# tjtiger86/dl-swin-gan

Measured on AMD Instinct MI355X. Metric: cine slices/sec (fwd+bwd) at 10-iter unroll, 1/2/4/8 GPU; PSNR vs ref, higher is better.
Workload: dtype fp32

## Files before the change

### dl-swin-gan_amd/csrc/conv3d_f16x3.hip

```cpp
#include "conv3d_common.h"
#include "f16x3_common.h"
#include <type_traits>

namespace {
__device__ uint4 g_wg_zero_row[160 / 8];
constexpr int kThinInHalfs = 2 * 4 * 4 * 160 * 8;
constexpr int kThinOutHalfs = 5 * 9 * 2 * 4 * 16 * 8;
constexpr int kThinOutW2 = 5 * 9 * 2 * 4 * 12 * 8;

DLCS_DEV f16x8_t tr_read16h(const f16* p0, const f16* p1) {
    return __builtin_bit_cast(f16x8_t, tr_read16(reinterpret_cast<const bf16*>(p0), reinterpret_cast<const bf16*>(p1)));
}

template <int EPI, int NPASS, bool PREF = true>
DLCS_DEV void conv_epilogue_h3(const ConvF32Args& a, const f32x4_t (&acc)[4][5], float* Es, int pw, int cw0,
                               int lane, int b, int pt, int pyq, int pxq, int nT, int nY, int nX,
                               f16* op, const unsigned* opmax, float* cpart) {
    const float ps = op ? f16x3_scale(*opmax) : 1.0f;
    static_assert(EPI == kEpiRes || EPI == kEpiMask, "fused forms only");
    constexpr int PC = 160 / NPASS, EL = PC + 4, NCH = PC / 8, PER = 256 * NCH / 512;
    static_assert(PC % 8 == 0 && 256 * NCH % 512 == 0 && PC <= 512, "whole 8-channel chunks per thread");
    const float* src = EPI == kEpiRes ? a.res : a.mask;
    const int sld = EPI == kEpiRes ? a.res_ld : a.mask_ld;
    const f16* mp = EPI == kEpiMask ? reinterpret_cast<const f16*>(a.mplanes) : nullptr;
    f32x4_t pre[PREF ? NPASS : 1][PER][2];
    long orows[PER];
    bool oks[PER];
#pragma unroll
    for (int k = 0; k < PER; ++k) {
        const int c = threadIdx.x + k * 512;
        const int vl = c / NCH;
        const int pwv = vl >> 6;
        const int py = pyq + (pwv >> 1), px = pxq + (pwv & 1);
        oks[k] = py < nY && px < nX;
        orows[k] = ((((long)b * nT + pt) * nY + min(py, nY - 1)) * nX + min(px, nX - 1)) * 64 + (vl & 63);
    }
    auto load_pre = [&](int pass, int slot) {
#pragma unroll
        for (int k = 0; k < PER; ++k) {
            const int c = threadIdx.x + k * 512;
            const int co = pass * PC + (c % NCH) * 8;
            if (mp) {
                const f16* q = mp + orows[k] * 320 + (co >> 5) * 64 + (co & 31);
                pre[slot][k][0] = *reinterpret_cast<const f32x4_t*>(q);
                pre[slot][k][1] = *reinterpret_cast<const f32x4_t*>(q + 32);
            } else {
                const float* sp = src + orows[k] * sld + co;
                pre[slot][k][0] = *reinterpret_cast<const f32x4_t*>(sp);
                pre[slot][k][1] = *reinterpret_cast<const f32x4_t*>(sp + 4);
            }
        }
    };
    if constexpr (PREF) {
#pragma unroll
        for (int pass = 0; pass < NPASS; ++pass) load_pre(pass, pass);
    }
    float vmax = 0.0f;
#pragma unroll
    for (int pass = 0; pass < NPASS; ++pass) {
        const int ps_ = PREF ? pass : 0;
        if constexpr (!PREF) load_pre(pass, 0);
#pragma unroll
        for (int j = 0; j < 5; ++j) {
            const int c0 = cw0 + j * 16 - pass * PC;
            if (c0 + 16 <= 0 || c0 >= PC) continue;
#pragma unroll
            for (int i = 0; i < 4; ++i)
#pragma unroll
                for (int r = 0; r < 4; ++r) {
                    const int vl = pw * 64 + i * 16 + (lane >> 4) * 4 + r;
                    const int cl = c0 + (lane & 15);
                    if (cl >= 0 && cl < PC) Es[vl * EL + cl] = acc[i][j][r];
                }
        }
        __syncthreads();
#pragma unroll
        for (int k = 0; k < PER; ++k) {
            const int c = threadIdx.x + k * 512;
            const int vl = c / NCH, ch = (c % NCH) * 8;
            const int co = pass * PC + ch;
            if (!oks[k]) {
                if (cpart) {
                    *reinterpret_cast<f32x4_t*>(Es + vl * EL + ch) = (f32x4_t)0.0f;
                    *reinterpret_cast<f32x4_t*>(Es + vl * EL + ch + 4) = (f32x4_t)0.0f;
                }
                continue;
            }
            f32x4_t v0 = *reinterpret_cast<const f32x4_t*>(Es + vl * EL + ch);
            f32x4_t v1 = *reinterpret_cast<const f32x4_t*>(Es + vl * EL + ch + 4);
            if (a.bias) {
                v0 += *reinterpret_cast<const f32x4_t*>(a.bias + co);
                v1 += *reinterpret_cast<const f32x4_t*>(a.bias + co + 4);
            }
            if (EPI == kEpiMask && mp) {
                const u32x4_h3 hb = __builtin_bit_cast(u32x4_h3, pre[ps_][k][0]);
                const u32x4_h3 lb = __builtin_bit_cast(u32x4_h3, pre[ps_][k][1]);
#pragma unroll
                for (int e = 0; e < 8; ++e) {
                    const unsigned nz = ((hb[e >> 1] | lb[e >> 1]) >> (16 * (e & 1))) & 0x7fffu;
                    if (e < 4) v0[e] = nz ? v0[e] : 0.0f;
                    else v1[e - 4] = nz ? v1[e - 4] : 0.0f;
                }
            } else if (EPI == kEpiMask) {
#pragma unroll
                for (int e = 0; e < 4; ++e) {
                    v0[e] = pre[ps_][k][0][e] > 0.0f ? v0[e] : 0.0f;
                    v1[e] = pre[ps_][k][1][e] > 0.0f ? v1[e] : 0.0f;
                }
            } else {
                v0 += a.res_scale * pre[ps_][k][0];
                v1 += a.res_scale * pre[ps_][k][1];
            }
            if (a.relu_out) {
#pragma unroll
                for (int e = 0; e < 4; ++e) { v0[e] = fmaxf(v0[e], 0.0f); v1[e] = fmaxf(v1[e], 0.0f); }
            }
            if (a.out) {
                float* o = a.out + orows[k] * a.cout_ld + co;
                *reinterpret_cast<f32x4_t*>(o) = v0;
                *reinterpret_cast<f32x4_t*>(o + 4) = v1;
            }
            if (op) put_planes8(op, orows[k], co, v0, v1, ps);
            if (cpart) {
                *reinterpret_cast<f32x4_t*>(Es + vl * EL + ch) = v0;
                *reinterpret_cast<f32x4_t*>(Es + vl * EL + ch + 4) = v1;
            }
            if (a.omax) {
#pragma unroll
                for (int e = 0; e < 4; ++e) vmax = fmaxf(vmax, fmaxf(fabsf(v0[e]), fabsf(v1[e])));
            }
        }
        if (cpart) {
            constexpr int G = 512 / PC;
            __syncthreads();
            float* red = Es + 256 * EL;
            const int t = threadIdx.x;
            if (t < G * PC) {
                const int cc = t % PC, g = t / PC;
                float cs = 0.0f;
                for (int r = g; r < 256; r += G) cs += Es[r * EL + cc];
                red[g * PC + cc] = cs;
            }
            __syncthreads();
            if (t < PC) {
                float cs = 0.0f;
#pragma unroll
                for (int g = 0; g < G; ++g) cs += red[g * PC + t];
                cpart[pass * PC + t] = cs;
            }
        }
        __syncthreads();
    }
    if (a.omax) {
        vmax = wave_max(vmax);
        if ((threadIdx.x & 63) == 0 && vmax > 0.0f && vmax > __uint_as_float(__atomic_load_n(a.omax, __ATOMIC_RELAXED)))
            atomicMax(a.omax, __float_as_uint(vmax));
    }
}

#include "conv3d_f16x3.inc"
#include "conv3d_thin_f16x3.inc"
#include "conv3d_thin_planes.inc"

}

using namespace dlcs_internal;

extern "C" {

#ifdef DLCS_DIAG_BUILD
int dlcs_debug_h3_stamps(void* host, int64_t n) {
    return (int)hipMemcpyFromSymbol(host, HIP_SYMBOL(g_h3_stamps), (size_t)n * 8, 0, hipMemcpyDeviceToHost);
}
#endif

size_t dlcs_conv3d_k3_f16x3_workspace_bytes(int64_t B, int64_t D, int64_t H, int64_t W, int has_colsum) {
    const long ntile = conv_tiles(B, D, H, W);
    return ws_align(colsum_part_bytes(ntile, has_colsum != 0)) + conv_tail_bytes(ntile);
}

int dlcs_conv3d_k3_f16x3(const void* xplanes, const void* wpacked, const float* bias, float* out, int64_t cout_ld,
                         int64_t B, int64_t D, int64_t H, int64_t W, const float* mask, int64_t mask_ld,
                         const float* residual, int64_t res_ld, float res_scale, int accumulate, int relu_out,
                         unsigned* out_max, void* out_planes, float* colsum, const void* mask_planes,
                         void* workspace, size_t workspace_bytes, dlcs_stream_t stream) {
    DLCS_CHECK_ARG(xplanes && wpacked && B > 0 && (out || (out_planes && !accumulate)) && !(mask && mask_planes));
    if (!out) cout_ld = 160;
    const long rows = (long)B * D * H * W;
    if (D % 4 || H % 4 || W % 4 || cout_ld % 4 || !al16(xplanes) || !al16(wpacked) || !al16(out) ||
        (mask && (mask_ld % 4 || !al16(mask))) || (residual && (res_ld % 4 || !al16(residual))) || (bias && !al16(bias)) ||
        rows * 320 >= (1L << 31))
        return DLCS_ERR_UNSUPPORTED_SIZE;
    ConvH3Args v{};
    v.xp = (const f16*)xplanes; v.wp = (const f16*)wpacked;
    v.xmax = planes_trailer(xplanes, rows); v.wmax = (const unsigned*)((const char*)wpacked + kW3Bytes);
    v.bias = bias; v.out = out; v.mask = mask; v.res = residual;
    v.B = (int)B; v.D = (int)D; v.H = (int)H; v.W = (int)W;
    v.cout_ld = (int)cout_ld; v.mask_ld = (int)mask_ld; v.res_ld = (int)res_ld; v.accumulate = accumulate;
    v.relu_out = relu_out; v.res_scale = res_scale; v.omax = out_max;
    if (mask_planes && !al16(mask_planes)) return DLCS_ERR_UNSUPPORTED_SIZE;
    v.mplanes = mask_planes;
    if (out_planes) {
        if (cout_ld != 160 || !al16(out_planes)) return DLCS_ERR_UNSUPPORTED_SIZE;
        v.oplanes = (f16*)out_planes; v.opmax = planes_trailer(out_planes, rows);
    }
#ifdef DLCS_DIAG_BUILD
    static const int stamps = [] { const char* e = dlcs_knob("DLCS_CONV_STAMP"); return e && e[0] == '1'; }();
    v.stamp = stamps;
    static const int h3_exp = [] { const char* e = dlcs_knob("DLCS_H3_EXP"); return e ? atoi(e) : 0; }();
    v.exp = h3_exp;
#endif
    hipStream_t st = (hipStream_t)stream;
    const long ntile = conv_tiles(B, D, H, W);
    if (!ws_ok(workspace, workspace_bytes, dlcs_conv3d_k3_f16x3_workspace_bytes(B, D, H, W, colsum != nullptr)))
        return DLCS_ERR_WORKSPACE;
    if (colsum) v.cpart = static_cast<float*>(workspace);
    float* tail_ws = reinterpret_cast<float*>(static_cast<char*>(workspace) +
                                              ws_align(colsum_part_bytes(ntile, colsum != nullptr)));
    const int rc = conv_f16x3_launch(v, tail_ws, st);
    if (rc || !colsum) return rc;
    return launch_colsum_parts(v.cpart, (int)ntile, colsum, st);
}

size_t dlcs_conv3d_k3_wgrad_f16x3_workspace_bytes(int64_t B, int64_t D, int64_t H, int64_t W) {
    return (size_t)wgh3_ranges(B * (D / 4) * (H / 4) * (W / 4), true).nr * kWgSlabBytes;
}

int dlcs_conv3d_k3_wgrad_f16x3(const void* xplanes, const void* gplanes, float* dw_packed, int64_t B, int64_t D,
                               int64_t H, int64_t W, void* workspace, size_t workspace_bytes,
                               dlcs_stream_t stream) {
    DLCS_CHECK_ARG(xplanes && gplanes && dw_packed && B > 0);
    const long rows = (long)B * D * H * W;
    if (D % 4 || H % 4 || W % 4 || !al16(xplanes) || !al16(gplanes) || rows * 320 >= (1L << 40))
        return DLCS_ERR_UNSUPPORTED_SIZE;
    WgradH3Args v{};
    v.xp = (const f16*)xplanes; v.gp = (const f16*)gplanes;
    v.xmax = planes_trailer(xplanes, rows); v.gmax = planes_trailer(gplanes, rows);
    v.dw = dw_packed; v.B = (int)B; v.D = (int)D; v.H = (int)H; v.W = (int)W;
    if (!ws_ok(workspace, workspace_bytes, dlcs_conv3d_k3_wgrad_f16x3_workspace_bytes(B, D, H, W)))
        return DLCS_ERR_WORKSPACE;
    v.part = static_cast<float*>(workspace);
    return wgrad_f16x3_launch(v, (hipStream_t)stream);
}

size_t dlcs_conv3d_thin_pack_f16x3_bytes(int kind) {
    return (size_t)(kind == 0 ? kThinInHalfs : kThinOutHalfs) * 2 + 256;
}

int dlcs_conv3d_thin_pack_f16x3(const float* wpacked, int64_t cout, int64_t cout_pad, int64_t cin, int64_t cin_pad,
                                int kind, void* out, dlcs_stream_t stream) {
    DLCS_CHECK_ARG(wpacked && out && (kind == 0 || kind == 1) && cout <= cout_pad && cin <= cin_pad);
    if (kind == 0 ? !(cout == 160 && cout_pad == 160 && cin >= 1 && cin <= 4)
                  : !(cin == 160 && cin_pad == 160 && cout >= 1 && cout <= 4))
        return DLCS_ERR_UNSUPPORTED_SIZE;
    if ((uintptr_t)out & 15) return DLCS_ERR_UNSUPPORTED_SIZE;
    hipStream_t st = (hipStream_t)stream;
    const int halfs = kind == 0 ? kThinInHalfs : kThinOutHalfs;
    unsigned* mx = reinterpret_cast<unsigned*>(reinterpret_cast<char*>(out) + (size_t)halfs * 2 + 16);
    if (hipMemsetAsync(mx, 0, 4, st) != hipSuccess) return dlcs_launch_status();
    const long n = 27L * cout_pad * cin_pad;
    const int rc = launch_absmax_flat(wpacked, n, mx, (unsigned)std::min<long>(64, (n / 4 + 255) / 256), st);
    if (rc) return rc;
    hipLaunchKernelGGL(pack_thin_f16x3_grid_kernel, dim3((unsigned)((halfs / 2 + 255) / 256)), dim3(256), 0, st,
                       wpacked, (int)cout, (int)cout_pad, (int)cin, (int)cin_pad, kind, (const unsigned*)mx, (f16*)out);
    return dlcs_launch_status();
}

size_t dlcs_conv3d_thin_f16x3_workspace_bytes(int64_t B, int64_t D, int64_t H, int64_t W, int has_colsum) {
    return colsum_part_bytes(conv_tiles(B, D, H, W), has_colsum != 0);
}

int dlcs_conv3d_thin_f16x3(const float* in, int64_t cin, int64_t cin_ld, const unsigned* in_max, const void* wthin,
                           const float* bias, float* out, int64_t cout, int64_t cout_ld, int64_t B, int64_t D,
                           int64_t H, int64_t W, const float* mask, int64_t mask_ld, const float* residual,
                           int64_t res_ld, float res_scale, int accumulate, int relu_out, unsigned* out_max,
                           void* out_planes, float* colsum, const void* mask_planes, void* workspace,
                           size_t workspace_bytes, dlcs_stream_t stream) {
    DLCS_CHECK_ARG(in && in_max && wthin && B > 0 && (out || out_planes) && !(mask && mask_planes));
    if (!out) cout_ld = 160;
    const long rows = (long)B * D * H * W;
    if (D % 4 || H % 4 || W % 4 || cin_ld % 4 || cout_ld % 4 || !al16(in) || !al16(out) || !al16(wthin) ||
        (bias && !al16(bias)) || rows * std::max(cin_ld, cout_ld) >= (1L << 31) || rows / 64 >= (1L << 24))
        return DLCS_ERR_UNSUPPORTED_SIZE;
    const bool thin_in = cin >= 1 && cin <= 4 && cout == 160;
    const bool thin_out = cin == 160 && cout >= 1 && cout <= 4;
    if (!thin_in && !thin_out) return DLCS_ERR_UNSUPPORTED_SIZE;
    if (thin_in && ((mask && (mask_ld % 4 || !al16(mask))) || (residual && (res_ld % 4 || !al16(residual)))))
        return DLCS_ERR_UNSUPPORTED_SIZE;
    if (thin_out && (mask || residual || out_max || cout_ld < 4)) return DLCS_ERR_UNSUPPORTED_SIZE;
    ConvF32Args v{};
    v.in = in; v.bias = bias; v.out = out; v.mask = mask; v.res = residual;
    v.B = (int)B; v.D = (int)D; v.H = (int)H; v.W = (int)W; v.cin_ld = (int)cin_ld; v.cin_pad = (int)cin;
    v.cout_ld = (int)cout_ld; v.mask_ld = (int)mask_ld; v.res_ld = (int)res_ld; v.accumulate = accumulate;
    v.relu_out = relu_out; v.res_scale = res_scale; v.cout = (int)cout; v.cout_pad = (int)cout; v.omax = out_max;
    v.mplanes = mask_planes;
    hipStream_t st = (hipStream_t)stream;
    if (!thin_in && (out_planes || colsum || mask_planes || !out)) return DLCS_ERR_UNSUPPORTED_SIZE;
    if (mask_planes && !al16(mask_planes)) return DLCS_ERR_UNSUPPORTED_SIZE;
    if (out_planes && (!al16(out_planes) || cout_ld != 160)) return DLCS_ERR_UNSUPPORTED_SIZE;
    const unsigned* opmax = out_planes ? planes_trailer(out_planes, rows) : nullptr;
    const long ntile = conv_tiles(B, D, H, W);
    if (!ws_ok(workspace, workspace_bytes, colsum_part_bytes(ntile, colsum != nullptr))) return DLCS_ERR_WORKSPACE;
    float* cpart = colsum ? static_cast<float*>(workspace) : nullptr;
    const int rc = conv_thin_f16x3_launch(v, (const f16*)wthin, in_max, (int)cin, thin_in, st, (f16*)out_planes, opmax,
                                          cpart);
    if (rc || !colsum) return rc;
    return launch_colsum_parts(cpart, (int)ntile, colsum, st);
}

int dlcs_conv3d_thin_wgrad_f16x3(const float* in, int64_t cin, int64_t cin_ld, const unsigned* in_max,
                                 const float* g, int64_t cout, int64_t g_ld, const unsigned* g_max, float* dw_packed,
                                 int64_t cout_pad, int64_t cin_pad, float* colsum, int64_t B, int64_t D, int64_t H,
                                 int64_t W, dlcs_stream_t stream) {
    DLCS_CHECK_ARG(in && in_max && g && g_max && dw_packed && B > 0 && cout <= cout_pad && cin <= cin_pad);
    const bool thin_sfe = cout == 160 && cin >= 1 && cin <= 4;
    const bool thin_fin = cin == 160 && cout >= 1 && cout <= 4;
    const long npatch = B * (D / 4) * (H / 4) * (W / 4);
    if ((!thin_sfe && !thin_fin) || (colsum && !thin_sfe) || D % 4 || H % 4 || W % 4 || cin_ld % 4 || g_ld % 4 ||
        !al16(in) || !al16(g) || npatch >= (1L << 24))
        return DLCS_ERR_UNSUPPORTED_SIZE;
    ThinWgH3Args t{};
    t.big = thin_sfe ? g : in;
    t.thin = thin_sfe ? in : g;
    t.big_max = thin_sfe ? g_max : in_max;
    t.thin_max = thin_sfe ? in_max : g_max;
    t.dw = dw_packed; t.colsum = colsum;
    t.big_ld = (int)(thin_sfe ? g_ld : cin_ld); t.thin_ld = (int)(thin_sfe ? cin_ld : g_ld);
    t.sgn = thin_sfe ? 1 : -1; t.big_is_co = thin_sfe; t.thin_ch = (int)(thin_sfe ? cin : cout);
    t.cout_pad = (int)cout_pad; t.cin_pad = (int)cin_pad;
    t.B = (int)B; t.D = (int)D; t.H = (int)H; t.W = (int)W;
    const int nr = (int)std::min<long>(256, npatch);
    const int pp = (int)((npatch + nr - 1) / nr);
    hipLaunchKernelGGL(conv3d_wgrad_thin_f16x3_kernel, dim3(nr), dim3(512), 0, (hipStream_t)stream, t, nr, pp);
    return dlcs_launch_status();
}

int dlcs_conv3d_thin_out_planes_f16x3(const void* xplanes, const void* wthin, const float* bias, float* out,
                                      int64_t cout, int64_t cout_ld, int64_t B, int64_t D, int64_t H, int64_t W,
                                      int accumulate, int relu_out, dlcs_stream_t stream) {
    DLCS_CHECK_ARG(xplanes && wthin && out && B > 0 && cout >= 1 && cout <= 4 && cout_ld >= 4);
    if (D % 4 || H % 4 || W % 4 || cout_ld % 4 || !al16(xplanes) || !al16(wthin) || !al16(out))
        return DLCS_ERR_UNSUPPORTED_SIZE;
    ConvF32Args v{};
    v.bias = bias; v.out = out;
    v.B = (int)B; v.D = (int)D; v.H = (int)H; v.W = (int)W;
    v.cout_ld = (int)cout_ld; v.accumulate = accumulate; v.relu_out = relu_out; v.cout = (int)cout;
    v.cout_pad = (int)cout;
    return conv_thin_out_p_launch(v, (const f16*)xplanes, (const f16*)wthin, (hipStream_t)stream);
}

size_t dlcs_conv3d_thin_wgrad_planes_f16x3_workspace_bytes(void) { return (size_t)kTwpWG * 160 * 128 * sizeof(float); }

int dlcs_conv3d_thin_wgrad_planes_f16x3(const void* bigplanes, const float* thin, int64_t thin_ch, int64_t thin_ld,
                                        const unsigned* thin_max, int big_is_co, float* dw_packed, int64_t cout_pad,
                                        int64_t cin_pad, int64_t B, int64_t D, int64_t H, int64_t W, void* workspace,
                                        size_t workspace_bytes, dlcs_stream_t stream) {
    DLCS_CHECK_ARG(bigplanes && thin && thin_max && dw_packed && B > 0 && thin_ch >= 1 && thin_ch <= 4 &&
                   thin_ld >= 4);
    if (D % 4 || H % 4 || W % 4 || thin_ld % 4 || !al16(bigplanes) || !al16(thin) ||
        (big_is_co ? (cout_pad < 160 || cin_pad < thin_ch) : (cin_pad < 160 || cout_pad < thin_ch)))
        return DLCS_ERR_UNSUPPORTED_SIZE;
    ThinWgPArgs t{};
    t.bp = (const f16*)bigplanes; t.thin = thin; t.dw = dw_packed; t.thin_max = thin_max;
    t.rows = (long)B * D * H * W;
    t.thin_ld = (int)thin_ld; t.sgn = big_is_co ? 1 : -1; t.big_is_co = big_is_co ? 1 : 0; t.thin_ch = (int)thin_ch;
    t.cout_pad = (int)cout_pad; t.cin_pad = (int)cin_pad;
    t.B = (int)B; t.D = (int)D; t.H = (int)H; t.W = (int)W;
    if (!ws_ok(workspace, workspace_bytes, dlcs_conv3d_thin_wgrad_planes_f16x3_workspace_bytes()))
        return DLCS_ERR_WORKSPACE;
    t.part = static_cast<float*>(workspace);
    return wgrad_thin_p_launch(t, (hipStream_t)stream);
}

}
```

### dl-swin-gan_amd/csrc/conv3d_f16x3.inc

```
constexpr int kH3Halo = kHalo * 64;
constexpr int kH3Tap = 160 * 64;
constexpr int kH3Slot = 2 * kH3Tap;

struct ConvH3Args {
    const f16* xp; const f16* wp; const unsigned* xmax; const unsigned* wmax;
    const float* bias; float* out; const float* mask; const float* res;
    int B, D, H, W;
    int cout_ld, mask_ld, res_ld, accumulate, relu_out;
    float res_scale;
    unsigned* omax;
    float* part; int tail_base;
    f16* oplanes; const unsigned* opmax;
    float* cpart;
    const void* mplanes;
    int stamp;
    int exp;
};

#ifdef DLCS_DIAG_BUILD
__device__ unsigned long long g_h3_stamps[4096 * 73];
#define H3_STAMP(k) do { if (!TAIL && a.stamp && threadIdx.x == 0 && blockIdx.x < 4096) \
    g_h3_stamps[blockIdx.x * 73 + (k)] = __builtin_readcyclecounter(); } while (0)
#else
#define H3_STAMP(k) do { } while (0)
// ... 285 lines not shown
#pragma unroll
            for (int r = 0; r < 4; ++r)
                acc[i][j][r] *= (FOLD == 3 && ((rsgn >> (4 * (lane >> 4) + r)) & 1)) ? -inv : inv;
    if constexpr (TAIL) {
        float* pp = a.part + (long)blockIdx.x * 256 * 160;
#pragma unroll
        for (int i = 0; i < 4; ++i)
#pragma unroll
            for (int j = 0; j < 5; ++j)
#pragma unroll
                for (int r = 0; r < 4; ++r)
                    pp[(pw * 64 + i * 16 + (lane >> 4) * 4 + r) * 160 + nh * 80 + j * 16 + (lane & 15)] = acc[i][j][r];
        return;
    }
    ConvF32Args ea{};
    ea.bias = a.bias; ea.out = a.out; ea.mask = a.mask; ea.res = a.res;
    ea.cout_ld = a.cout_ld; ea.mask_ld = a.mask_ld; ea.res_ld = a.res_ld; ea.accumulate = a.accumulate;
    ea.relu_out = a.relu_out; ea.res_scale = a.res_scale; ea.omax = a.omax; ea.mplanes = a.mplanes;
    if constexpr (EPI == kEpiRes || EPI == kEpiMask)
        conv_epilogue_h3<EPI, 2>(ea, acc, reinterpret_cast<float*>(smem_h3), pw, nh * 80, lane, b, pt, tyy * 2, txx * 2,
                                 nT, nY, nX, a.oplanes, a.opmax, a.cpart ? a.cpart + (long)vb * 160 : nullptr);
    else
        conv_epilogue_f32<EPI>(ea, acc, reinterpret_cast<float*>(smem_h3), pw, nh * 80, lane, b, pt, tyy * 2, txx * 2,
                               nT, nY, nX);
    H3_STAMP(72);
}

__global__ void __launch_bounds__(256) conv_f16x3_tail_reduce_kernel(ConvH3Args a, int ntail) {
    __shared__ float red[4];
    const int nT = a.D >> 2, nY = a.H >> 2, nX = a.W >> 2;
    const int nYt = (nY + 1) >> 1, nXt = (nX + 1) >> 1;
    const int nblk = a.B * nT * nYt * nXt;
    const long i = (long)blockIdx.x * 256 + threadIdx.x;
    float vmax = 0.0f;
    if (i < (long)ntail * 256 * 40) {
        const int t = (int)(i / (256 * 40)), rem = (int)(i % (256 * 40));
        const int vl = rem / 40, c = (rem % 40) * 4;
        f32x4_t v = (f32x4_t)0.0f;
#pragma unroll
        for (int w = 0; w < 5; ++w) v += *reinterpret_cast<const f32x4_t*>(a.part + ((long)(t * 5 + w) * 256 + vl) * 160 + c);
        const int vb = a.tail_base + t;
        const int q8 = nblk >> 3, r8 = nblk & 7, xcd = vb & 7;
        int bid = xcd * q8 + min(xcd, r8) + (vb >> 3);
        const int txx = bid % nXt; bid /= nXt;
        const int tyy = bid % nYt; bid /= nYt;
        const int pt = bid % nT;
        const int b = bid / nT;
        const int pwv = vl >> 6;
        const int py = tyy * 2 + (pwv >> 1), px = txx * 2 + (pwv & 1);
        if (py < nY && px < nX) {
            const long orow = ((((long)b * nT + pt) * nY + py) * nX + px) * 64 + (vl & 63);
            if (a.bias) v += *reinterpret_cast<const f32x4_t*>(a.bias + c);
            if (a.mask) {
                const f32x4_t m = *reinterpret_cast<const f32x4_t*>(a.mask + orow * a.mask_ld + c);
#pragma unroll
                for (int e = 0; e < 4; ++e) v[e] = m[e] > 0.0f ? v[e] : 0.0f;
            } else if (a.mplanes) {
                const f16* q = reinterpret_cast<const f16*>(a.mplanes) + orow * 320 + (c >> 5) * 64 + (c & 31);
                const f16x4_t h = *reinterpret_cast<const f16x4_t*>(q), l = *reinterpret_cast<const f16x4_t*>(q + 32);
#pragma unroll
                for (int e = 0; e < 4; ++e) v[e] = (h[e] != (f16)0.0f || l[e] != (f16)0.0f) ? v[e] : 0.0f;
            }
            if (a.res) v += a.res_scale * *reinterpret_cast<const f32x4_t*>(a.res + orow * a.res_ld + c);
            if (a.relu_out) {
#pragma unroll
                for (int e = 0; e < 4; ++e) v[e] = fmaxf(v[e], 0.0f);
            }
            if (a.out) {
                float* o = a.out + orow * a.cout_ld + c;
                if (a.accumulate) v += *reinterpret_cast<const f32x4_t*>(o);
                *reinterpret_cast<f32x4_t*>(o) = v;
            }
            if (a.oplanes) put_planes4(a.oplanes, orow, c, v, f16x3_scale(*a.opmax));
            vmax = fmaxf(fmaxf(fabsf(v[0]), fabsf(v[1])), fmaxf(fabsf(v[2]), fabsf(v[3])));
        } else {
            v = (f32x4_t)0.0f;
        }
        if (a.cpart) *reinterpret_cast<f32x4_t*>(a.part + ((long)(t * 5) * 256 + vl) * 160 + c) = v;
    }
    if (a.omax) block_max_to(a.omax, vmax, red);
}

__global__ void __launch_bounds__(160) tail_colsum_kernel(ConvH3Args a, int nparts) {
    const int t = blockIdx.x, c = threadIdx.x;
    const float* p = a.part + (long)(t * nparts) * 256 * 160 + c;
    float cs = 0.0f;
    for (int r = 0; r < 256; ++r) cs += p[(long)r * 160];
    a.cpart[(long)(a.tail_base + t) * 160 + c] = cs;
}

static int conv_f16x3_launch(const ConvH3Args& v0, float* tail_ws, hipStream_t st) {
    ConvH3Args v = v0;
    unsigned nblk = (unsigned)conv_tiles(v.B, v.D, v.H, v.W);
    const char* te = dlcs_test_hook("DLCS_H3_TAIL");
    const bool tail_split = !(te && te[0] == '0');
    const unsigned ntail = tail_split ? conv_tail_tiles(nblk) : 0u, nmain = nblk - ntail;
    const bool split = ntail > 0;
    if (split) nblk = nmain;
    const int epi = conv_epi_code(v.res, v.mask || v.mplanes, !v.accumulate, true);
    if ((v.oplanes || v.cpart || v.mplanes) && epi != kEpiRes && epi != kEpiMask)
        return DLCS_ERR_UNSUPPORTED_SIZE;
    static const int fold_mode = [] {
        const char* e = dlcs_knob("DLCS_H3_FOLD");
        return !e ? 4 : e[0] == '0' ? 0 : e[0] == 'm' ? 2 : e[0] == 'a' ? 3 : e[0] == 'r' ? 4 : e[0] == 'R' ? 5 : 1;
    }();
    const bool masked = v.mask || v.mplanes;
    const int pf = fold_mode == 1 || (fold_mode == 2 && masked) ? 1 : (fold_mode == 3 && masked) ? 2
                 : (fold_mode == 5 || (fold_mode == 4 && masked)) ? 3 : 0;
    auto launch = [&](auto F) {
        constexpr int f = decltype(F)::value;
        const dim3 g(nblk);
        if (epi == 0) hipLaunchKernelGGL((conv3d_k3_f16x3_kernel<0, f>), g, dim3(512), 0, st, v);
        else if (epi == kEpiRes) hipLaunchKernelGGL((conv3d_k3_f16x3_kernel<kEpiRes, f>), g, dim3(512), 0, st, v);
        else if (epi == kEpiMask) hipLaunchKernelGGL((conv3d_k3_f16x3_kernel<kEpiMask, f>), g, dim3(512), 0, st, v);
        else hipLaunchKernelGGL((conv3d_k3_f16x3_kernel<kEpiGeneric, f>), g, dim3(512), 0, st, v);
    };
#ifdef DLCS_DIAG_BUILD
    if (pf == 1) launch(std::integral_constant<int, 1>{});
    else if (pf == 2) launch(std::integral_constant<int, 2>{});
    else
#endif
    if (pf == 3) launch(std::integral_constant<int, 3>{});
    else launch(std::integral_constant<int, 0>{});
    if (split) {
        ConvH3Args t = v;
        t.part = tail_ws;
        t.tail_base = (int)nmain;
#ifdef DLCS_DIAG_BUILD
        if (pf == 1) hipLaunchKernelGGL((conv3d_k3_f16x3_kernel<0, 1, true>), dim3(ntail * 5), dim3(512), 0, st, t);
        else if (pf == 2) hipLaunchKernelGGL((conv3d_k3_f16x3_kernel<0, 2, true>), dim3(ntail * 5), dim3(512), 0, st, t);
        else
#endif
        if (pf == 3) hipLaunchKernelGGL((conv3d_k3_f16x3_kernel<0, 3, true>), dim3(ntail * 5), dim3(512), 0, st, t);
        else hipLaunchKernelGGL((conv3d_k3_f16x3_kernel<0, 0, true>), dim3(ntail * 5), dim3(512), 0, st, t);
        hipLaunchKernelGGL(conv_f16x3_tail_reduce_kernel, dim3((unsigned)cdiv((long)ntail * 256 * 40, 256)), dim3(256),
                           0, st, t, (int)ntail);
        if (v.cpart) hipLaunchKernelGGL(tail_colsum_kernel, dim3(ntail), dim3(160), 0, st, t, 5);
    }
    return dlcs_launch_status();
}

constexpr int kWhRows = 32 + 48;
constexpr int kWhPlane = kWhRows * 160;
constexpr int kWhBuf = 2 * kWhPlane;

struct WgradH3Args {
    const f16* gp; const f16* xp;
    const unsigned* gmax; const unsigned* xmax;
    float* dw;
    float* part;
    int B, D, H, W;
};

__global__ void __launch_bounds__(768) conv3d_wgrad_f16x3_kernel(WgradH3Args a, int nrange, int ppr) {
    __shared__ __attribute__((aligned(16))) f16 smem_wh[3 * kWhBuf];
    const int b = blockIdx.x;
    int range, grp;
    {
        const int xcd = b & 7, slot = b >> 3;
        const int q = nrange >> 3;
        if ((nrange & 7) == 0) { range = (slot / 9) * 8 + xcd; grp = slot % 9; }
        else if ((nrange & 7) == 4) {
            if (slot < 9 * q) { range = (slot / 9) * 8 + xcd; grp = slot % 9; }
            else { range = 8 * q + (xcd & 3); grp = (slot - 9 * q) + (xcd < 4 ? 0 : 5); }
        } else { range = b / 9; grp = b % 9; }
    }
    if (range >= nrange || grp >= 9) return;
    const int kd = grp / 3 - 1, kh = grp % 3 - 1;
    const int nT = a.D >> 2, nY = a.H >> 2, nX = a.W >> 2;
    const int nYX = nY * nX;
    const int npatch = a.B * nT * nYX;
    const int p0 = range * ppr, p1 = min(npatch, p0 + ppr);
    if (p0 >= p1) return;
    const int lane = threadIdx.x & 63, wave = __builtin_amdgcn_readfirstlane(threadIdx.x >> 6);
    const int kwi = wave >> 2, coh = (wave >> 1) & 1, cih = wave & 1;
    const int bias_rows = (nYX + nX + 1) * 64;
    const long rows = (long)npatch * 64;

    unsigned pk[5];
#pragma unroll
    for (int k = 0; k < 5; ++k) {
        const int wi = k * 12 + wave;
        const int pl = wi >= 25 ? 1 : 0, wl = wi - pl * 25;
        const int c = wl * 64 + lane;
        const int row = c / 20, kp = c - row * 20;
        int vrow, swz;
        unsigned req = 0;
        if (wl < 10) {
            vrow = row;
            swz = (row >> 3) & 1;
        } else {
            const int hr = row - 32, ty = hr / 6, xh = hr - ty * 6;
            const int tl = ty >> 2, y = ty & 3;
            swz = (y >> 1) & 1;
            const int tt = tl + kd, yy = y + kh, xx = xh - 1;
            req = (tt < 0 ? 1u : 0u) | (tt >= 4 ? 2u : 0u) | (yy < 0 ? 4u : 0u) | (yy >= 4 ? 8u : 0u) |
                  (xx < 0 ? 16u : 0u) | (xx >= 4 ? 32u : 0u) | (tt + 2 >= 4 ? 64u : 0u);
            vrow = (((tt >> 2) * nYX + (yy >> 2) * nX + (xx >> 2)) << 6) + ((tt & 3) << 4) + ((yy & 3) << 2) +
                   (xx & 3);
        }
        const int kl = kp ^ (swz << 1);
        const unsigned off16 = (unsigned)((vrow + bias_rows) * 40 + (kl >> 2) * 8 + pl * 4 + (kl & 3));
        pk[k] = wi < 50 ? (off16 << 7) | req : 0u;
    }
    const unsigned dst0 = __builtin_amdgcn_readfirstlane(lds_offset(smem_wh));
    int ip = p0, ipt, ipy, ipx;
    {
        const int r = ip % (nT * nYX);
        ipt = r / nYX;
        ipy = (r / nX) % nY;
        ipx = r % nX;
    }
    auto missing = [&]() {
        return (ipt == 0 ? 1u : 0u) | (ipt == nT - 1 ? 2u : 0u) | (ipy == 0 ? 4u : 0u) | (ipy == nY - 1 ? 8u : 0u) |
               (ipx == 0 ? 16u : 0u) | (ipx == nX - 1 ? 32u : 0u);
    };
    auto next_patch = [&]() {
        ++ip;
        if (++ipx == nX) {
            ipx = 0;
            if (++ipy == nY) {
                ipy = 0;
                if (++ipt == nT) ipt = 0;
            }
        }
    };
    const unsigned d32 = 32 * 640, dcross = (unsigned)(nYX * 64 - 32) * 640;
    auto issue_piece = [&](int k, int th, int buf, unsigned miss, const char* gbase, const char* xbase,
                           unsigned xzero) {
        const int wi = k * 12 + wave;
        if (wi >= 50) return;
        const int pl = wi >= 25 ? 1 : 0, wl = wi - pl * 25;
        const unsigned v = pk[k];
        unsigned off = (v >> 3) & ~15u;
        if (wl < 10) {
            if (th) off += d32;
        } else {
            unsigned req = v & 63u;
            if (th) {
                const bool cross = (v & 65u) != 0u;
                off += cross ? dcross : d32;
                req = (v & 60u) | ((v >> 5) & 2u);
            }
            off = (req & miss) ? xzero : off;
        }
        glds16_s(wl < 10 ? gbase : xbase, off, dst0 + (unsigned)(buf * kWhBuf * 2 + pl * kWhPlane * 2 + wl * 1024));
    };
    auto bases = [&](const char*& gb, const char*& xb, unsigned& xz) {
        const long r0 = (long)ip * 64 - bias_rows;
        gb = reinterpret_cast<const char*>(a.gp) + r0 * 640;
        xb = reinterpret_cast<const char*>(a.xp) + r0 * 640;
        xz = (unsigned)(h3_zero_row_byte(rows) - r0 * 640);
    };

    f32x4_t acc[5][5];
#pragma unroll
    for (int i = 0; i < 5; ++i)
#pragma unroll
        for (int j = 0; j < 5; ++j) acc[i][j] = (f32x4_t)0.0f;

    const int gq = lane >> 4, q = (lane >> 2) & 3, p4 = (lane & 3) * 4, swb = gq & 1;
    auto acol = [&](int i) { return (((coh * 5 + i) ^ swb) << 4) + p4; };
    auto bcol = [&](int j) { return (((cih * 5 + j) ^ swb) << 4) + p4; };
    const int grow = (8 * gq + q) * 160;
    const int xrow = (32 + ((gq >> 1) * 4 + 2 * swb) * 6 + q + kwi) * 160;

    {
        const char *gb, *xb;
        unsigned xz;
        bases(gb, xb, xz);
        const unsigned miss = missing();
#pragma unroll
        for (int k = 0; k < 5; ++k) issue_piece(k, 0, 0, miss, gb, xb, xz);
#pragma unroll
        for (int k = 0; k < 5; ++k) issue_piece(k, 1, 1, miss, gb, xb, xz);
    }
    next_patch();
    asm volatile("s_waitcnt vmcnt(0)" ::: "memory");
    __syncthreads();
    int cur = 0;
    auto unit = [&](int TH, bool ahead) {
#pragma unroll
        for (int k = 0; k < 5; ++k) asm volatile("" : "+v"(pk[k]));
        const int nbuf = cur == 0 ? 2 : cur - 1;
        const char *gb, *xb;
        unsigned xz;
        bases(gb, xb, xz);
        const unsigned miss = missing();
        const f16* S = smem_wh + cur * kWhBuf;
        const f16* Gh = S + grow;
        const f16* Gl = S + kWhPlane + grow;
        const f16* Xh = S + xrow;
        const f16* Xl = S + kWhPlane + xrow;
        f16x8_t gh[5], gl[5];
#pragma unroll
        for (int i = 0; i < 5; ++i) gh[i] = tr_read16h(Gh + acol(i), Gh + 4 * 160 + acol(i));
        f16x8_t xh = tr_read16h(Xh + bcol(0), Xh + 6 * 160 + bcol(0));
        f16x8_t xl = tr_read16h(Xl + bcol(0), Xl + 6 * 160 + bcol(0));
#pragma unroll
        for (int j = 0; j < 5; ++j) {
            if (j == 0) {
#pragma unroll
                for (int i = 0; i < 5; ++i) gl[i] = tr_read16h(Gl + acol(i), Gl + 4 * 160 + acol(i));
            }
#pragma unroll
            for (int i = 0; i < 5; ++i) mfma16h(acc[i][j], gh[i], xh);
#pragma unroll
            for (int i = 0; i < 5; ++i) mfma16h(acc[i][j], gh[i], xl);
#pragma unroll
            for (int i = 0; i < 5; ++i) mfma16h(acc[i][j], gl[i], xh);
            if (ahead) issue_piece(j, TH, nbuf, miss, gb, xb, xz);
            if (j + 1 < 5) {
                xh = tr_read16h(Xh + bcol(j + 1), Xh + 6 * 160 + bcol(j + 1));
                xl = tr_read16h(Xl + bcol(j + 1), Xl + 6 * 160 + bcol(j + 1));
            }
        }
        if (!ahead) asm volatile("s_waitcnt vmcnt(0)" ::: "memory");
        else if (wave < 2) asm volatile("s_waitcnt vmcnt(5)" ::: "memory");
        else asm volatile("s_waitcnt vmcnt(4)" ::: "memory");
        __syncthreads();
        cur = cur == 2 ? 0 : cur + 1;
    };
    for (int u = 2 * p0; u < 2 * p1; ++u) {
        const int th = u & 1;
        unit(th, (u >> 1) + 1 < p1);
        if (th) next_patch();
    }
    const int tap = (kd + 1) * 9 + (kh + 1) * 3 + kwi;
    float* pp = a.part + ((long)range * 27 + tap) * 160 * 160;
    float* st = reinterpret_cast<float*>(smem_wh) + wave * (16 * 84);
#pragma unroll
    for (int i = 0; i < 5; ++i) {
#pragma unroll
        for (int j = 0; j < 5; ++j)
#pragma unroll
            for (int r = 0; r < 4; ++r) st[(gq * 4 + r) * 84 + j * 16 + (lane & 15)] = acc[i][j][r];
#pragma unroll
        for (int s = 0; s < 5; ++s) {
            const int e = s * 64 + lane, r = e / 20, c4 = (e % 20) * 4;
            const f32x4_t v = *reinterpret_cast<const f32x4_t*>(st + r * 84 + c4);
            *reinterpret_cast<f32x4_t*>(pp + (coh * 80 + 16 * i + r) * 160 + cih * 80 + c4) = v;
        }
    }
}

__global__ void __launch_bounds__(256) wgrad_f16x3_reduce_kernel(WgradH3Args a, int nrange) {
    const long i = (long)blockIdx.x * 256 + threadIdx.x;
    if (i >= 27L * 160 * 40) return;
    const float inv = 1.0f / (f16x3_scale(*a.gmax) * f16x3_scale(*a.xmax));
    const f32x4_t* src = reinterpret_cast<const f32x4_t*>(a.part);
    f32x4_t s = src[i];
    for (int r = 1; r < nrange; ++r) s += src[(long)r * 27 * 160 * 40 + i];
    f32x4_t* d = reinterpret_cast<f32x4_t*>(a.dw) + i;
    *d = *d + s * inv;
}

constexpr int kWgH3MaxRanges = 32;

static PatchRanges wgh3_ranges(long npatch, bool bound) {
    static const int env_nr = [] { const char* e = dlcs_knob("DLCS_WGH3_RANGES"); return e ? atoi(e) : 0; }();
    return patch_ranges(npatch, bound ? kWgH3MaxRanges : env_nr > 0 ? std::min(env_nr, kWgH3MaxRanges) : 28);
}

static int wgrad_f16x3_launch(const WgradH3Args& a, hipStream_t st) {
    const long npatch = (long)a.B * (a.D / 4) * (a.H / 4) * (a.W / 4);
    const long bias_rows = ((long)(a.H / 4) * (a.W / 4) + a.W / 4 + 1) * 64;
    if ((2 * bias_rows + 128) * 40 >= (1L << 25) || (npatch * 64 + bias_rows) * 640 + 1024 >= (1L << 32))
        return DLCS_ERR_UNSUPPORTED_SIZE;
    const PatchRanges r = wgh3_ranges(npatch, false);
    const int nr = r.nr;
    const long pp = r.pp;
    hipLaunchKernelGGL(conv3d_wgrad_f16x3_kernel, dim3((unsigned)(9 * nr)), dim3(768), 0, st, a, nr, (int)pp);
    hipLaunchKernelGGL(wgrad_f16x3_reduce_kernel, dim3((unsigned)cdiv(27L * 160 * 40, 256)), dim3(256), 0, st, a, nr);
    return dlcs_launch_status();
}
```

### dl-swin-gan_amd/csrc/conv3d_thin_planes.inc

```

constexpr int kTpHY = 10, kTpHX = 6, kTpHalo = 6 * kTpHY * kTpHX;
constexpr int kTpBuf = kTpHalo * 64;
constexpr int kTpPieces = kTpHalo * 8 / 64;

#ifdef DLCS_DIAG_BUILD
__global__ void __launch_bounds__(512, 1) conv3d_thin_out_p_kernel(ConvF32Args a, const f16* xp, const f16* wimg,
                                                                   long rows) {
    __shared__ __attribute__((aligned(16))) f16 smem_tp[2 * kTpBuf + kThinOutW2];
    f16* Wl = smem_tp + 2 * kTpBuf;
    for (int i = threadIdx.x; i < kThinOutW2 / 8; i += 512) {
        const int n = i % 12, rest = i / 12;
        const int kg = rest & 3, pl = (rest >> 2) & 1, ck = rest >> 3;
        reinterpret_cast<uint4*>(Wl)[i] = reinterpret_cast<const uint4*>(wimg)[(ck * 1024 + pl * 512 + (kg * 16 + n) * 8) / 8];
    }
    const float sx = f16x3_scale(*reinterpret_cast<const unsigned*>(reinterpret_cast<const char*>(xp) + rows * 640));
    const float inv = 1.0f / (sx * *reinterpret_cast<const float*>(wimg + kThinOutHalfs));
    const int nT = a.D >> 2, nY = a.H >> 2, nX = a.W >> 2;
    const int nYX = nY * nX, nYt = (nY + 1) >> 1;
    const int lane = threadIdx.x & 63, wave = __builtin_amdgcn_readfirstlane(threadIdx.x >> 6);
    const int m = lane & 15, kg = lane >> 4;
    const int wn = m < 12 ? m : 11;
    const int bias_rows = (nYX + nX + 1) * 64;

    unsigned pk[6];
#pragma unroll
    for (int k = 0; k < 6; ++k) {
        const int wi = 8 * k + wave;
        const int hv = min(wi * 8 + (lane >> 3), kTpHalo - 1);
        const int ht = hv / (kTpHY * kTpHX), hy = (hv / kTpHX) % kTpHY, hx = hv % kTpHX;
        const int L = (lane & 7) ^ (((hv >> 1) & 3) << 1);
        const int t = ht - 1, y = hy - 1, x = hx - 1;
        const int dt = t >> 2, dy = y >> 2, dx = x >> 2;
        const unsigned req = (dt < 0 ? 1u : 0u) | (dt > 0 ? 2u : 0u) | (dy < 0 ? 4u : 0u) | (dy == 1 ? 8u : 0u) |
                             (dy == 2 ? 16u : 0u) | (dx < 0 ? 32u : 0u) | (dx > 0 ? 64u : 0u);
        const int rel = ((dt * nYX + dy * nX + dx) << 6) + ((t & 3) << 4) + ((y & 3) << 2) + (x & 3);
        const unsigned off16 = (unsigned)((rel + bias_rows) * 40 + L);
        pk[k] = wi < kTpPieces ? (off16 << 8) | req : 0u;
    }
    const unsigned dst0 = __builtin_amdgcn_readfirstlane(lds_offset(smem_tp));
    const int nBY = (nYt + 3) >> 2, nBX = (nX + 7) >> 3;
    const int nblocks = a.B * nT * nBY * nBX, xcd = blockIdx.x & 7, kw = blockIdx.x >> 3;
    const int nrounds = xcd < nblocks ? (nblocks - xcd + 7) >> 3 : 0;
    const int nitems = nrounds * 5;
    auto decode = [&](int r, int& b, int& pt, int& py2, int& px) {
        int bid = r * 8 + xcd;
        const int bx = bid % nBX; bid /= nBX;
        const int by = bid % nBY; bid /= nBY;
        pt = bid % nT;
        b = bid / nT;
        py2 = by * 4 + (kw >> 3);
        px = bx * 8 + (kw & 7);
        return py2 < nYt && px < nX;
    };
    auto issue = [&](int s) {
        if (s >= nitems) return;
        int b, pt, py2, px;
        if (!decode(s / 5, b, pt, py2, px)) return;
        const int cc = s % 5;
        const long r0 = ((((long)b * nT + pt) * nY + 2 * py2) * nX + px) * 64 - bias_rows;
        const char* sb = reinterpret_cast<const char*>(xp) + r0 * 640 + cc * 128;
        const unsigned zoff = (unsigned)(rows * 640 + 256 - r0 * 640 - cc * 128);
        const unsigned miss = (pt == 0 ? 1u : 0u) | (pt == nT - 1 ? 2u : 0u) | (py2 == 0 ? 4u : 0u) |
                              (2 * py2 + 1 >= nY ? 8u : 0u) | (2 * py2 + 2 >= nY ? 16u : 0u) | (px == 0 ? 32u : 0u) |
                              (px == nX - 1 ? 64u : 0u);
        const unsigned dst = dst0 + (unsigned)((s & 1) * kTpBuf * 2);
#pragma unroll
        for (int k = 0; k < 6; ++k) {
            const int wi = 8 * k + wave;
            if (wi < kTpPieces) {
                const unsigned v = pk[k];
                const unsigned off = (v & miss) ? zoff : ((v >> 4) & ~15u);
                glds16_s(sb, off, dst + (unsigned)(wi * 1024));
            }
        }
    };
    int hb[3];
#pragma unroll
    for (int i = 0; i < 3; ++i) {
        const int r = 16 * (3 * (wave & 3) + i) + m;
        const int xq = r % 6, y = (r / 6) % 8, t = r / 48;
        hb[i] = (t * kTpHY + y) * kTpHX + xq;
    }
    const int kk0 = wave < 4 ? 0 : 5, kk1 = wave < 4 ? 5 : 9;
    f32x4_t acc[3];
#pragma unroll
    for (int i = 0; i < 3; ++i) acc[i] = (f32x4_t)0.0f;

    issue(0);
    asm volatile("s_waitcnt vmcnt(0)" ::: "memory");
    __syncthreads();
    for (int s = 0; s < nitems; ++s) {
#pragma unroll
        for (int k = 0; k < 6; ++k) asm volatile("" : "+v"(pk[k]));
        issue(s + 1);
        const int cc = s % 5;
        int b, pt, py2, px;
        const bool live = decode(s / 5, b, pt, py2, px);
        const f16* Hs = smem_tp + (s & 1) * kTpBuf;
        const f16* wc = Wl + cc * 9 * 768 + (kg * 12 + wn) * 8;
        for (int kk = live ? kk0 : kk1; kk < kk1; ++kk) {
            const int kd = kk / 3, kh = kk - 3 * kd;
            const f16* wb = wc + kk * 768;
            const f16x8_t bh = *reinterpret_cast<const f16x8_t*>(wb);
            const f16x8_t bl = *reinterpret_cast<const f16x8_t*>(wb + 384);
#pragma unroll
            for (int i = 0; i < 3; ++i) {
                const int R = hb[i] + (kd * kTpHY + kh) * kTpHX;
                const int swz = ((R >> 1) & 3) << 1;
                const f16x8_t ah = *reinterpret_cast<const f16x8_t*>(Hs + R * 64 + ((kg ^ swz) << 3));
                const f16x8_t al = *reinterpret_cast<const f16x8_t*>(Hs + R * 64 + (((4 + kg) ^ swz) << 3));
                f32x4_t t = (f32x4_t)0.0f;
                mfma16h(t, al, bh);
                mfma16h(t, ah, bl);
                mfma16h(t, ah, bh);
                acc[i] += t;
            }
        }
        if (cc == 4 && live) {
            __syncthreads();
            float* Q = reinterpret_cast<float*>(smem_tp + (s & 1) * kTpBuf);
#pragma unroll
            for (int i = 0; i < 3; ++i)
#pragma unroll
                for (int r = 0; r < 4; ++r)
                    Q[((wave >> 2) * 192 + 16 * (3 * (wave & 3) + i) + 4 * kg + r) * 17 + m] = acc[i][r] * inv;
#pragma unroll
            for (int i = 0; i < 3; ++i) acc[i] = (f32x4_t)0.0f;
            __syncthreads();
            if (threadIdx.x < 128) {
                const int v = threadIdx.x;
                const int t = v >> 5, y = (v >> 2) & 7, x = v & 3;
                const int py = 2 * py2 + (y >> 2);
                if (py < nY) {
                    f32x4_t o = (f32x4_t)0.0f;
#pragma unroll
                    for (int kw = 0; kw < 3; ++kw) {
                        const int qr = (t * 8 + y) * 6 + x + kw;
#pragma unroll
                        for (int co = 0; co < 4; ++co) o[co] += Q[qr * 17 + kw * 4 + co] + Q[(192 + qr) * 17 + kw * 4 + co];
                    }
                    const long row = brow(b, pt * 4 + t, py * 4 + (y & 3), px * 4 + x, nT, nY, nX);
                    float* op = a.out + row * a.cout_ld;
                    if (a.bias) for (int co = 0; co < a.cout; ++co) o[co] += a.bias[co];
                    if (a.relu_out) for (int co = 0; co < 4; ++co) o[co] = fmaxf(o[co], 0.0f);
                    if (a.accumulate) o += *reinterpret_cast<const f32x4_t*>(op);
                    *reinterpret_cast<f32x4_t*>(op) = o;
                }
            }
        }
        asm volatile("s_waitcnt vmcnt(0)" ::: "memory");
        __syncthreads();
    }
}
#endif

template <int SET>
DLCS_DEV void thin_out_p3_b(const f16* wimg, int cc, int kk0, int kg, int m, f16x8_t (&bh)[2][5], f16x8_t (&bl)[2][5]) {
#pragma unroll
    for (int q = 0; q < 5; ++q) {
        const int kk = min(kk0 + q, 8);
        const f16* wb = wimg + (cc * 9 + kk) * 1024 + (kg * 16 + m) * 8;
        bh[SET][q] = *reinterpret_cast<const f16x8_t*>(wb);
        bl[SET][q] = *reinterpret_cast<const f16x8_t*>(wb + 512);
    }
}

__global__ void __launch_bounds__(512, 1) conv3d_thin_out_p3_kernel(ConvF32Args a, const f16* xp, const f16* wimg,
                                                                    long rows) {
    __shared__ __attribute__((aligned(16))) f16 smem_tp3[3 * kTpBuf];
    const float sx = f16x3_scale(*reinterpret_cast<const unsigned*>(reinterpret_cast<const char*>(xp) + rows * 640));
    const float inv = 1.0f / (sx * *reinterpret_cast<const float*>(wimg + kThinOutHalfs));
    const int nT = a.D >> 2, nY = a.H >> 2, nX = a.W >> 2;
    const int nYX = nY * nX, nYt = (nY + 1) >> 1;
    const int lane = threadIdx.x & 63, wave = __builtin_amdgcn_readfirstlane(threadIdx.x >> 6);
    const int m = lane & 15, kg = lane >> 4;
    const int bias_rows = (nYX + nX + 1) * 64;
    unsigned pk[6];
#pragma unroll
    for (int k = 0; k < 6; ++k) {
        const int wi = 8 * k + wave;
        const int hv = min(wi * 8 + (lane >> 3), kTpHalo - 1);
        const int ht = hv / (kTpHY * kTpHX), hy = (hv / kTpHX) % kTpHY, hx = hv % kTpHX;
        const int L = (lane & 7) ^ (((hv >> 1) & 3) << 1);
        const int t = ht - 1, y = hy - 1, x = hx - 1;
        const int dt = t >> 2, dy = y >> 2, dx = x >> 2;
        const unsigned req = (dt < 0 ? 1u : 0u) | (dt > 0 ? 2u : 0u) | (dy < 0 ? 4u : 0u) | (dy == 1 ? 8u : 0u) |
                             (dy == 2 ? 16u : 0u) | (dx < 0 ? 32u : 0u) | (dx > 0 ? 64u : 0u);
        const int rel = ((dt * nYX + dy * nX + dx) << 6) + ((t & 3) << 4) + ((y & 3) << 2) + (x & 3);
        const unsigned off16 = (unsigned)((rel + bias_rows) * 40 + L);
        pk[k] = wi < kTpPieces ? (off16 << 8) | req : 0u;
    }
    const int npc = wave < kTpPieces - 40 ? 6 : 5;
    const unsigned dst0 = __builtin_amdgcn_readfirstlane(lds_offset(smem_tp3));
    const int nBY = (nYt + 3) >> 2, nBX = (nX + 7) >> 3;
    const int nblocks = a.B * nT * nBY * nBX, xcd = blockIdx.x & 7, kw = blockIdx.x >> 3;
    const int nrounds = xcd < nblocks ? (nblocks - xcd + 7) >> 3 : 0;
    const int nitems = nrounds * 5;
    auto decode = [&](int r, int& b, int& pt, int& py2, int& px) {
        int bid = r * 8 + xcd;
        const int bx = bid % nBX; bid /= nBX;
        const int by = bid % nBY; bid /= nBY;
        pt = bid % nT;
        b = bid / nT;
        py2 = by * 4 + (kw >> 3);
        px = bx * 8 + (kw & 7);
        return py2 < nYt && px < nX;
    };
    auto issue = [&](int s) {
        if (s >= nitems) return 0;
        int b, pt, py2, px;
        if (!decode(s / 5, b, pt, py2, px)) return 0;
        const int cc = s % 5;
        const long r0 = ((((long)b * nT + pt) * nY + 2 * py2) * nX + px) * 64 - bias_rows;
        const char* sb = reinterpret_cast<const char*>(xp) + r0 * 640 + cc * 128;
        const unsigned zoff = (unsigned)(rows * 640 + 256 - r0 * 640 - cc * 128);
        const unsigned miss = (pt == 0 ? 1u : 0u) | (pt == nT - 1 ? 2u : 0u) | (py2 == 0 ? 4u : 0u) |
                              (2 * py2 + 1 >= nY ? 8u : 0u) | (2 * py2 + 2 >= nY ? 16u : 0u) | (px == 0 ? 32u : 0u) |
                              (px == nX - 1 ? 64u : 0u);
        const unsigned dst = dst0 + (unsigned)((s % 3) * kTpBuf * 2);
#pragma unroll
        for (int k = 0; k < 6; ++k) {
            const int wi = 8 * k + wave;
            if (wi < kTpPieces) {
                const unsigned v = pk[k];
                const unsigned off = (v & miss) ? zoff : ((v >> 4) & ~15u);
                glds16_s(sb, off, dst + (unsigned)(wi * 1024));
            }
        }
        return npc;
    };
    auto vmwait = [&](int n) {
        if (n >= 6) asm volatile("s_waitcnt vmcnt(6)" ::: "memory");
        else if (n == 5) asm volatile("s_waitcnt vmcnt(5)" ::: "memory");
        else asm volatile("s_waitcnt vmcnt(0)" ::: "memory");
    };
    int hb[3];
#pragma unroll
    for (int i = 0; i < 3; ++i) {
        const int r = 16 * (3 * (wave & 3) + i) + m;
        const int xq = r % 6, y = (r / 6) % 8, t = r / 48;
        hb[i] = (t * kTpHY + y) * kTpHX + xq;
    }
    const int kk0 = wave < 4 ? 0 : 5, nkk = wave < 4 ? 5 : 4;
    f32x4_t acc[3];
#pragma unroll
    for (int i = 0; i < 3; ++i) acc[i] = (f32x4_t)0.0f;
    f16x8_t bh[2][5], bl[2][5];

    thin_out_p3_b<0>(wimg, 0, kk0, kg, m, bh, bl);
    issue(0);
    const int n1 = issue(1);
    vmwait(n1);
    __syncthreads();
    auto body = [&](int s, auto SETc) {
        constexpr int SET = decltype(SETc)::value;
#pragma unroll
        for (int k = 0; k < 6; ++k) asm volatile("" : "+v"(pk[k]));
        if (s + 1 < nitems) thin_out_p3_b<SET ^ 1>(wimg, (s + 1) % 5, kk0, kg, m, bh, bl);
        const int n2 = issue(s + 2);
        const int cc = s % 5;
        int b, pt, py2, px;
        const bool live = decode(s / 5, b, pt, py2, px);
        const f16* Hs = smem_tp3 + (s % 3) * kTpBuf;
        if (live) {
#pragma unroll
            for (int q = 0; q < 5; ++q) {
                if (q < nkk) {
                    const int kk = kk0 + q;
                    const int kd = kk / 3, kh = kk - 3 * kd;
#pragma unroll
                    for (int i = 0; i < 3; ++i) {
                        const int R = hb[i] + (kd * kTpHY + kh) * kTpHX;
                        const int swz = ((R >> 1) & 3) << 1;
                        const f16x8_t ah = *reinterpret_cast<const f16x8_t*>(Hs + R * 64 + ((kg ^ swz) << 3));
                        const f16x8_t al = *reinterpret_cast<const f16x8_t*>(Hs + R * 64 + (((4 + kg) ^ swz) << 3));
                        f32x4_t t = (f32x4_t)0.0f;
                        mfma16h(t, al, bh[SET][q]);
                        mfma16h(t, ah, bl[SET][q]);
                        mfma16h(t, ah, bh[SET][q]);
                        acc[i] += t;
                    }
                }
            }
        }
        if (cc == 4 && live) {
            __syncthreads();
            float* Q = reinterpret_cast<float*>(smem_tp3 + (s % 3) * kTpBuf);
#pragma unroll
            for (int i = 0; i < 3; ++i)
#pragma unroll
                for (int r = 0; r < 4; ++r)
                    Q[((wave >> 2) * 192 + 16 * (3 * (wave & 3) + i) + 4 * kg + r) * 17 + m] = acc[i][r] * inv;
#pragma unroll
            for (int i = 0; i < 3; ++i) acc[i] = (f32x4_t)0.0f;
            __syncthreads();
            if (threadIdx.x < 128) {
                const int v = threadIdx.x;
                const int t = v >> 5, y = (v >> 2) & 7, x = v & 3;
                const int py = 2 * py2 + (y >> 2);
                if (py < nY) {
                    f32x4_t o = (f32x4_t)0.0f;
#pragma unroll
                    for (int kw3 = 0; kw3 < 3; ++kw3) {
                        const int qr = (t * 8 + y) * 6 + x + kw3;
#pragma unroll
                        for (int co = 0; co < 4; ++co) o[co] += Q[qr * 17 + kw3 * 4 + co] + Q[(192 + qr) * 17 + kw3 * 4 + co];
                    }
                    const long row = brow(b, pt * 4 + t, py * 4 + (y & 3), px * 4 + x, nT, nY, nX);
                    float* op = a.out + row * a.cout_ld;
                    if (a.bias) for (int co = 0; co < a.cout; ++co) o[co] += a.bias[co];
                    if (a.relu_out) for (int co = 0; co < 4; ++co) o[co] = fmaxf(o[co], 0.0f);
                    if (a.accumulate) o += *reinterpret_cast<const f32x4_t*>(op);
                    *reinterpret_cast<f32x4_t*>(op) = o;
                }
            }
        }
        vmwait(n2);
        __syncthreads();
    };
    for (int s = 0; s < nitems; s += 2) {
        body(s, std::integral_constant<int, 0>{});
        if (s + 1 < nitems) body(s + 1, std::integral_constant<int, 1>{});
    }
}

static int conv_thin_out_p_launch(const ConvF32Args& v, const f16* xp, const f16* wimg, hipStream_t st) {
    const int nT = v.D / 4, nY = v.H / 4, nX = v.W / 4;
    const long rows = (long)v.B * v.D * v.H * v.W;
    const long bias_rows = ((long)nY * nX + nX + 1) * 64;
    if ((2 * bias_rows + 4L * nX * 64 + 256) * 40 >= (1L << 24) || (rows + bias_rows) * 640 + 1024 >= (1L << 32))
        return DLCS_ERR_UNSUPPORTED_SIZE;
#ifdef DLCS_DIAG_BUILD
    static const bool p2 = [] { const char* e = dlcs_knob("DLCS_THIN_OUT_P2"); return e && e[0] == '1'; }();
    if (p2) hipLaunchKernelGGL(conv3d_thin_out_p_kernel, dim3(256), dim3(512), 0, st, v, xp, wimg, rows);
    else
#endif
    hipLaunchKernelGGL(conv3d_thin_out_p3_kernel, dim3(256), dim3(512), 0, st, v, xp, wimg, rows);
    return dlcs_launch_status();
}

struct ThinWgPArgs {
    const f16* bp; const float* thin; float* dw; float* part;
    const unsigned* thin_max;
    long rows;
    int thin_ld, sgn, big_is_co, thin_ch, cout_pad, cin_pad;
    int B, D, H, W;
};
constexpr int kTwImg = 32 * 160;
constexpr int kTwBigB = 2 * 2 * kTwImg;
constexpr int kTwTR = 256 * 8;
constexpr int kTwBuf = kTwBigB + kTwTR;
constexpr int kTwIm = 32 * 128;

__global__ void __launch_bounds__(512, 1) conv3d_wgrad_thin_p_kernel(ThinWgPArgs a, int ppr) {
    __shared__ __attribute__((aligned(16))) f16 smem_twp[2 * kTwBuf + 4 * kTwIm];
    f16* IM = smem_twp + 2 * kTwBuf;
    const int nT = a.D >> 2, nY = a.H >> 2, nX = a.W >> 2;
    const int npatch = a.B * nT * nY * nX;
    const int p0 = (int)blockIdx.x * ppr, p1 = min(npatch, p0 + ppr);
    const int tid = threadIdx.x, lane = tid & 63, wave = __builtin_amdgcn_readfirstlane(tid >> 6);
    const float st = f16x3_scale(*a.thin_max);
    for (int i = tid; i < 4 * 32 * 20; i += 512) {
        const int img = i / 640, r = (i / 20) % 32, c = 108 + i % 20;
        IM[img * kTwIm + r * 128 + (c ^ (((r >> 3) & 1) << 4))] = (f16)0.0f;
    }
    unsigned boff[5];
#pragma unroll
    for (int k = 0; k < 5; ++k) {
        const int wi = 8 * k + wave, wl = wi % 10, pl = (wi / 10) & 1, un = wi / 20;
        const int c = wl * 64 + lane;
        const int row = c / 20, kp = c - row * 20;
        const int kl = kp ^ (((row >> 3) & 1) << 1);
        boff[k] = (unsigned)(((un * 32 + row) * 320 + (kl >> 2) * 64 + pl * 32 + (kl & 3) * 8) * 2);
    }
    const unsigned lds0 = __builtin_amdgcn_readfirstlane(lds_offset(smem_twp));
    auto coords = [&](int patch, int& bb, int& pt, int& py, int& px) {
        px = patch % nX;
        int r = patch / nX;
        py = r % nY; r /= nY;
        pt = r % nT;
        bb = r / nT;
    };
    auto issue = [&](int patch, int buf) {
        if (patch >= p1) return;
        const char* sb = reinterpret_cast<const char*>(a.bp) + (long)patch * 64 * 640;
        const unsigned dst = lds0 + (unsigned)(buf * kTwBuf * 2);
#pragma unroll
        for (int k = 0; k < 5; ++k) {
            const int wi = 8 * k + wave, wl = wi % 10, pl = (wi / 10) & 1, un = wi / 20;
            glds16_s(sb, boff[k], dst + (unsigned)((un * 2 + pl) * kTwImg * 2 + wl * 1024));
        }
        if (wave < 4) {
            int bb, pt, py, px;
            coords(patch, bb, pt, py, px);
            const int hv = min(wave * 64 + lane, 215);
            const int ht = hv / 36, hy = (hv / 6) % 6, hx = hv % 6;
            const int T = min(max(pt * 4 - 1 + ht, 0), a.D - 1), Y = min(max(py * 4 - 1 + hy, 0), a.H - 1),
                      X = min(max(px * 4 - 1 + hx, 0), a.W - 1);
            glds16(a.thin + brow(bb, T, Y, X, nT, nY, nX) * a.thin_ld,
                   dst + (unsigned)(kTwBigB * 2 + wave * 1024));
        }
    };
    const int jtap = tid >> 3, tc = tid & 7;
    const int skd = a.sgn * (jtap / 9 - 1), skh = a.sgn * ((jtap / 3) % 3 - 1), skw = a.sgn * (jtap % 3 - 1);
    auto build = [&](int patch, int buf) {
        if (tid >= 216) return;
        int bb, pt, py, px;
        coords(patch, bb, pt, py, px);
        const float* TR = reinterpret_cast<const float*>(smem_twp + buf * kTwBuf + kTwBigB);
        const int t = tc >> 1;
        const bool tok = (unsigned)(pt * 4 + t + skd) < (unsigned)a.D;
#pragma unroll
        for (int j = 0; j < 8; ++j) {
            const int y = 2 * (tc & 1) + (j >> 2), x = j & 3;
            const bool ok = tok && (unsigned)(py * 4 + y + skh) < (unsigned)a.H && (unsigned)(px * 4 + x + skw) < (unsigned)a.W;
            const int hv = (t + 1 + skd) * 36 + (y + 1 + skh) * 6 + (x + 1 + skw);
            f32x4_t v = *reinterpret_cast<const f32x4_t*>(TR + hv * 4);
            f16x4_t h, l;
#pragma unroll
            for (int e = 0; e < 4; ++e) {
                const float u = (ok && e < a.thin_ch) ? v[e] * st : 0.0f;
                const f16 hh = (f16)u;
                h[e] = hh;
                l[e] = (f16)(u - (float)hh);
            }
            const int un = t >> 1, row = (t & 1) * 16 + y * 4 + x;
            const int col = (jtap * 4) ^ (((row >> 3) & 1) << 4);
            *reinterpret_cast<f16x4_t*>(IM + (un * 2 + 0) * kTwIm + row * 128 + col) = h;
            *reinterpret_cast<f16x4_t*>(IM + (un * 2 + 1) * kTwIm + row * 128 + col) = l;
        }
    };

    const int mh = wave & 1, nq = wave >> 1;
    f32x4_t acc[5][2];
#pragma unroll
    for (int i = 0; i < 5; ++i)
#pragma unroll
        for (int j = 0; j < 2; ++j) acc[i][j] = (f32x4_t)0.0f;
    const int gq = lane >> 4, q = (lane >> 2) & 3, p4 = (lane & 3) * 4, swb = gq & 1;
    auto acol = [&](int i) { return (((mh * 5 + i) ^ swb) << 4) + p4; };
    auto bcol = [&](int j) { return (((nq * 2 + j) ^ swb) << 4) + p4; };
    const int grow = (8 * gq + q) * 160, trow = (8 * gq + q) * 128;

    if (p0 < p1) issue(p0, 0);
    asm volatile("s_waitcnt vmcnt(0)" ::: "memory");
    __syncthreads();
    for (int p = p0; p < p1; ++p) {
#pragma unroll
        for (int k = 0; k < 5; ++k) asm volatile("" : "+v"(boff[k]));
        const int buf = (p - p0) & 1;
        issue(p + 1, buf ^ 1);
        build(p, buf);
        __syncthreads();
#pragma unroll
        for (int un = 0; un < 2; ++un) {
            const f16* Gh = smem_twp + buf * kTwBuf + (un * 2) * kTwImg + grow;
            const f16* Gl = Gh + kTwImg;
            const f16* Th = IM + (un * 2) * kTwIm + trow;
            const f16* Tl = Th + kTwIm;
            f16x8_t bh[2], bl[2];
#pragma unroll
            for (int j = 0; j < 2; ++j) {
                bh[j] = tr_read16h(Th + bcol(j), Th + 4 * 128 + bcol(j));
                bl[j] = tr_read16h(Tl + bcol(j), Tl + 4 * 128 + bcol(j));
            }
#pragma unroll
            for (int i = 0; i < 5; ++i) {
                const f16x8_t gh = tr_read16h(Gh + acol(i), Gh + 4 * 160 + acol(i));
                const f16x8_t gl = tr_read16h(Gl + acol(i), Gl + 4 * 160 + acol(i));
#pragma unroll
                for (int j = 0; j < 2; ++j) {
                    mfma16h(acc[i][j], gh, bh[j]);
                    mfma16h(acc[i][j], gh, bl[j]);
                    mfma16h(acc[i][j], gl, bh[j]);
                }
            }
        }
        asm volatile("s_waitcnt vmcnt(0)" ::: "memory");
        __syncthreads();
    }
    float* pp = a.part + (long)blockIdx.x * 160 * 128;
#pragma unroll
    for (int i = 0; i < 5; ++i)
#pragma unroll
        for (int j = 0; j < 2; ++j)
#pragma unroll
            for (int r = 0; r < 4; ++r)
                pp[(16 * (mh * 5 + i) + 4 * gq + r) * 128 + 16 * (nq * 2 + j) + (lane & 15)] = acc[i][j][r];
}

__global__ void __launch_bounds__(256) wgrad_thin_p_reduce_kernel(ThinWgPArgs a, int nwg) {
    __shared__ float red[4][64];
    const int o = blockIdx.x * 64 + (threadIdx.x & 63), wq = threadIdx.x >> 6;
    float s4[4] = {0.0f, 0.0f, 0.0f, 0.0f};
    const int per = nwg / 4;
    const float* pp = a.part + (long)(wq * per) * 160 * 128 + o;
    for (int w = 0; w < per; w += 4) {
#pragma unroll
        for (int u = 0; u < 4; ++u) s4[u] += pp[(long)(w + u) * 160 * 128];
    }
    red[wq][threadIdx.x & 63] = (s4[0] + s4[1]) + (s4[2] + s4[3]);
    __syncthreads();
    if (wq != 0) return;
    const int mm = o / 128, n = o % 128, tap = n >> 2, s = n & 3;
    if (n >= 108 || s >= a.thin_ch) return;
    const int l = threadIdx.x;
    const float v = (red[0][l] + red[1][l]) + (red[2][l] + red[3][l]);
    const unsigned bmax = *reinterpret_cast<const unsigned*>(reinterpret_cast<const char*>(a.bp) + a.rows * 640);
    const float inv = 1.0f / (f16x3_scale(bmax) * f16x3_scale(*a.thin_max));
    const int co = a.big_is_co ? mm : s, ci = a.big_is_co ? s : mm;
    float* d = a.dw + ((long)tap * a.cout_pad + co) * a.cin_pad + ci;
    *d += v * inv;
}

constexpr int kTwpWG = 256;

static int wgrad_thin_p_launch(const ThinWgPArgs& a, hipStream_t st) {
    const long npatch = (long)a.B * (a.D / 4) * (a.H / 4) * (a.W / 4);
    if (npatch * 64 * 640 >= (1L << 32)) return DLCS_ERR_UNSUPPORTED_SIZE;
    const int ppr = (int)((npatch + kTwpWG - 1) / kTwpWG);
    hipLaunchKernelGGL(conv3d_wgrad_thin_p_kernel, dim3(kTwpWG), dim3(512), 0, st, a, ppr);
    hipLaunchKernelGGL(wgrad_thin_p_reduce_kernel, dim3(160 * 128 / 64), dim3(256), 0, st, a, kTwpWG);
    return dlcs_launch_status();
}
```

### dl-swin-gan_amd/dl_cs/_lib.py

```python
import ctypes
import os

import torch

_HERE = os.path.dirname(os.path.abspath(__file__))
LIB_PATH = os.environ.get("DLCS_HIP_LIB", os.path.join(_HERE, "libdlcs_hip.so"))

F32, BF16 = 0, 1
_LIB = None

_P = ctypes.c_void_p
_I64 = ctypes.c_int64
_INT = ctypes.c_int
_F = ctypes.c_float
_SZ = ctypes.c_size_t

SIGNATURES = {
    "dlcs_version": [],
    "dlcs_status_string": [_INT],
    "dlcs_sense_workspace_bytes": [_I64, _I64, _I64, _I64, _I64],
    "dlcs_sense_fwd": [_P, _P, _P, _I64, _P, _I64, _I64, _I64, _I64, _I64, _I64, _P, _SZ, _P],
    "dlcs_sense_adj": [_P, _P, _P, _I64, _P, _P, _P, _F, _I64, _I64, _I64, _I64, _I64, _I64, _P, _SZ, _P],
    "dlcs_sense_normal": [_P, _P, _P, _I64, _P, _P, _F, _F, _I64, _I64, _I64, _I64, _I64, _I64, _P, _SZ, _P],
    "dlcs_sense_cg_workspace_bytes": [_I64] * 6,
    "dlcs_sense_cg": [_P, _P, _P, _P, _I64, _F, _INT, _I64, _I64, _I64, _I64, _I64, _I64, _P, _SZ, _P],
    "dlcs_sense_rowtab_bytes": [_I64] * 4,
    "dlcs_sense_rowtab": [_P, _I64, _I64, _I64, _I64, _I64, _P, _SZ, _P],
    "dlcs_sense_rows_workspace_bytes": [_I64] * 5,
    "dlcs_sense_adj_rows": [_P, _P, _P, _I64, _P, _I64, _P, _P, _P, _F, _I64, _I64, _I64, _I64, _I64, _I64, _P,
                            _SZ, _P],
    "dlcs_sense_normal_rows": [_P, _P, _P, _I64, _P, _I64, _P, _P, _F, _F, _I64, _I64, _I64, _I64, _I64, _I64, _P,
                               _SZ, _P],
    "dlcs_sense_cg_rows": [_P, _P, _P, _P, _I64, _P, _I64, _F, _INT, _I64, _I64, _I64, _I64, _I64, _I64, _P, _SZ, _P],
    "dlcs_fft2": [_P, _P, _I64, _I64, _I64, _INT, _P, _SZ, _P],
    "dlcs_fft_plan": [_I64, _P, _P],
    "dlcs_window_index": [_I64] * 10 + [_P, _P, _P, _P],
    "dlcs_gather_rows": [_INT, _INT, _P, _P, _P, _I64, _I64, _I64, _I64, _P],
    "dlcs_layernorm_fwd": [_INT, _P, _P, _P, _P, _F, _P, _P, _P, _I64, _I64, _P],
    "dlcs_layernorm_bwd_workspace_bytes": [_I64, _I64],
    "dlcs_layernorm_bwd": [_P, _P, _P, _P, _P, _P, _P, _P, _P, _P, _I64, _I64, _P, _SZ, _P],
    "dlcs_colsum": [_INT, _P, _I64, _I64, _I64, _P, _P],
    "dlcs_gemm": [_INT, _I64, _I64, _I64, _P, _I64, _INT, _P, _I64, _INT, _P, _I64, _INT,
                  _P, _INT, _P, _P, _I64, _F, _P, _I64, _INT, _F, _P, _I64, _INT, _F, _P, _INT, _INT, _P],
    "dlcs_gemm_dw_workspace_bytes": [_INT, _P, _P, _I64],
    "dlcs_gemm_dw_grouped": [_INT, _P, _P, _P, _P, _P, _P, _P, _P, _P, _I64, _P, _SZ, _P],
    "dlcs_gemm_dw_grouped_f32": [_INT, _P, _P, _P, _P, _P, _P, _P, _P, _P, _I64, _P, _SZ, _P],
    "dlcs_window_attn_fwd": [_INT, _P, _P, _P, _P, _P, _P, _I64, _I64, _I64, _I64, _I64,
                             _I64, _I64, _I64, _F, _P],
    "dlcs_window_attn_bwd": [_INT, _P, _P, _P, _P, _P, _P, _P, _I64, _P, _P, _I64, _I64, _I64, _I64,
                             _I64, _I64, _I64, _F, _P],
    "dlcs_conv3d_k3_workspace_bytes": [_INT, _I64, _I64, _I64, _I64, _INT, _I64, _I64, _I64, _I64],
    "dlcs_conv3d_k3": [_INT, _P, _I64, _I64, _P, _I64, _P, _P, _INT, _I64, _I64, _I64, _I64, _I64, _I64,
                       _I64, _INT, _P, _I64, _P, _INT, _I64, _F, _INT, _INT, _P, _SZ, _P],
    "dlcs_conv3d_k3_wgrad_workspace_bytes": [_INT, _I64, _I64, _I64, _I64, _INT, _INT, _I64, _I64, _I64, _I64],
    "dlcs_conv3d_k3_wgrad": [_INT, _P, _I64, _I64, _I64, _INT, _P, _I64, _I64, _I64, _P, _P, _I64, _I64, _I64,
                             _I64, _I64, _P, _SZ, _P],
    "dlcs_conv3d_pack_weights": [_INT, _P, _P, _I64, _I64, _I64, _I64, _INT, _P],
    "dlcs_conv3d_unpack_wgrad": [_P, _P, _I64, _I64, _I64, _I64, _INT, _P],
    "dlcs_split2_f16_bytes": [_I64],
    "dlcs_split2_f16_workspace_bytes": [_I64, _INT],
    "dlcs_split2_f16": [_P, _I64, _I64, _P, _INT, _P, _P, _SZ, _P],
    "dlcs_conv3d_pack_weights_f16x3_bytes": [],
    "dlcs_conv3d_pack_weights_f16x3": [_P, _INT, _P, _P],
    "dlcs_gemm_k160_f16x3_workspace_bytes": [_I64, _I64, _INT],
    "dlcs_gemm_k160_f16x3": [_P, _I64, _P, _I64, _P, _I64, _P, _INT, _F, _P, _I64, _F, _P, _I64, _F, _INT, _P, _P, _P,
                             _P, _P, _P, _SZ, _P],
    "dlcs_planes_bound": [_P, _I64, _P, _P, _F, _P, _P, _F, _P, _I64, _F, _P],
    "dlcs_abs_row_sum_max": [_P, _I64, _I64, _I64, _I64, _I64, _P, _P],
    "dlcs_h3r_pack_bytes": [_I64, _I64],
    "dlcs_h3r_pack_multi": [_INT, _P, _P, _P, _P, _P, _P, _P],
    "dlcs_gemm_h3r_workspace_bytes": [_I64, _I64, _I64, _INT, _INT, _INT],
    "dlcs_gemm_h3r": [_P, _I64, _I64, _I64, _P, _I64, _P, _I64, _P, _INT, _P, _P, _I64, _F, _P, _I64, _P, _INT, _P, _SZ,
                      _P],
    "dlcs_f8r_quant": [_P, _I64, _I64, _I64, _P, _P, _P],
    "dlcs_gemm_f8r": [_P, _P, _I64, _I64, _P, _P, _I64, _P, _I64, _P, _INT, _P, _I64, _F, _P, _I64, _P, _P],
    "dlcs_linear_k160_f16x3": [_P, _I64, _P, _I64, _P, _I64, _P, _INT, _P, _P, _I64, _F, _P, _I64, _P, _INT, _P],
    "dlcs_gemm_f32_splitk_det": [_P, _I64, _P, _I64, _I64, _I64, _I64, _P, _P, _SZ, _P],
    "dlcs_gemm_f32_splitk_det_workspace_bytes": [_I64, _I64],
    "dlcs_conv3d_k3_wgrad_f16x3_workspace_bytes": [_I64] * 4,
    "dlcs_conv3d_k3_wgrad_f16x3": [_P, _P, _P, _I64, _I64, _I64, _I64, _P, _SZ, _P],
    "dlcs_conv3d_k3_f16x3_workspace_bytes": [_I64, _I64, _I64, _I64, _INT],
    "dlcs_conv3d_k3_f16x3": [_P, _P, _P, _P, _I64, _I64, _I64, _I64, _I64, _P, _I64, _P, _I64, _F, _INT, _INT, _P, _P, _P,
                             _P, _P, _SZ, _P],
    "dlcs_conv3d_thin_pack_f16x3_bytes": [_INT],
    "dlcs_conv3d_thin_pack_f16x3": [_P, _I64, _I64, _I64, _I64, _INT, _P, _P],
    "dlcs_absmax_f32": [_P, _I64, _P, _P],
    "dlcs_conv3d_thin_f16x3_workspace_bytes": [_I64, _I64, _I64, _I64, _INT],
    "dlcs_conv3d_thin_f16x3": [_P, _I64, _I64, _P, _P, _P, _P, _I64, _I64, _I64, _I64, _I64, _I64, _P, _I64, _P,
                               _I64, _F, _INT, _INT, _P, _P, _P, _P, _P, _SZ, _P],
    "dlcs_conv3d_thin_out_planes_f16x3": [_P, _P, _P, _P, _I64, _I64, _I64, _I64, _I64, _I64, _INT, _INT, _P],
    "dlcs_conv3d_thin_wgrad_planes_f16x3_workspace_bytes": [],
    "dlcs_conv3d_thin_wgrad_planes_f16x3": [_P, _P, _I64, _I64, _P, _INT, _P, _I64, _I64, _I64, _I64, _I64, _I64,
                                            _P, _SZ, _P],
    "dlcs_conv3d_thin_wgrad_f16x3": [_P, _I64, _I64, _P, _P, _I64, _I64, _P, _P, _I64, _I64, _P, _I64, _I64, _I64,
                                     _I64, _P],
    "dlcs_swin_pre": [_INT, _P, _P, _I64, _I64, _I64, _I64, _I64, _I64, _I64, _P],
    "dlcs_swin_pre_bwd": [_INT, _P, _P, _I64, _I64, _I64, _I64, _I64, _I64, _I64, _P],
    "dlcs_swin_post": [_INT, _P, _P, _I64, _I64, _I64, _I64, _I64, _I64, _I64, _P],
    "dlcs_swin_post_bwd": [_INT, _P, _P, _I64, _I64, _I64, _I64, _I64, _I64, _I64, _P],
    "dlcs_box_pre": [_P, _P] + [_I64] * 10 + [_P],
    "dlcs_box_pre_bwd": [_P, _P] + [_I64] * 10 + [_P],
    "dlcs_box_post": [_P, _P] + [_I64] * 10 + [_P],
    "dlcs_box_post_bwd": [_P, _P] + [_I64] * 10 + [_P],
    "dlcs_box_zero": [_P] + [_I64] * 9 + [_P],
    "dlcs_box_shift": [_P, _I64, _P] + [_I64] * 12 + [_INT, _P, _I64, _INT, _P],
    "dlcs_box_pre_bf16": [_P, _P] + [_I64] * 10 + [_P],
    "dlcs_box_post_bwd_bf16": [_P, _P] + [_I64] * 10 + [_P],
    "dlcs_box_zero_bf16": [_P] + [_I64] * 9 + [_P],
    "dlcs_axpby": [_INT, _INT, _P, _P, _I64, _F, _F, _P],
    "dlcs_relu_grad": [_INT, _P, _INT, _P, _I64, _P],
    "dlcs_permute": [_INT, _INT, _P, _P, _I64, _P, _P, _INT, _P],
    "dlcs_fill_bias": [_P, _P, _I64, _I64, _I64, _P],
    "dlcs_block_layout": [_INT, _INT, _P, _P, _I64, _I64, _I64, _I64, _I64, _I64, _INT, _P],
    "dlcs_cast_multi_bf16": [_I64, _P, _P, _P, _P],
    "dlcs_kt_window_average": [_P, _P, _I64, _I64, _I64, _I64, _INT, _P],
    "dlcs_kth_largest_abs": [_P, _I64, _I64, _P, _P],
    "dlcs_cplx_mask_scale": [_P, _P, _P, _I64, _I64, _I64, _P, _INT, _P],
    "dlcs_crop_flip": [_P, _P, _I64, _I64, _I64, _I64, _I64, _I64, _I64, _I64, _INT, _INT, _INT, _P],
    "dlcs_mhsa_fwd": [_INT, _P, _P, _P, _I64, _I64, _I64, _I64, _F, _P],
    "dlcs_mhsa_bwd_workspace_bytes": [_I64, _I64, _I64],
    "dlcs_mhsa_bwd": [_INT, _P, _P, _P, _P, _P, _I64, _I64, _I64, _I64, _F, _P, _SZ, _P],
    "dlcs_conv3d_thin_im2col": [_P, _I64, _I64, _P, _I64, _INT, _I64, _I64, _I64, _I64, _P],
    "dlcs_conv3d_thin_col2im": [_P, _I64, _I64, _P, _I64, _P, _INT, _INT, _I64, _I64, _I64, _I64, _P],
    "dlcs_dit_vec": [_INT, _P, _P, _P, _I64, _P],
    "dlcs_timestep_embedding": [_P, _I64, _I64, _F, _P, _P],
    "dlcs_scale_rows": [_P, _P, _P, _P, _P, _I64, _I64, _P],
    "dlcs_gated_linear_grad": [_P, _P, _P, _P, _P, _P, _P, _P, _I64, _I64, _P],
    "dlcs_rows_add": [_P, _P, _P, _I64, _I64, _P],
    "dlcs_se_pool_workspace_bytes": [_I64, _I64, _I64],
    "dlcs_se_pool": [_P, _I64, _I64, _I64, _I64, _P, _P, _SZ, _P],
    "dlcs_se_pool_bf16": [_P, _I64, _I64, _I64, _I64, _P, _P, _SZ, _P],
    "dlcs_se_gate": [_P, _P, _P, _P, _P, _I64, _I64, _I64, _P, _P, _P],
    "dlcs_se_scale_res_relu": [_P, _P, _P, _P, _I64, _I64, _I64, _I64, _P],
    "dlcs_se_scale_res_relu_bf16": [_P, _P, _P, _P, _I64, _I64, _I64, _I64, _P],
    "dlcs_se_bwd_reduce_workspace_bytes": [_I64, _I64, _I64],
    "dlcs_se_bwd_reduce": [_P, _P, _P, _I64, _I64, _I64, _I64, _P, _P, _SZ, _P],
    "dlcs_se_bwd_reduce_bf16": [_P, _P, _P, _I64, _I64, _I64, _I64, _P, _P, _SZ, _P],
    "dlcs_se_gate_bwd_workspace_bytes": [_I64, _I64, _I64],
    "dlcs_se_gate_bwd": [_P, _P, _P, _P, _P, _P, _I64, _I64, _I64, _F, _P, _P, _P, _P, _P, _P, _SZ, _P],
    "dlcs_se_bwd_apply": [_P, _P, _P, _P, _P, _I64, _I64, _I64, _I64, _P],
    "dlcs_se_bwd_apply_bf16": [_P, _P, _P, _P, _P, _I64, _I64, _I64, _I64, _P],
    "dlcs_cbam_chan_mean": [_P, _P, _I64, _I64, _I64, _I64, _I64, _I64, _P, _P],
    "dlcs_cbam_chan_mean_bf16": [_P, _P, _I64, _I64, _I64, _I64, _I64, _I64, _P, _P],
    "dlcs_cbam_stencil5": [_P, _P, _P, _INT, _P, _I64, _I64, _I64, _I64, _P],
    "dlcs_cbam_stencil5_wgrad_workspace_bytes": [_I64, _I64, _I64, _I64],
    "dlcs_cbam_stencil5_wgrad": [_P, _P, _I64, _I64, _I64, _I64, _P, _P, _P, _SZ, _P],
    "dlcs_cbam_scale_res_relu": [_P, _P, _P, _P, _P, _I64, _I64, _I64, _I64, _I64, _I64, _P],
    "dlcs_cbam_scale_res_relu_bf16": [_P, _P, _P, _P, _P, _I64, _I64, _I64, _I64, _I64, _I64, _P],
    "dlcs_cbam_bwd_rowdot": [_P, _P, _P, _P, _I64, _I64, _I64, _I64, _I64, _I64, _P, _P],
    "dlcs_cbam_bwd_rowdot_bf16": [_P, _P, _P, _P, _I64, _I64, _I64, _I64, _I64, _I64, _P, _P],
    "dlcs_cbam_bwd_reduce_workspace_bytes": [_I64, _I64, _I64, _I64, _I64],
    "dlcs_cbam_bwd_reduce": [_P, _P, _P, _P, _P, _I64, _I64, _I64, _I64, _I64, _I64, _P, _P, _SZ, _P],
    "dlcs_cbam_bwd_reduce_bf16": [_P, _P, _P, _P, _P, _I64, _I64, _I64, _I64, _I64, _I64, _P, _P, _SZ, _P],
    "dlcs_cbam_bwd_apply": [_P, _P, _P, _P, _P, _P, _P, _I64, _I64, _I64, _I64, _I64, _I64, _P],
    "dlcs_cbam_bwd_apply_bf16": [_P, _P, _P, _P, _P, _P, _P, _I64, _I64, _I64, _I64, _I64, _I64, _P],
    "dlcs_lr_extract": [_P, _P, _P, _INT, _P, _I64, _I64, _I64, _I64, _I64, _P],
    "dlcs_lr_combine": [_P, _P, _P, _INT, _P, _I64, _I64, _I64, _I64, _I64, _P],
    "dlcs_lr_compose": [_P, _P, _P, _P, _INT, _P, _I64, _I64, _I64, _I64, _I64, _I64, _P],
    "dlcs_lr_project_l": [_P, _P, _P, _P, _INT, _P, _I64, _I64, _I64, _I64, _I64, _I64, _P],
    "dlcs_lr_project_r": [_P, _P, _P, _P, _INT, _P, _I64, _I64, _I64, _I64, _I64, _I64, _P],
    "dlcs_lr_decompose": [_P, _P, _P, _P, _P, _P, _I64, _I64, _I64, _I64, _I64, _I64, _P],
    "dlcs_conv2d_k3": [_P, _I64, _I64, _P, _I64, _P, _P, _INT, _I64, _I64, _I64, _I64, _I64, _I64, _INT, _P, _I64,
                       _P, _INT, _I64, _F, _INT, _P],
    "dlcs_conv2d_pack_weights": [_P, _P, _I64, _I64, _I64, _I64, _INT, _INT, _P],
    "dlcs_conv2d_k3_wgrad_workspace_bytes": [_I64, _I64, _I64, _I64, _I64, _INT, _I64],
    "dlcs_conv2d_k3_wgrad": [_P, _I64, _I64, _I64, _P, _I64, _I64, _I64, _P, _P, _I64, _I64, _I64, _INT, _I64, _P, _SZ, _P],
    "dlcs_conv2d_unpack_wgrad": [_P, _P, _I64, _I64, _I64, _I64, _INT, _INT, _P],
}
DIAG_SIGNATURES = {
    "dlcs_conv3d_k3_x6": [_P, _P, _P, _P, _P, _I64, _I64, _I64, _I64, _I64, _P, _I64, _P, _I64, _F, _INT,
                          _INT, _P],
    "dlcs_split3_bf16": [_P, _I64, _I64, _P, _P, _P],
    "dlcs_conv3d_k3_wgrad_x6": [_P, _P, _P, _P, _P, _I64, _I64, _I64, _I64, _P],
    "dlcs_gemm_nt_x6": [_P, _I64, _P, _I64, _I64, _I64, _I64, _P, _P, _SZ, _P],
    "dlcs_gemm_nt_x6_workspace_bytes": [_I64, _I64, _I64],
    "dlcs_debug_conv_stamps": [_P, _I64],
    "dlcs_debug_h3_stamps": [_P, _I64],
}
_RESTYPE = {name: _SZ for name in list(SIGNATURES) + list(DIAG_SIGNATURES) if name.endswith("_bytes")}
_RESTYPE["dlcs_status_string"] = ctypes.c_char_p


class DlcsError(RuntimeError):
    pass


def lib():
    global _LIB
    if _LIB is None:
        if not os.path.exists(LIB_PATH):
            raise DlcsError(f"libdlcs_hip.so not found at {LIB_PATH}; build it with "
                            "`make -C dl-swin-gan_amd/csrc` (or __graft_entry__.build())")
        L = ctypes.CDLL(LIB_PATH)
        for name, args in SIGNATURES.items():
            fn = getattr(L, name)
            fn.argtypes = args
            fn.restype = _RESTYPE.get(name, _INT)
        for name, args in DIAG_SIGNATURES.items():
            if hasattr(L, name):
                fn = getattr(L, name)
                fn.argtypes = args
                fn.restype = _RESTYPE.get(name, _INT)
        _LIB = L
    return _LIB


def exported_symbols():
    return sorted(SIGNATURES.keys())


def has_symbol(name):
    return hasattr(lib(), name)


def check(status, name):
    if status != 0:
        msg = lib().dlcs_status_string(int(status))
        raise DlcsError(f"{name} failed with status {status}: {msg.decode() if msg else '?'}")


def call(name, *args):
    check(getattr(lib(), name)(*args), name)


_RAW_STREAM = getattr(torch._C, "_cuda_getCurrentRawStream", None)
_GET_DEVICE = getattr(torch._C, "_cuda_getDevice", None)


def stream():
    if _RAW_STREAM is not None and _GET_DEVICE is not None:
        return ctypes.c_void_p(_RAW_STREAM(_GET_DEVICE()))
    return ctypes.c_void_p(torch.cuda.current_stream().cuda_stream)


def ptr(t):
    return None if t is None else ctypes.c_void_p(t.data_ptr())


def require_gpu(*tensors):
    for t in tensors:
        if t is not None and not t.is_cuda:
            raise DlcsError("dl_cs HIP ops need GPU tensors (no CPU fallback in the product path)")


def dtype_code(dt):
    if dt == torch.float32:
# ... 5 lines not shown
```

### dl-swin-gan_amd/dl_cs/models/_ops.py

```python
import ctypes

import torch

from .. import _lib
from .. import diag as _diag

F32, BF16 = _lib.F32, _lib.BF16
_I64P = ctypes.POINTER(ctypes.c_int64)


def code(t_or_dtype):
    dt = t_or_dtype.dtype if torch.is_tensor(t_or_dtype) else t_or_dtype
    return _lib.dtype_code(dt)


p = _lib.ptr
S = _lib.stream
call = _lib.call


def empty(shape, dtype, device):
    return torch.empty(shape, dtype=dtype, device=device)


# ... 262 lines not shown
    lse = empty((nwin, heads, N), torch.float32, qkv.device)
    call("dlcs_window_attn_fwd", code(qkv), p(qkv), p(out), p(lse), p(table), p(labels), p(mask),
         int(mask_nw), nwin, N, heads, hd, window0[0], window0[1], window0[2], float(scale), S())
    return out, lse


def attn_bwd(qkv, out, dout, lse, table, labels, dtable, nwin, N, heads, hd, window0, scale,
             mask=None, mask_nw=0):
    dqkv = empty(qkv.shape, torch.float32, qkv.device)
    call("dlcs_window_attn_bwd", code(qkv), p(qkv), p(out), p(dout), p(lse), p(table), p(labels),
         p(mask), int(mask_nw), p(dqkv), p(dtable), nwin, N, heads, hd, window0[0], window0[1],
         window0[2], float(scale), S())
    return dqkv


def pad32(n):
    return (n + 31) // 32 * 32


def conv_pack(w, dtype, mode):
    cout, cin = w.shape[0], w.shape[1]
    rows, cols = (pad32(cout), pad32(cin)) if mode == 0 else (pad32(cin), pad32(cout))
    out = empty((27, rows, cols), dtype, w.device)
    call("dlcs_conv3d_pack_weights", code(out), p(w.contiguous()), p(out), cout, cin, rows, cols, mode, S())
    return out


def conv3d(x, cin, packed, cout, out_ld, grid, bias=None, out=None, out_dtype=None, relu_in=0,
           mask=None, res=None, res_scale=1.0, accumulate=0, relu_out=0):
    B, D, H, W = grid
    rows = B * D * H * W
    if out is None:
        out = empty((rows, out_ld), out_dtype or x.dtype, x.device)
    ws, nb = _ws("dlcs_conv3d_k3", out.device, code(x), cin, packed.shape[2], cout, packed.shape[1], int(relu_in),
             B, D, H, W)
    call("dlcs_conv3d_k3", code(x), p(x), cin, x.shape[-1], p(packed), packed.shape[2], p(bias),
         p(out), code(out), cout, packed.shape[1], out.shape[-1], B, D, H, W, int(relu_in),
         p(mask), mask.shape[-1] if mask is not None else 0, p(res),
         code(res) if res is not None else F32, res.shape[-1] if res is not None else 0,
         float(res_scale), int(accumulate), int(relu_out), p(ws), nb, S())
    return out


def split3(x, out=None):
    rows = x.shape[0]
    if out is None:
        out = (empty((rows, 320), torch.bfloat16, x.device), empty((rows, 160), torch.bfloat16, x.device))
    call("dlcs_split3_bf16", p(x), rows, x.shape[-1], p(out[0]), p(out[1]), S())
    return out


def conv_pack_x6(w, mode):
    packed = empty((27 * 160 * 480,), torch.bfloat16, w.device)
    call("dlcs_conv3d_pack_weights", F32, p(w.contiguous()), p(packed), 160, 160, 0, 0, 2 + mode, S())
    return packed


def conv3d_x6(planes, packed, grid, bias=None, out=None, mask=None, res=None, res_scale=1.0, accumulate=0,
              relu_out=0):
    B, D, H, W = grid
    xa, xb = planes
    if out is None:
        out = empty((xa.shape[0], 160), torch.float32, xa.device)
    call("dlcs_conv3d_k3_x6", p(xa), p(xb), p(packed), p(bias), p(out), out.shape[-1], B, D, H, W, p(mask),
         mask.shape[-1] if mask is not None else 0, p(res), res.shape[-1] if res is not None else 0,
         float(res_scale), int(accumulate), int(relu_out), S())
    return out


def conv3d_wgrad_x6(x_planes, g_planes, grid, dw_packed):
    B, D, H, W = grid
    call("dlcs_conv3d_k3_wgrad_x6", p(x_planes[0]), p(x_planes[1]), p(g_planes[0]), p(g_planes[1]), p(dw_packed),
         B, D, H, W, S())
    return dw_packed


def split2(x, out=None, have_max=False, colsum=None):
    rows = x.shape[0]
    if out is None:
        out = empty((int(_lib.lib().dlcs_split2_f16_bytes(rows)),), torch.uint8, x.device)
    ws, nb = _ws("dlcs_split2_f16", out.device, rows, colsum is not None)
    call("dlcs_split2_f16", p(x), rows, x.shape[-1], p(out), int(bool(have_max)), p(colsum), p(ws), nb, S())
    return out


def planes_alloc(rows, device):
    out = empty((int(_lib.lib().dlcs_split2_f16_bytes(rows)),), torch.uint8, device)
    out[rows * 640:rows * 640 + 4].zero_()
    return out


def planes_max(planes, rows):
    return ctypes.c_void_p(planes.data_ptr() + rows * 640)


def conv_pack_f16x3(w, mode):
    packed = empty((int(_lib.lib().dlcs_conv3d_pack_weights_f16x3_bytes()),), torch.uint8, w.device)
    call("dlcs_conv3d_pack_weights_f16x3", p(w.contiguous()), int(mode), p(packed), S())
    return packed


def conv3d_f16x3(planes, packed, grid, bias=None, out=None, mask=None, res=None, res_scale=1.0, accumulate=0,
                 relu_out=0, out_max=None, out_planes=None, colsum=None, planes_only=False, mask_planes=None):
    B, D, H, W = grid
    rows = B * D * H * W
    if out is None and not planes_only:
        out = empty((rows, 160), torch.float32, planes.device)
    ws, nb = _ws("dlcs_conv3d_k3_f16x3", planes.device, B, D, H, W, colsum is not None)
    call("dlcs_conv3d_k3_f16x3", p(planes), p(packed), p(bias), p(out), out.shape[-1] if out is not None else 160,
         B, D, H, W, p(mask), mask.shape[-1] if mask is not None else 0, p(res), res.shape[-1] if res is not None else 0,
         float(res_scale), int(accumulate), int(relu_out), out_max, p(out_planes), p(colsum), p(mask_planes), p(ws), nb, S())
    return out


def gemm_k160_f16x3(a_planes, M, b_planes, N, C, bias=None, act=0, alpha=1.0, res=None, res_scale=1.0,
                    res2=None, res2_scale=1.0, accumulate=0, out_max=None, out_planes=None, colsum=None,
                    res_planes=None, res2_planes=None):
    ws, nb = _ws("dlcs_gemm_k160_f16x3", a_planes.device, M, N, colsum is not None)
    call("dlcs_gemm_k160_f16x3", p(a_planes), M, p(b_planes), N, p(C), C.shape[-1] if C is not None else N,
         p(bias), int(act), float(alpha), p(res), res.shape[-1] if res is not None else 0, float(res_scale),
         p(res2), res2.shape[-1] if res2 is not None else 0, float(res2_scale), int(accumulate), out_max,
         p(out_planes), p(colsum), p(res_planes), p(res2_planes), p(ws), nb, S())
    return C


def _w(m):
    if m is None or isinstance(m, ctypes.c_void_p):
        return m
    return p(m)


def planes_bound(planes, rows, m0=None, n0=None, c0=1.0, m1=None, n1=None, c1=1.0, vec=None, cvec=1.0):
    call("dlcs_planes_bound", p(planes), rows, _w(m0), _w(n0), float(c0), _w(m1), _w(n1), float(c1), p(vec),
         vec.numel() if vec is not None else 0, float(cvec), S())
    return planes


def abs_row_sum_max(w, rows, row_stride, inner, n_outer=1, outer_stride=0, out=None):
    if out is None:
        out = empty((1,), torch.int32, w.device)
    call("dlcs_abs_row_sum_max", p(w), rows, row_stride, n_outer, outer_stride, inner, p(out), S())
    return out


def linear_k160_f16x3(x_planes, M, w_planes, N, out, bias=None, act=0, aux=None, aux_out=None, alpha=1.0,
                      res=None, row_map=None, accumulate=0):
    ldaux = (aux if aux is not None else aux_out).shape[-1] if (aux is not None or aux_out is not None) else 0
    call("dlcs_linear_k160_f16x3", p(x_planes), M, p(w_planes), N, p(out), out.shape[-1], p(bias), int(act),
         p(aux), p(aux_out), ldaux, float(alpha), p(res), res.shape[-1] if res is not None else 0, p(row_map),
         int(accumulate), S())
    return out


def conv3d_wgrad_f16x3(x_planes, g_planes, grid, dw_packed):
    B, D, H, W = grid
    ws, nb = _ws("dlcs_conv3d_k3_wgrad_f16x3", dw_packed.device, B, D, H, W)
    call("dlcs_conv3d_k3_wgrad_f16x3", p(x_planes), p(g_planes), p(dw_packed), B, D, H, W, p(ws), nb, S())
    return dw_packed


def absmax(x, out=None):
    if out is None:
        out = zeros((1,), torch.int32, x.device)
    call("dlcs_absmax_f32", p(x), x.numel(), p(out), S())
    return out


def _word(m):
    return m if isinstance(m, ctypes.c_void_p) else p(m)


def thin_pack_f16x3(packed, cout, cin, kind):
    out = empty((int(_lib.lib().dlcs_conv3d_thin_pack_f16x3_bytes(kind)),), torch.uint8, packed.device)
    call("dlcs_conv3d_thin_pack_f16x3", p(packed), cout, packed.shape[1], cin, packed.shape[2], int(kind), p(out), S())
    return out


def conv3d_thin_f16x3(x, cin, x_max, wthin, cout, out_ld, grid, bias=None, out=None, mask=None, res=None,
                      res_scale=1.0, accumulate=0, relu_out=0, out_max=None, out_planes=None, colsum=None,
                      planes_only=False, mask_planes=None):
    B, D, H, W = grid
    rows = B * D * H * W
    if out is None and not planes_only:
        out = empty((rows, out_ld), torch.float32, x.device)
    ws, nb = _ws("dlcs_conv3d_thin_f16x3", x.device, B, D, H, W, colsum is not None)
    call("dlcs_conv3d_thin_f16x3", p(x), cin, x.shape[-1], _word(x_max), p(wthin), p(bias), p(out), cout,
         out.shape[-1] if out is not None else 160, B, D, H, W, p(mask), mask.shape[-1] if mask is not None else 0,
         p(res), res.shape[-1] if res is not None else 0, float(res_scale), int(accumulate), int(relu_out),
         _word(out_max) if out_max is not None else None, p(out_planes), p(colsum), p(mask_planes), p(ws), nb, S())
    return out


def conv3d_thin_wgrad_f16x3(x, cin, x_max, g, cout, g_max, grid, dw_packed, colsum=None):
    B, D, H, W = grid
    call("dlcs_conv3d_thin_wgrad_f16x3", p(x), cin, x.shape[-1], _word(x_max), p(g), cout, g.shape[-1],
         _word(g_max), p(dw_packed), dw_packed.shape[1], dw_packed.shape[2], p(colsum), B, D, H, W, S())
    return dw_packed


def conv3d_thin_out_planes(planes, wthin, cout, out_ld, grid, bias=None, out=None, accumulate=0, relu_out=0):
    B, D, H, W = grid
    rows = B * D * H * W
    if out is None:
        out = empty((rows, out_ld), torch.float32, planes.device)
    call("dlcs_conv3d_thin_out_planes_f16x3", p(planes), p(wthin), p(bias), p(out), cout, out.shape[-1], B, D, H, W,
         int(accumulate), int(relu_out), S())
    return out


def conv3d_thin_wgrad_planes(big_planes, thin, thin_ch, thin_max, big_is_co, grid, dw_packed):
    B, D, H, W = grid
    ws, nb = _ws("dlcs_conv3d_thin_wgrad_planes_f16x3", dw_packed.device)
    call("dlcs_conv3d_thin_wgrad_planes_f16x3", p(big_planes), p(thin), thin_ch, thin.shape[-1], _word(thin_max),
         int(big_is_co), p(dw_packed), dw_packed.shape[1], dw_packed.shape[2], B, D, H, W, p(ws), nb, S())
    return dw_packed


def conv3d_wgrad(x, cin, relu_in, g, cout, grid, dw_packed, vox_per_block=16384, dbias=None):
    B, D, H, W = grid
    ws, nb = _ws("dlcs_conv3d_k3_wgrad", dw_packed.device, code(x), cin, dw_packed.shape[2], cout, dw_packed.shape[1],
             int(relu_in), dbias is not None, B, D, H, W)
    call("dlcs_conv3d_k3_wgrad", code(x), p(x), cin, x.shape[-1], dw_packed.shape[2], int(relu_in),
         p(g), cout, g.shape[-1], dw_packed.shape[1], p(dw_packed), p(dbias), B, D, H, W, vox_per_block, p(ws), nb, S())
    return dw_packed


def conv_unpack_grad(dw_packed, grad, cout, cin, accumulate=1):
    call("dlcs_conv3d_unpack_wgrad", p(dw_packed), p(grad), cout, cin, dw_packed.shape[1],
         dw_packed.shape[2], int(accumulate), S())
    return grad


def swin_pre(x, dtype, pad, ldc):
    B, E, T, Y, X = x.shape
    u = empty((B * (T + 2 * pad) * Y * X, ldc), dtype, x.device)
    call("dlcs_swin_pre", code(dtype), p(x), p(u), B, E, T, Y, X, pad, ldc, S())
    return u


def swin_pre_bwd(gu, shape, pad):
    B, E, T, Y, X = shape
    gx = empty(shape, torch.complex64, gu.device)
    call("dlcs_swin_pre_bwd", code(gu), p(gu), p(gx), B, E, T, Y, X, pad, gu.shape[-1], S())
    return gx


def swin_post(o, shape, pad):
    B, E, T, Y, X = shape
    out = empty(shape, torch.complex64, o.device)
    call("dlcs_swin_post", code(o), p(o), p(out), B, E, T, Y, X, pad, o.shape[-1], S())
    return out


def swin_post_bwd(gout, dtype, pad, ldc):
    B, E, T, Y, X = gout.shape
    go = empty((B * (T + 2 * pad) * Y * X, ldc), dtype, gout.device)
    call("dlcs_swin_post_bwd", code(dtype), p(gout), p(go), B, E, T, Y, X, pad, ldc, S())
    return go


def pad4(n):
    return (n + 3) // 4 * 4


def box_pre_bf16(x, pad, ldc, grid):
    B, E, T, Y, X = x.shape
    u = empty((grid[0] * grid[1] * grid[2] * grid[3], ldc), torch.bfloat16, x.device)
    call("dlcs_box_pre_bf16", p(x), p(u), B, E, T, Y, X, pad, grid[1], grid[2], grid[3], ldc, S())
    return u


def box_post_bwd_bf16(gout, pad, ldc, grid):
    B, E, T, Y, X = gout.shape
    go = empty((grid[0] * grid[1] * grid[2] * grid[3], ldc), torch.bfloat16, gout.device)
    call("dlcs_box_post_bwd_bf16", p(gout), p(go), B, E, T, Y, X, pad, grid[1], grid[2], grid[3], ldc, S())
    return go


def box_zero_bf16(x, C, grid, box):
    call("dlcs_box_zero_bf16", p(x), x.shape[-1], C, *grid, *box[1:], S())
    return x


def box_pre(x, pad, ldc, grid, dtype=torch.float32):
    if dtype == torch.bfloat16:
        return box_pre_bf16(x, pad, ldc, grid)
    B, E, T, Y, X = x.shape
    u = empty((grid[0] * grid[1] * grid[2] * grid[3], ldc), torch.float32, x.device)
    call("dlcs_box_pre", p(x), p(u), B, E, T, Y, X, pad, grid[1], grid[2], grid[3], ldc, S())
    return u


def box_pre_bwd(gu, shape, pad, grid):
    B, E, T, Y, X = shape
    gx = empty(shape, torch.complex64, gu.device)
    call("dlcs_box_pre_bwd", p(gu), p(gx), B, E, T, Y, X, pad, grid[1], grid[2], grid[3], gu.shape[-1], S())
    return gx


def box_post(o, shape, pad, grid):
    B, E, T, Y, X = shape
    out = empty(shape, torch.complex64, o.device)
    call("dlcs_box_post", p(o), p(out), B, E, T, Y, X, pad, grid[1], grid[2], grid[3], o.shape[-1], S())
    return out


def box_post_bwd(gout, pad, ldc, grid, dtype=torch.float32):
    if dtype == torch.bfloat16:
        return box_post_bwd_bf16(gout, pad, ldc, grid)
    B, E, T, Y, X = gout.shape
    go = empty((grid[0] * grid[1] * grid[2] * grid[3], ldc), torch.float32, gout.device)
    call("dlcs_box_post_bwd", p(gout), p(go), B, E, T, Y, X, pad, grid[1], grid[2], grid[3], ldc, S())
    return go


def box_zero(x, C, grid, box):
    if x.dtype == torch.bfloat16:
        return box_zero_bf16(x, C, grid, box)
    call("dlcs_box_zero", p(x), x.shape[-1], C, *grid, *box[1:], S())
    return x


def box_shift(src, C, grid, box, shift, transpose=False, out=None, res=None, relu=False):
    if out is None:
        out = empty(src.shape, torch.float32, src.device)
    call("dlcs_box_shift", p(src), src.shape[-1], p(out), out.shape[-1], C, *grid, *box[1:], *shift, int(transpose),
         p(res), res.shape[-1] if res is not None else 0, int(relu), S())
    return out


def relu_grad(g, a):
    assert g.numel() == a.numel()
    call("dlcs_relu_grad", code(g), p(g), code(a), p(a), g.numel(), S())
    return g


def bf16_rows_call(name, *args):
    call(name + "_bf16", *args)


def _rows_call(rows, name, *args):
    if rows.dtype == torch.bfloat16:
        bf16_rows_call(name, *args)
    else:
        call(name, *args)


def se_pool(o, B, N, C, mean=None):
    if mean is None:
        mean = empty((B, C), torch.float32, o.device)
    ws, nb = _ws("dlcs_se_pool", o.device, B, N, C)
    _rows_call(o, "dlcs_se_pool", p(o), B, N, C, o.shape[-1], p(mean), p(ws), nb, S())
    return mean


def se_gate(mean, w1, b1, w2, b2, hidden=None, gate=None):
    B, C = mean.shape
    R = w1.shape[0]
    if hidden is None:
        hidden = empty((B, R), torch.float32, mean.device)
    if gate is None:
        gate = empty((B, C), torch.float32, mean.device)
    call("dlcs_se_gate", p(mean), p(w1), p(b1), p(w2), p(b2), B, C, R, p(hidden), p(gate), S())
    return hidden, gate


def se_scale_res_relu(o, gate, res, B, N, C, out=None):
# ... 225 lines not shown
```

### dl-swin-gan_amd/dl_cs/models/engine.py

```python
import ctypes
import math
import weakref


import torch

from .. import diag as _diag
from . import _ops as K
from ._window import get_window_size as get_window_size_tuple


class BlockWeights:

    NAMES = ("norm1.weight", "norm1.bias", "attn.relative_position_bias_table", "attn.qkv.weight",
             "attn.qkv.bias", "attn.proj.weight", "attn.proj.bias", "norm2.weight", "norm2.bias",
             "mlp.fc1.weight", "mlp.fc1.bias", "mlp.fc2.weight", "mlp.fc2.bias")

    LINEARS = ("attn.qkv.weight", "attn.proj.weight", "mlp.fc1.weight", "mlp.fc2.weight")

    def __init__(self, params, dtype, cast=None, hr=None):
        self.p = params
        w = cast if cast is not None else [K.cast(params[n], dtype) for n in self.LINEARS]
        self.w = dict(zip(("qkv", "proj", "fc1", "fc2"), w))
        self.hr = None
# ... 4 lines not shown

    def lin(self, name, x, bias, act=0, aux_out=None, alpha=1.0, res=None, row_map=None, out=None):
        w = self.w[name]
        if self.hr is not None:
            return K.linear_h3r(x, self.hr[name], w.shape[0], out=out, bias=bias, act=act, aux_out=aux_out,
                                alpha=alpha, res=res, row_map=row_map)
        return K.linear(x, w, bias, out=out, act=act, aux_out=aux_out, alpha=alpha, res=res, row_map=row_map)

    def lin_dx(self, name, g, out_dtype, act=0, aux=None):
        w = self.w[name]
        if self.hr is not None:
            return K.linear_h3r(g, self.hr[name + "T"], w.shape[1], act=act, aux=aux)
        return K.linear_dx(g, w, out_dtype=out_dtype, act=act, aux=aux)


def h3r_ok(dtype, wqkv, wproj, wfc1, wfc2):
    if dtype != torch.float32 or not H3R:
        return False
    ks = (160, 480, 640)
    return all(w.dim() == 2 and w.shape[0] % 160 == 0 and w.shape[1] % 160 == 0 and w.shape[0] in ks and
               w.shape[1] in ks for w in (wqkv, wproj, wfc1, wfc2))


class SwinGeometry:

    def __init__(self, B, D, H, W, window, shift_enabled, device):
        self.B, self.D, self.H, self.W = B, D, H, W
        self.window0 = tuple(window)
        shift = tuple(i // 2 for i in window) if shift_enabled else (0, 0, 0)
        self.ws, self.ss = get_window_size_tuple((D, H, W), window, shift)
        self.shifted = any(s > 0 for s in self.ss)
        self.N = self.ws[0] * self.ws[1] * self.ws[2]
        self.part, self.rev, self.labels, self.nrows = K.window_tables(
            B, D, H, W, self.ws, self.ss if self.shifted else (0, 0, 0), device, self.shifted)
        self.nwin = self.nrows // self.N
        self.ntok = B * D * H * W


def block_forward(bw, geo, x, dtype, heads, drop_scale=(1.0, 1.0), mask=None, mask_nw=0):
    P = bw.p
    C = x.shape[1]
    hd = C // heads
    scale = hd ** -0.5
    s = {}
    ln1, m1, r1 = K.layernorm_fwd(x, P["norm1.weight"], P["norm1.bias"], geo.nrows, src_map=geo.part,
                                  out_dtype=dtype)
    qkv = bw.lin("qkv", ln1, P["attn.qkv.bias"])
    labels = geo.labels if (geo.shifted and mask is None) else None
    if ATTN_PROFILE is not None:
        e0, e1 = torch.cuda.Event(enable_timing=True), torch.cuda.Event(enable_timing=True)
        e0.record()
    att, lse = K.attn_fwd(qkv, P["attn.relative_position_bias_table"], labels, geo.nwin, geo.N, heads, hd,
                          geo.window0, scale, mask=mask if geo.shifted else None, mask_nw=mask_nw)
    if ATTN_PROFILE is not None:
        e1.record()
        ATTN_PROFILE.append((e0, e1, 4.0 * geo.nwin * geo.N * geo.N * hd * heads))
    x1 = torch.empty_like(x)
    if drop_scale[0] == 0.0:
        x1.copy_(x)
    else:
        bw.lin("proj", att, P["attn.proj.bias"], alpha=drop_scale[0], res=x, row_map=geo.part, out=x1)
    ln2, m2, r2 = K.layernorm_fwd(x1, P["norm2.weight"], P["norm2.bias"], geo.ntok, out_dtype=dtype)
    h1 = K.empty((geo.ntok, bw.w["fc1"].shape[0]), dtype, x.device)
    a1 = bw.lin("fc1", ln2, P["mlp.fc1.bias"], act=1, aux_out=h1)
    x2 = torch.empty_like(x)
    if drop_scale[1] == 0.0:
        x2.copy_(x1)
    else:
        bw.lin("fc2", a1, P["mlp.fc2.bias"], alpha=drop_scale[1], res=x1, out=x2)
    s.update(x=x, ln1=ln1, m1=m1, r1=r1, qkv=qkv, att=att, lse=lse, x1=x1, ln2=ln2, m2=m2, r2=r2,
             h1=h1, a1=a1, drop=drop_scale, mask=mask, mask_nw=mask_nw)
    return x2, s


def block_backward(bw, geo, s, g2, grads, dtype, heads):
    P = bw.p
    C = g2.shape[1]
    hd = C // heads
    scale = hd ** -0.5
    d0, d1 = s["drop"]
    dw_jobs = []

    def weight_grad(gout, act, wname, bname, T):
        if K.dw_grouped_ok(T, [(gout, act)]):
            dw_jobs.append((T, (gout, act, grads[wname], grads[bname], 0)))
        else:
            K.linear_dw(gout, act, grads[wname])
            K.colsum(gout, grads[bname])

    g1 = g2
    if d1 != 0.0:
        g2s = K.scaled_copy(g2, dtype, d1) if d1 != 1.0 else K.cast(g2, dtype)
        dh = bw.lin_dx("fc2", g2s, dtype, act=2, aux=s["h1"])
        weight_grad(g2s, s["a1"], "mlp.fc2.weight", "mlp.fc2.bias", geo.ntok)
        dln2 = bw.lin_dx("fc1", dh, torch.float32)
        weight_grad(dh, s["ln2"], "mlp.fc1.weight", "mlp.fc1.bias", geo.ntok)
        g1 = torch.empty_like(g2)
        K.layernorm_bwd(dln2, s["x1"], P["norm2.weight"], s["m2"], s["r2"], g1,
                        grads["norm2.weight"], grads["norm2.bias"], dx_in=g2)
    g0 = g1
    if d0 != 0.0:
        gw = K.gather_rows(g1, geo.part, geo.nrows, dtype)
        if d0 != 1.0:
            K.axpby(gw, gw, d0, 0.0)
        datt = bw.lin_dx("proj", gw, dtype)
        weight_grad(gw, s["att"], "attn.proj.weight", "attn.proj.bias", geo.nrows)
        labels = geo.labels if (geo.shifted and s["mask"] is None) else None
        if ATTN_BWD_PROFILE is not None:
            e0, e1 = torch.cuda.Event(enable_timing=True), torch.cuda.Event(enable_timing=True)
            e0.record()
        dqkv = K.attn_bwd(s["qkv"], s["att"], datt, s["lse"], P["attn.relative_position_bias_table"], labels,
                          grads["attn.relative_position_bias_table"], geo.nwin, geo.N, heads, hd, geo.window0,
                          scale, mask=s["mask"] if geo.shifted else None, mask_nw=s["mask_nw"])
        if ATTN_BWD_PROFILE is not None:
            e1.record()
            ATTN_BWD_PROFILE.append((e0, e1, 8.0 * geo.nwin * geo.N * geo.N * hd * heads))
        dqkv_t = K.cast(dqkv, dtype)
        dln1 = bw.lin_dx("qkv", dqkv_t, torch.float32)
        if K.dw_grouped_ok(geo.nrows, [(dqkv_t, s["ln1"])]):
            dw_jobs.append((geo.nrows, (dqkv_t, s["ln1"], grads["attn.qkv.weight"], grads["attn.qkv.bias"], 0)))
        else:
            K.linear_dw(dqkv_t, s["ln1"], grads["attn.qkv.weight"])
            K.colsum(dqkv, grads["attn.qkv.bias"])
        g0 = torch.empty_like(g1)
        K.layernorm_bwd(dln1, s["x"], P["norm1.weight"], s["m1"], s["r1"], g0,
                        grads["norm1.weight"], grads["norm1.bias"], src_map=geo.part, dx_in=g1)
    for T in sorted({t for t, _ in dw_jobs}):
        K.gemm_dw_grouped(T, [job for t, job in dw_jobs if t == T])
    return g0


PAD_CIN = 8

PROFILE = None
ATTN_PROFILE = None
ATTN_BWD_PROFILE = None
CAPTURE = None


def _timed(role, flops, fn, *args, **kw):
    if PROFILE is None:
        return fn(*args, **kw)
    e0 = torch.cuda.Event(enable_timing=True)
    e1 = torch.cuda.Event(enable_timing=True)
    e0.record()
    out = fn(*args, **kw)
    e1.record()
    PROFILE.setdefault(role, []).append((e0, e1, flops))
    return out


def _conv_flops(grid, cin, cout):
    return 2.0 * grid[0] * grid[1] * grid[2] * grid[3] * cout * cin * 27


def _timed_conv(*args, **kw):
    return _timed("conv_fwd", _conv_flops(args[5], args[1], args[3]), K.conv3d, *args, **kw)


FP32_CONV = _diag.knob("DLCS_FP32_CONV", "f32" if _diag.knob("DLCS_CONV_X6", "") == "0" else "f16x3")
if FP32_CONV not in ("f16x3", "f32"):
    raise ValueError(f"DLCS_FP32_CONV={FP32_CONV!r}: 'f16x3' (default) or 'f32'")
X6 = FP32_CONV != "f32"
H3R = _diag.knob("DLCS_H3R", "1") != "0"


_CONV_NORMS = []


def clear_norm_cache():
    del _CONV_NORMS[:]


def _conv_norm(w, C, dgrad=False):
    for t, ver, dg, nrm in _CONV_NORMS:
        if t() is w and ver == w._version and dg == dgrad:
            return nrm
    if dgrad == "patch":
        nrm = K.abs_row_sum_max(w, C * 64, 1, 1, n_outer=w.shape[0], outer_stride=C * 64)
    elif dgrad:
        nrm = K.abs_row_sum_max(w, C, 27, 27, n_outer=w.shape[0], outer_stride=27 * C)
    else:
        nrm = K.abs_row_sum_max(w, C, 27 * C, 27 * C)
    _CONV_NORMS.insert(0, (weakref.ref(w), w._version, dgrad, nrm))
    del _CONV_NORMS[12:]
    return nrm


def _use_split(dtype, C):
    return X6 and dtype == torch.float32 and C == 160


class StageWeights:

    def __init__(self, params, pre, dtype, depth, split):
        self.pre = pre
        P = lambda n: params[pre + n]
        tail = P("swin_tail.weight")
        self.tail = K.conv_pack_f16x3(tail, 0) if split else K.conv_pack(tail, dtype, 0)
        we = P("patch_embed.proj.weight")
        C = we.shape[0]
        self.emb = K.permute(we, (C, 4, 4, 4, C), (C * 64, 16, 4, 1, 64), dst_dtype=dtype)
        wu = P("patch_unembed.proj.weight")
        self.unemb = K.permute(wu, (4, 4, 4, C, C), (16, 4, 1, 64, C * 64), dst_dtype=dtype)
        self.unemb_bias = K.fill_bias(K.empty((64 * C,), torch.float32, we.device), P("patch_unembed.proj.bias"),
                                      1, 64 * C, C)
        self.unemb_dx = self.emb_h3r = None
        if split:
            self.unemb_dx, self.emb_h3r = K.h3r_pack([(self.unemb.reshape(64 * C, C), True),
                                                      (self.emb.reshape(C, 64 * C), False)])
            self.unemb_h3 = K.split2(self.unemb.reshape(64 * C, C))
            self.embT_h3 = K.split2(self.emb.reshape(C, 64 * C).t().contiguous())
            self.embT_norm = _conv_norm(we, C, dgrad="patch")
            self.unemb_norm = _conv_norm(wu, C, dgrad="patch")
            self.tail_norm = _conv_norm(tail, C)
        bp = [{n: P(f"blocks.{i}.{n}") for n in BlockWeights.NAMES} for i in range(depth)]
        casts = [None] * depth
        hrs = [None] * depth
        if depth and h3r_ok(dtype, *[bp[0][n] for n in BlockWeights.LINEARS]):
            flat = K.h3r_pack([(b[n], t) for b in bp for t in (False, True) for n in BlockWeights.LINEARS])
            hrs = [flat[8 * i:8 * i + 8] for i in range(depth)]
        if dtype == torch.bfloat16:
            flat = K.cast_multi_bf16([b[n] for b in bp for n in BlockWeights.LINEARS])
            casts = [flat[4 * i:4 * i + 4] for i in range(depth)]
        self.blocks = [BlockWeights(bp[i], dtype, casts[i], hrs[i]) for i in range(depth)]


class NetWeights:

    def __init__(self, params, dtype, depth, nstages=1):
        self.p = params
        self.dtype = dtype
        C = params["SFE.layers.2.conv.bias"].shape[0]
        self.split = _use_split(dtype, C)
        self.sfe = K.conv_pack(params["SFE.layers.2.conv.weight"], dtype, 0)
        self.fin = K.conv_pack(params["final_layer.layers.2.conv.weight"], dtype, 0)
        dfe = params["dfe_tail.weight"]
        self.dfe = K.conv_pack_f16x3(dfe, 0) if self.split else K.conv_pack(dfe, dtype, 0)
        self.dfe_norm = _conv_norm(dfe, C) if self.split else None
        if self.split:
            cin = params["SFE.layers.2.conv.weight"].shape[1]
            self.sfe_h3 = K.thin_pack_f16x3(self.sfe, C, cin, 0)
            self.fin_h3 = K.thin_pack_f16x3(self.fin, cin, C, 1)
        self.stages = [StageWeights(params, f"rs{k}.", dtype, depth, self.split) for k in range(nstages)]


def _stage_swin_forward(W, st, inp, geos, ntok, heads, drops):
    dtype, P = W.dtype, W.p
    C = st.emb.shape[0]
    if st.emb_h3r is not None:
        tok = K.linear_h3r(inp.view(ntok, 64 * C), st.emb_h3r, C, bias=P[st.pre + "patch_embed.proj.bias"])
    else:
        tok = K.fill_bias(K.empty((ntok, C), torch.float32, inp.device), P[st.pre + "patch_embed.proj.bias"],
                          ntok, C, C)
        if dtype == torch.float32:
            K.gemm_f32_splitk_det(inp, st.emb, tok, ntok, C, 64 * C, 64 * C, 64 * C)
        else:
            K.gemm(inp, st.emb, tok, ntok, C, 64 * C, 64 * C, 64 * C, C, accumulate=1, splitk=1)
    bsaved = []
    for i, bw in enumerate(st.blocks):
        ds = drops[i] if drops is not None else (1.0, 1.0)
        tok, sv = block_forward(bw, geos[i], tok, dtype, heads, drop_scale=ds)
        bsaved.append(sv)
    return K.cast(tok, dtype), bsaved


def swinnet_forward(W, x, heads=8, window=(7, 8, 8), pad=4, drop_scales=None):
    B, E, T, Y, X = x.shape
    if (T + 2 * pad) % 4 or Y % 4 or X % 4:
        raise NotImplementedError("dl_cs HIP path: T+2*pad, Y and X must be multiples of 4")
    out, saved = (_split_forward if W.split else _plain_forward)(W, x, heads, window, pad, drop_scales)
    if CAPTURE is not None:
        CAPTURE.append(dict(relu_inputs=[ss["a"] for ss in saved["stages"]] + [saved["b"], saved["h"]],
                            grid=saved["grid"], C=saved["C"]))
    return out, saved


def _geometries(grid, window, depth, dev):
    B, nT, nY, nX = grid[0], grid[1] // 4, grid[2] // 4, grid[3] // 4
    return B * nT * nY * nX, [SwinGeometry(B, nT, nY, nX, window, i % 2 == 1, dev) for i in range(depth)]


def _plain_forward(W, x, heads, window, pad, drop_scales):
    dtype, P = W.dtype, W.p
    B, E, T, Y, X = x.shape
    grid = (B, T + 2 * pad, Y, X)
    C = P["SFE.layers.2.conv.bias"].shape[0]
    cin = 2 * E
    dev = x.device
    rows = grid[0] * grid[1] * grid[2] * grid[3]
    u = K.swin_pre(x.contiguous(), dtype, pad, PAD_CIN)
    s = K.conv3d(u, cin, W.sfe, C, C, grid, bias=P["SFE.layers.2.conv.bias"])
    ntok, geos = _geometries(grid, window, len(W.stages[0].blocks), dev)
    nst = len(W.stages)
    stages = []
    inp = s
    for k, st in enumerate(W.stages):
        tok_t, bsaved = _stage_swin_forward(W, st, inp, geos, ntok, heads,
                                            drop_scales[k] if drop_scales is not None else None)
        a = K.empty((rows, C), dtype, dev)
        K.gemm(tok_t, st.unemb, a, ntok, 64 * C, C, C, C, 64 * C, bias=st.unemb_bias, act=3)
        out = _timed_conv(a, C, st.tail, C, C, grid, bias=P[st.pre + "swin_tail.bias"], res=inp,
                          relu_out=int(k == nst - 1))
        stages.append(dict(inp=inp, tok_t=tok_t, bsaved=bsaved, a=a, out=out))
        inp = out
    b = inp
    h = _timed_conv(b, C, W.dfe, C, C, grid, bias=P["dfe_tail.bias"], res=s, res_scale=2.0, relu_out=1)
    o = K.conv3d(h, C, W.fin, cin, PAD_CIN, grid, bias=P["final_layer.layers.2.conv.bias"],
                 out_dtype=torch.float32)
    out = K.swin_post(o, (B, E, T, Y, X), pad)
    saved = dict(u=u, s=s, b=b, pout=None, h=h, ph=None, stages=stages, geos=geos, shape=(B, E, T, Y, X), grid=grid,
                 pad=pad, heads=heads, cin=cin, C=C, ntok=ntok, umax=None, hmax=None)
    return out, saved


def _split_forward(W, x, heads, window, pad, drop_scales):
    dtype, P = W.dtype, W.p
    B, E, T, Y, X = x.shape
    grid = (B, T + 2 * pad, Y, X)
    C = P["SFE.layers.2.conv.bias"].shape[0]
    cin = 2 * E
    dev = x.device
    rows = grid[0] * grid[1] * grid[2] * grid[3]
    flops = _conv_flops(grid, C, C)
    keep_fp32 = CAPTURE is not None
    u = K.swin_pre(x.contiguous(), dtype, pad, PAD_CIN)
    mx = K.zeros((2 * len(W.stages) + 2,), torch.int32, dev)
    word = lambda i: ctypes.c_void_p(mx.data_ptr() + 4 * i)
    umax = K.absmax(u)
    s = K.conv3d_thin_f16x3(u, cin, umax, W.sfe_h3, C, C, grid, bias=P["SFE.layers.2.conv.bias"],
                            out_max=word(0))
    ntok, geos = _geometries(grid, window, len(W.stages[0].blocks), dev)
    nst = len(W.stages)
    stages = []
    inp, pout = s, None
    inp_max = word(0)
    for k, st in enumerate(W.stages):
        tok_t, bsaved = _stage_swin_forward(W, st, inp, geos, ntok, heads,
                                            drop_scales[k] if drop_scales is not None else None)
        a = K.empty((rows, C), dtype, dev) if keep_fp32 else None
        ss = dict(inp=inp, tok_t=tok_t, bsaved=bsaved, a=a)
        tb = P[st.pre + "swin_tail.bias"]
        pa = K.planes_alloc(rows, dev)
        amax, omax = word(1 + 2 * k), word(2 + 2 * k)
        tp = K.split2(tok_t)
        K.planes_bound(pa, rows, m0=K.planes_max(tp, ntok), n0=st.unemb_norm, vec=st.unemb_bias)
        K.gemm_k160_f16x3(tp, ntok, st.unemb_h3, 64 * C, a.view(ntok, 64 * C) if keep_fp32 else None,
                          bias=st.unemb_bias, act=3, out_max=amax, out_planes=pa)
        ss["planes"] = pa
        if k == nst - 1:
            pout = K.planes_alloc(rows, dev)
            K.planes_bound(pout, rows, m0=amax, n0=st.tail_norm, m1=inp_max, vec=tb)
            out = _timed("conv_fwd", flops, K.conv3d_f16x3, pa, st.tail, grid, bias=tb, res=inp,
                         relu_out=1, out_max=omax, out_planes=pout, planes_only=not keep_fp32)
        else:
            out = _timed("conv_fwd", flops, K.conv3d_f16x3, pa, st.tail, grid, bias=tb, res=inp, out_max=omax)
        inp_max = omax
        ss["out"] = out
        stages.append(ss)
        inp = out
    b = inp
    hmax = mx[-1:]
    ph = K.planes_alloc(rows, dev)
    K.planes_bound(ph, rows, m0=inp_max, n0=W.dfe_norm, m1=word(0), c1=2.0, vec=P["dfe_tail.bias"])
    h = _timed("conv_fwd", flops, K.conv3d_f16x3, pout, W.dfe, grid, bias=P["dfe_tail.bias"], res=s,
               res_scale=2.0, relu_out=1, out_max=K.p(hmax), out_planes=ph, planes_only=not keep_fp32)
    o = K.conv3d_thin_out_planes(ph, W.fin_h3, cin, PAD_CIN, grid, bias=P["final_layer.layers.2.conv.bias"])
    out = K.swin_post(o, (B, E, T, Y, X), pad)
    saved = dict(u=u, s=s, b=b, pout=pout, h=h, ph=ph, stages=stages, geos=geos, shape=(B, E, T, Y, X), grid=grid,
                 pad=pad, heads=heads, cin=cin, C=C, ntok=ntok, umax=umax, hmax=hmax)
    return out, saved


def swinnet_backward(W, sv, gout, grads):
    return (_split_backward if W.split else _plain_backward)(W, sv, gout, grads)


def _stage_swin_backward(W, st, ss, sv, g, grads):
    C, ntok = sv["C"], sv["ntok"]
    pre = st.pre
    g_a = g.pop()
    dev = g_a.device
    if st.unemb_dx is not None:
        d_tok = K.empty((ntok, C), torch.float32, dev)
        K.linear_h3r(g_a.view(ntok, 64 * C), st.unemb_dx, C, out=d_tok)
    else:
        d_tok = K.zeros((ntok, C), torch.float32, dev)
        K.gemm(g_a, st.unemb, d_tok, ntok, C, 64 * C, 64 * C, C, C, b_trans=1, accumulate=1, splitk=16)
    g_a_tok = g_a.view(ntok, 64 * C)
    if K.dw_grouped_ok(ntok, [(g_a_tok, ss["tok_t"])]):
        K.gemm_dw_grouped(ntok, [(g_a_tok, ss["tok_t"], grads[pre + "unemb_packed"],
                                  grads[pre + "patch_unembed.proj.bias"], C)])
    else:
        K.gemm(g_a, ss["tok_t"], grads[pre + "unemb_packed"], 64 * C, C, ntok, 64 * C, C, C, a_trans=1,
               b_trans=1, accumulate=1, splitk=max(1, min(16, ntok // 256)))
        K.colsum(g_a, grads[pre + "patch_unembed.proj.bias"], rows=64 * ntok, C=C, ld=C)
    del g_a, g_a_tok
    for i in reversed(range(len(st.blocks))):
        bg = {n: grads[f"{pre}blocks.{i}.{n}"] for n in BlockWeights.NAMES}
        d_tok = block_backward(st.blocks[i], sv["geos"][i], ss["bsaved"][i], d_tok, bg, W.dtype, sv["heads"])
    return d_tok, K.cast(d_tok, W.dtype)


def _embed_wgrad(st, ss, sv, d_tok, d_tok_t, grads):
    C, ntok = sv["C"], sv["ntok"]
    pre = st.pre
    in_tok = ss["inp"].view(ntok, 64 * C)
    if K.dw_grouped_ok(ntok, [(d_tok_t, in_tok)]):
        K.gemm_dw_grouped(ntok, [(d_tok_t, in_tok, grads[pre + "emb_packed"], grads[pre + "patch_embed.proj.bias"],
                                  0)])
    else:
        K.gemm(d_tok_t, ss["inp"], grads[pre + "emb_packed"], C, 64 * C, ntok, C, 64 * C, 64 * C, a_trans=1,
               b_trans=1, accumulate=1, splitk=max(1, min(16, ntok // 256)))
        K.colsum(d_tok, grads[pre + "patch_embed.proj.bias"])


def _plain_backward(W, sv, gout, grads):
    dtype, P = W.dtype, W.p
    grid, pad, C, cin, ntok = sv["grid"], sv["pad"], sv["C"], sv["cin"], sv["ntok"]
    dev = gout.device
    rows = grid[0] * grid[1] * grid[2] * grid[3]
    flops = _conv_flops(grid, C, C)
    go = K.swin_post_bwd(gout.contiguous(), dtype, pad, PAD_CIN)

    def conv_grads(x_in, cin_, g, cout, wname, bname):
        dwp = torch.zeros((27, K.pad32(cout), K.pad32(cin_)), dtype=torch.float32, device=dev)
        if cin_ == C and cout == C:
            _timed("conv_wgrad", flops, K.conv3d_wgrad, x_in, cin_, 0, g, cout, grid, dwp, dbias=grads[bname])
        else:
            K.conv3d_wgrad(x_in, cin_, 0, g, cout, grid, dwp, dbias=grads[bname])
        K.conv_unpack_grad(dwp, grads[wname], cout, cin_)

    wf = K.conv_pack(P["final_layer.layers.2.conv.weight"], dtype, 1)
    g_h = K.conv3d(go, cin, wf, C, C, grid, relu_in=0, mask=sv["h"])
    conv_grads(sv["h"], C, go, cin, "final_layer.layers.2.conv.weight", "final_layer.layers.2.conv.bias")
    w2 = K.conv_pack(P["dfe_tail.weight"], dtype, 1)
    g_out = _timed("conv_dgrad", flops, K.conv3d, g_h, C, w2, C, C, grid, mask=sv["b"])
    conv_grads(sv["b"], C, g_h, C, "dfe_tail.weight", "dfe_tail.bias")
    for k in reversed(range(len(W.stages))):
        st, ss = W.stages[k], sv["stages"][k]
        pre = st.pre
        w1 = K.conv_pack(P[pre + "swin_tail.weight"], dtype, 1)
        g = [_timed("conv_dgrad", flops, K.conv3d, g_out, C, w1, C, C, grid, mask=ss["a"])]
        conv_grads(ss["a"], C, g_out, C, pre + "swin_tail.weight", pre + "swin_tail.bias")
        d_tok, d_tok_t = _stage_swin_backward(W, st, ss, sv, g, grads)
        g_in = K.empty((rows, C), dtype, dev)
        if k == 0:
            K.gemm(d_tok_t, st.emb, g_in, ntok, 64 * C, C, C, 64 * C, 64 * C, b_trans=1,
                   res=g_h, ldr=64 * C, res_scale=2.0, res2=g_out, ldr2=64 * C)
        else:
            K.gemm(d_tok_t, st.emb, g_in, ntok, 64 * C, C, C, 64 * C, 64 * C, b_trans=1, res=g_out, ldr=64 * C)
        _embed_wgrad(st, ss, sv, d_tok, d_tok_t, grads)
        g_out = g_in
    wsfe = K.conv_pack(P["SFE.layers.2.conv.weight"], dtype, 1)
    g_u = K.conv3d(g_out, C, wsfe, cin, PAD_CIN, grid)
    conv_grads(sv["u"], cin, g_out, C, "SFE.layers.2.conv.weight", "SFE.layers.2.conv.bias")
    return K.swin_pre_bwd(g_u, sv["shape"], pad)


def _relu_mask(x, planes):
    return (x, None) if x is not None else (None, planes)


def _split_backward(W, sv, gout, grads):
    dtype, P = W.dtype, W.p
    grid, pad, C, cin, ntok = sv["grid"], sv["pad"], sv["C"], sv["cin"], sv["ntok"]
    dev = gout.device
    rows = grid[0] * grid[1] * grid[2] * grid[3]
    flops = _conv_flops(grid, C, C)
    go = K.swin_post_bwd(gout.contiguous(), dtype, pad, PAD_CIN)

    def split_wgrad(x_planes, g_planes, wname):
        dwp = torch.zeros((27, C, C), dtype=torch.float32, device=dev)
        _timed("conv_wgrad", flops, K.conv3d_wgrad_f16x3, x_planes, g_planes, grid, dwp)
        K.conv_unpack_grad(dwp, grads[wname], C, C)

    wf = K.conv_pack(P["final_layer.layers.2.conv.weight"], dtype, 1)
    pg = K.planes_alloc(rows, dev)
    gomax = K.absmax(go)
    ghmax = K.zeros((1,), torch.int32, dev)
    K.planes_bound(pg, rows, m0=gomax, n0=_conv_norm(P["final_layer.layers.2.conv.weight"], C, dgrad=True))
    mask, mask_planes = _relu_mask(sv["h"], sv["ph"])
    K.conv3d_thin_f16x3(go, cin, gomax, K.thin_pack_f16x3(wf, C, cin, 0), C, C, grid, mask=mask,
                        mask_planes=mask_planes, out_max=K.p(ghmax), out_planes=pg, planes_only=True,
                        colsum=grads["dfe_tail.bias"])
    dwp = torch.zeros((27, K.pad32(cin), C), dtype=torch.float32, device=dev)
    K.conv3d_thin_wgrad_planes(sv["ph"], go, cin, gomax, 0, grid, dwp)
    K.conv_unpack_grad(dwp, grads["final_layer.layers.2.conv.weight"], cin, C)
    K.colsum(go, grads["final_layer.layers.2.conv.bias"], rows=rows, C=cin, ld=go.shape[-1])
    gh_pl = pg
    pg = K.planes_alloc(rows, dev)
    gom = K.zeros((1,), torch.int32, dev)
    K.planes_bound(pg, rows, m0=ghmax, n0=_conv_norm(P["dfe_tail.weight"], C, dgrad=True))
    mask, mask_planes = _relu_mask(sv["b"], sv["pout"])
    _timed("conv_dgrad", flops, K.conv3d_f16x3, gh_pl, K.conv_pack_f16x3(P["dfe_tail.weight"], 1), grid,
           mask=mask, mask_planes=mask_planes, out_max=K.p(gom), out_planes=pg, planes_only=True,
           colsum=grads[W.stages[-1].pre + "swin_tail.bias"])
    split_wgrad(sv["pout"], gh_pl, "dfe_tail.weight")
    g_out = None
    for k in reversed(range(len(W.stages))):
        st, ss = W.stages[k], sv["stages"][k]
        pre = st.pre
        if g_out is None:
            gp = gout_pl = pg
            gomax = gom
        else:
            gout_pl = None
            gp = K.split2(g_out, out=pg, have_max=True, colsum=grads[pre + "swin_tail.bias"])
            gomax = gp[rows * 640:rows * 640 + 4].view(torch.int32).clone()
        mask, mask_planes = _relu_mask(ss["a"], ss["planes"])
        g = [_timed("conv_dgrad", flops, K.conv3d_f16x3, gp, K.conv_pack_f16x3(P[pre + "swin_tail.weight"], 1),
                    grid, mask=mask, mask_planes=mask_planes)]
        split_wgrad(ss["planes"], gp, pre + "swin_tail.weight")
        del gp
        d_tok, d_tok_t = _stage_swin_backward(W, st, ss, sv, g, grads)
        if k == 0:
            g_in = None
            dtp = K.split2(d_tok_t)
            pgs = K.planes_alloc(rows, dev)
            K.planes_bound(pgs, rows, m0=K.planes_max(dtp, ntok), n0=st.embT_norm, m1=ghmax, c1=2.0,
                           vec=gomax.view(torch.float32))
            K.gemm_k160_f16x3(dtp, ntok, st.embT_h3, 64 * C, None, res_planes=gh_pl, res_scale=2.0,
                              res2=g_out.view(ntok, 64 * C) if g_out is not None else None, res2_planes=gout_pl,
                              out_planes=pgs, colsum=grads["SFE.layers.2.conv.bias"])
        else:
            g_in = K.empty((rows, C), dtype, dev)
            pg = K.planes_alloc(rows, dev)
            K.gemm_k160_f16x3(K.split2(d_tok_t), ntok, st.embT_h3, 64 * C, g_in.view(ntok, 64 * C),
                              res=g_out.view(ntok, 64 * C) if g_out is not None else None, res_planes=gout_pl,
                              out_max=K.planes_max(pg, rows))
        _embed_wgrad(st, ss, sv, d_tok, d_tok_t, grads)
        g_out = g_in
    wsfe = K.conv_pack(P["SFE.layers.2.conv.weight"], dtype, 1)
    g_u = K.conv3d_thin_out_planes(pgs, K.thin_pack_f16x3(wsfe, cin, C, 1), cin, PAD_CIN, grid)
    dwp = torch.zeros((27, C, K.pad32(cin)), dtype=torch.float32, device=dev)
    K.conv3d_thin_wgrad_planes(pgs, sv["u"], cin, sv["umax"], 1, grid, dwp)
    K.conv_unpack_grad(dwp, grads["SFE.layers.2.conv.weight"], C, cin)
    return K.swin_pre_bwd(g_u, sv["shape"], pad)


def unpack_patch_grads(grads, C, nstages=1):
    for k in range(nstages):
        pre = f"rs{k}."
        K.permute(grads[pre + "emb_packed"], (C, C, 4, 4, 4), (64 * C, 1, 16 * C, 4 * C, C),
                  out=grads[pre + "patch_embed.proj.weight"], accumulate=1)
        K.permute(grads[pre + "unemb_packed"], (C, C, 4, 4, 4), (1, C, 16 * C * C, 4 * C * C, C * C),
                  out=grads[pre + "patch_unembed.proj.weight"], accumulate=1)
```

### include/dlcs.h

```cpp
#ifndef DLCS_H
#define DLCS_H

#include <stddef.h>
#include <stdint.h>

#ifdef __cplusplus
extern "C" {
#endif

#define DLCS_VERSION 1

enum dlcs_dtype { DLCS_F32 = 0, DLCS_BF16 = 1 };

enum dlcs_status {
    DLCS_OK = 0,
    DLCS_ERR_INVALID_ARG = 100001,
    DLCS_ERR_UNSUPPORTED_SIZE = 100002,
    DLCS_ERR_WORKSPACE = 100003
};

typedef void* dlcs_stream_t;

int dlcs_version(void);
const char* dlcs_status_string(int status);
// ... 22 lines not shown
size_t dlcs_sense_rowtab_bytes(int64_t B, int64_t weights_coils, int64_t T, int64_t Y);
int dlcs_sense_rowtab(const float* weights, int64_t weights_coils, int64_t B, int64_t T, int64_t Y, int64_t X,
                      void* table, size_t table_bytes, dlcs_stream_t stream);
size_t dlcs_sense_rows_workspace_bytes(int64_t B, int64_t C, int64_t T, int64_t jcap, int64_t X);
int dlcs_sense_normal_rows(const void* x, const void* maps, const float* weights, int64_t weights_coils,
                           const void* table, int64_t jcap, void* out, const void* sub, float base_scale, float step,
                           int64_t B, int64_t E, int64_t C, int64_t T, int64_t Y, int64_t X,
                           void* workspace, size_t workspace_bytes, dlcs_stream_t stream);
int dlcs_sense_adj_rows(const void* y, const void* maps, const float* weights, int64_t weights_coils,
                        const void* table, int64_t jcap, void* out, const void* base, const void* sub, float step,
                        int64_t B, int64_t E, int64_t C, int64_t T, int64_t Y, int64_t X,
                        void* workspace, size_t workspace_bytes, dlcs_stream_t stream);
int dlcs_sense_cg_rows(void* x, const void* b, const void* maps, const float* weights, int64_t weights_coils,
                       const void* table, int64_t jcap, float lamda, int num_iter,
                       int64_t B, int64_t E, int64_t C, int64_t T, int64_t Y, int64_t X,
                       void* workspace, size_t workspace_bytes, dlcs_stream_t stream);

int dlcs_fft2(const void* in, void* out, int64_t nplanes, int64_t Y, int64_t X, int inverse,
              void* workspace, size_t workspace_bytes, dlcs_stream_t stream);

int dlcs_fft_plan(int64_t n, int* kind, int* padded_len);


int dlcs_window_index(int64_t B, int64_t D, int64_t H, int64_t W, int64_t wd, int64_t wh, int64_t ww,
                      int64_t sd, int64_t sh, int64_t sw, int32_t* part_src, int32_t* rev_dst,
                      int32_t* labels, dlcs_stream_t stream);

int dlcs_gather_rows(int src_dtype, int dst_dtype, const void* src, const int32_t* idx, void* dst,
                     int64_t nrows, int64_t C, int64_t ld_src, int64_t ld_dst, dlcs_stream_t stream);

int dlcs_layernorm_fwd(int out_dtype, const float* x, const int32_t* src_map, const float* gamma,
                       const float* beta, float eps, void* out, float* mean, float* rstd,
                       int64_t rows, int64_t C, dlcs_stream_t stream);
size_t dlcs_layernorm_bwd_workspace_bytes(int64_t rows, int64_t C);
int dlcs_layernorm_bwd(const float* dy, const float* x, const int32_t* src_map, const float* gamma,
                       const float* mean, const float* rstd, const float* dx_in, float* dx, float* dgamma, float* dbeta,
                       int64_t rows, int64_t C, void* workspace, size_t workspace_bytes,
                       dlcs_stream_t stream);

int dlcs_colsum(int dtype, const void* x, int64_t rows, int64_t C, int64_t ld, float* out, dlcs_stream_t stream);

int dlcs_gemm(int dtype, int64_t M, int64_t N, int64_t K,
              const void* A, int64_t lda, int a_trans,
              const void* B, int64_t ldb, int b_trans,
              void* C, int64_t ldc, int c_dtype,
              const float* bias, int act, const void* aux, void* aux_out, int64_t ldaux, float alpha,
              const void* residual, int64_t ldr, int r_dtype, float res_scale,
              const void* residual2, int64_t ldr2, int r2_dtype, float res2_scale,
              const int32_t* row_map, int accumulate, int splitk, dlcs_stream_t stream);

size_t dlcs_gemm_dw_workspace_bytes(int ngroups, const int64_t* M, const int64_t* N, int64_t T);
int dlcs_gemm_dw_grouped(int ngroups, const void* const* A, const int64_t* lda, const void* const* B,
                         const int64_t* ldb, const int64_t* M, const int64_t* N, float* const* dW,
                         float* const* db, const int64_t* db_period, int64_t T, void* workspace,
                         size_t workspace_bytes, dlcs_stream_t stream);
int dlcs_gemm_dw_grouped_f32(int ngroups, const void* const* A, const int64_t* lda, const void* const* B,
                             const int64_t* ldb, const int64_t* M, const int64_t* N, float* const* dW,
                             float* const* db, const int64_t* db_period, int64_t T, void* workspace,
                             size_t workspace_bytes, dlcs_stream_t stream);

int dlcs_window_attn_fwd(int dtype, const void* qkv, void* out, float* lse, const float* table,
                         const int32_t* labels, const float* mask, int64_t mask_nw, int64_t nwin,
                         int64_t N, int64_t heads, int64_t head_dim,
                         int64_t wd0, int64_t wh0, int64_t ww0, float scale, dlcs_stream_t stream);
int dlcs_window_attn_bwd(int dtype, const void* qkv, const void* out, const void* dout, const float* lse,
                         const float* table, const int32_t* labels, const float* mask, int64_t mask_nw,
                         float* dqkv, float* dtable,
                         int64_t nwin, int64_t N, int64_t heads, int64_t head_dim,
                         int64_t wd0, int64_t wh0, int64_t ww0, float scale, dlcs_stream_t stream);

size_t dlcs_conv3d_k3_workspace_bytes(int dtype, int64_t cin, int64_t cin_pad, int64_t cout, int64_t cout_pad,
                                      int relu_in, int64_t B, int64_t D, int64_t H, int64_t W);
int dlcs_conv3d_k3(int dtype, const void* in, int64_t cin, int64_t cin_ld, const void* wpacked,
                   int64_t cin_pad, const float* bias, void* out, int out_dtype, int64_t cout,
                   int64_t cout_pad, int64_t cout_ld, int64_t B, int64_t D, int64_t H, int64_t W,
                   int relu_in, const void* mask, int64_t mask_ld, const void* residual, int res_dtype,
                   int64_t res_ld, float res_scale, int accumulate, int relu_out, void* workspace,
                   size_t workspace_bytes, dlcs_stream_t stream);
size_t dlcs_conv3d_k3_wgrad_workspace_bytes(int dtype, int64_t cin, int64_t cin_pad, int64_t cout, int64_t cout_pad,
                                            int relu_in, int has_dbias, int64_t B, int64_t D, int64_t H, int64_t W);
int dlcs_conv3d_k3_wgrad(int dtype, const void* in, int64_t cin, int64_t cin_ld, int64_t cin_pad, int relu_in,
                         const void* gout, int64_t cout, int64_t g_ld, int64_t cout_pad, float* dw_packed,
                         float* dbias, int64_t B, int64_t D, int64_t H, int64_t W, int64_t vox_per_block,
                         void* workspace, size_t workspace_bytes, dlcs_stream_t stream);
int dlcs_conv3d_pack_weights(int dtype, const float* w, void* packed, int64_t cout, int64_t cin,
                             int64_t rows_pad, int64_t cols_pad, int mode, dlcs_stream_t stream);
#ifdef DLCS_DIAG_BUILD
int dlcs_conv3d_k3_x6(const void* xa, const void* xb, const void* wpacked, const float* bias, float* out,
                      int64_t cout_ld, int64_t B, int64_t D, int64_t H, int64_t W, const float* mask, int64_t mask_ld,
                      const float* residual, int64_t res_ld, float res_scale, int accumulate, int relu_out,
                      dlcs_stream_t stream);
int dlcs_conv3d_k3_wgrad_x6(const void* xa, const void* xb, const void* ga, const void* gb, float* dw_packed,
                            int64_t B, int64_t D, int64_t H, int64_t W, dlcs_stream_t stream);
int dlcs_split3_bf16(const float* x, int64_t rows, int64_t ld, void* xa, void* xb, dlcs_stream_t stream);
int dlcs_debug_conv_stamps(void* host, int64_t n);
int dlcs_debug_h3_stamps(void* host, int64_t n);
#endif

size_t dlcs_split2_f16_bytes(int64_t rows);
size_t dlcs_split2_f16_workspace_bytes(int64_t rows, int has_colsum);
int dlcs_split2_f16(const float* x, int64_t rows, int64_t ld, void* planes, int have_max, float* colsum,
                    void* workspace, size_t workspace_bytes, dlcs_stream_t stream);
size_t dlcs_conv3d_pack_weights_f16x3_bytes(void);
int dlcs_conv3d_pack_weights_f16x3(const float* w, int mode, void* packed, dlcs_stream_t stream);
size_t dlcs_conv3d_k3_f16x3_workspace_bytes(int64_t B, int64_t D, int64_t H, int64_t W, int has_colsum);
int dlcs_conv3d_k3_f16x3(const void* xplanes, const void* wpacked, const float* bias, float* out, int64_t cout_ld,
                         int64_t B, int64_t D, int64_t H, int64_t W, const float* mask, int64_t mask_ld,
                         const float* residual, int64_t res_ld, float res_scale, int accumulate, int relu_out,
                         unsigned* out_max, void* out_planes, float* colsum, const void* mask_planes,
                         void* workspace, size_t workspace_bytes, dlcs_stream_t stream);
size_t dlcs_gemm_k160_f16x3_workspace_bytes(int64_t M, int64_t N, int has_colsum);
int dlcs_gemm_k160_f16x3(const void* aplanes, int64_t M, const void* bplanes, int64_t N, float* C, int64_t ldc,
                         const float* bias, int act, float alpha, const float* residual, int64_t ldr, float res_scale,
                         const float* residual2, int64_t ldr2, float res2_scale, int accumulate, unsigned* out_max,
                         void* out_planes, float* colsum, const void* res_planes, const void* res2_planes,
                         void* workspace, size_t workspace_bytes, dlcs_stream_t stream);
int dlcs_planes_bound(void* planes, int64_t rows, const unsigned* m0, const unsigned* n0, float c0,
                      const unsigned* m1, const unsigned* n1, float c1, const float* vec, int64_t nvec, float cvec,
                      dlcs_stream_t stream);
int dlcs_abs_row_sum_max(const float* w, int64_t rows, int64_t row_stride, int64_t n_outer, int64_t outer_stride,
                         int64_t inner, unsigned* out, dlcs_stream_t stream);

int dlcs_linear_k160_f16x3(const void* xplanes, int64_t M, const void* wplanes, int64_t N, float* C, int64_t ldc,
                           const float* bias, int act, const float* aux, float* aux_out, int64_t ldaux, float alpha,
                           const float* residual, int64_t ldr, const int32_t* row_map, int accumulate,
                           dlcs_stream_t stream);

size_t dlcs_h3r_pack_bytes(int64_t rows, int64_t K);
int dlcs_h3r_pack_multi(int n, const float* const* src, const int64_t* ld, const int* trans, const int64_t* rows,
                        const int64_t* K, void* const* dst, dlcs_stream_t stream);
size_t dlcs_gemm_h3r_workspace_bytes(int64_t M, int64_t K, int64_t N, int act, int has_row_map, int has_aux_out);
int dlcs_gemm_h3r(const float* A, int64_t M, int64_t K, int64_t lda, const void* bpacked, int64_t N, float* C,
                  int64_t ldc, const float* bias, int act, const float* aux, float* aux_out, int64_t ldaux, float alpha,
                  const float* residual, int64_t ldr, const int32_t* row_map, int accumulate, void* workspace,
                  size_t workspace_bytes, dlcs_stream_t stream);

int dlcs_f8r_quant(const float* x, int64_t rows, int64_t K, int64_t ld, void* q, float* inv, dlcs_stream_t stream);
int dlcs_gemm_f8r(const void* aq, const float* ainv, int64_t M, int64_t K, const void* bq, const float* binv,
                  int64_t N, float* C, int64_t ldc, const float* bias, int act, float* aux_out, int64_t ldaux,
                  float alpha, const float* residual, int64_t ldr, const int32_t* row_map, dlcs_stream_t stream);

size_t dlcs_gemm_f32_splitk_det_workspace_bytes(int64_t M, int64_t N);
int dlcs_gemm_f32_splitk_det(const float* A, int64_t lda, const float* B, int64_t ldb, int64_t M, int64_t N,
                             int64_t K, float* C, void* workspace, size_t workspace_bytes, dlcs_stream_t stream);
#ifdef DLCS_DIAG_BUILD
size_t dlcs_gemm_nt_x6_workspace_bytes(int64_t M, int64_t N, int64_t K);
int dlcs_gemm_nt_x6(const float* A, int64_t lda, const float* B, int64_t ldb, int64_t M, int64_t N, int64_t K,
                    float* C, void* workspace, size_t workspace_bytes, dlcs_stream_t stream);
#endif
size_t dlcs_conv3d_k3_wgrad_f16x3_workspace_bytes(int64_t B, int64_t D, int64_t H, int64_t W);
int dlcs_conv3d_k3_wgrad_f16x3(const void* xplanes, const void* gplanes, float* dw_packed, int64_t B, int64_t D,
                               int64_t H, int64_t W, void* workspace, size_t workspace_bytes,
                               dlcs_stream_t stream);
int dlcs_absmax_f32(const float* x, int64_t n, unsigned* out, dlcs_stream_t stream);
size_t dlcs_conv3d_thin_pack_f16x3_bytes(int kind);
int dlcs_conv3d_thin_pack_f16x3(const float* wpacked, int64_t cout, int64_t cout_pad, int64_t cin, int64_t cin_pad,
                                int kind, void* out, dlcs_stream_t stream);
size_t dlcs_conv3d_thin_f16x3_workspace_bytes(int64_t B, int64_t D, int64_t H, int64_t W, int has_colsum);
int dlcs_conv3d_thin_f16x3(const float* in, int64_t cin, int64_t cin_ld, const unsigned* in_max, const void* wthin,
                           const float* bias, float* out, int64_t cout, int64_t cout_ld, int64_t B, int64_t D,
                           int64_t H, int64_t W, const float* mask, int64_t mask_ld, const float* residual,
                           int64_t res_ld, float res_scale, int accumulate, int relu_out, unsigned* out_max,
                           void* out_planes, float* colsum, const void* mask_planes, void* workspace,
                           size_t workspace_bytes, dlcs_stream_t stream);
int dlcs_conv3d_thin_wgrad_f16x3(const float* in, int64_t cin, int64_t cin_ld, const unsigned* in_max,
                                 const float* g, int64_t cout, int64_t g_ld, const unsigned* g_max, float* dw_packed,
                                 int64_t cout_pad, int64_t cin_pad, float* colsum, int64_t B, int64_t D, int64_t H,
                                 int64_t W, dlcs_stream_t stream);
int dlcs_conv3d_thin_out_planes_f16x3(const void* xplanes, const void* wthin, const float* bias, float* out,
                                      int64_t cout, int64_t cout_ld, int64_t B, int64_t D, int64_t H, int64_t W,
                                      int accumulate, int relu_out, dlcs_stream_t stream);
size_t dlcs_conv3d_thin_wgrad_planes_f16x3_workspace_bytes(void);
int dlcs_conv3d_thin_wgrad_planes_f16x3(const void* bigplanes, const float* thin, int64_t thin_ch, int64_t thin_ld,
                                        const unsigned* thin_max, int big_is_co, float* dw_packed, int64_t cout_pad,
                                        int64_t cin_pad, int64_t B, int64_t D, int64_t H, int64_t W, void* workspace,
                                        size_t workspace_bytes, dlcs_stream_t stream);
int dlcs_conv3d_unpack_wgrad(const float* dw_packed, float* grad, int64_t cout, int64_t cin, int64_t cout_pad,
                             int64_t cin_pad, int accumulate, dlcs_stream_t stream);

int dlcs_swin_pre(int dtype, const void* x, void* u, int64_t B, int64_t E, int64_t T, int64_t Y, int64_t X,
                  int64_t pad, int64_t ldc, dlcs_stream_t stream);
int dlcs_swin_pre_bwd(int dtype, const void* gu, void* gx, int64_t B, int64_t E, int64_t T, int64_t Y, int64_t X,
                      int64_t pad, int64_t ldc, dlcs_stream_t stream);
int dlcs_swin_post(int dtype, const void* o, void* out, int64_t B, int64_t E, int64_t T, int64_t Y, int64_t X,
                   int64_t pad, int64_t ldc, dlcs_stream_t stream);
int dlcs_swin_post_bwd(int dtype, const void* gout, void* go, int64_t B, int64_t E, int64_t T, int64_t Y, int64_t X,
                       int64_t pad, int64_t ldc, dlcs_stream_t stream);

int dlcs_box_pre(const void* x, float* u, int64_t B, int64_t E, int64_t T, int64_t Y, int64_t X, int64_t pad,
                 int64_t Dp, int64_t Hp, int64_t Wp, int64_t ldc, dlcs_stream_t stream);
int dlcs_box_pre_bwd(const float* gu, void* gx, int64_t B, int64_t E, int64_t T, int64_t Y, int64_t X, int64_t pad,
                     int64_t Dp, int64_t Hp, int64_t Wp, int64_t ldc, dlcs_stream_t stream);
int dlcs_box_post(const float* o, void* out, int64_t B, int64_t E, int64_t T, int64_t Y, int64_t X, int64_t pad,
                  int64_t Dp, int64_t Hp, int64_t Wp, int64_t ldc, dlcs_stream_t stream);
int dlcs_box_post_bwd(const void* gout, float* go, int64_t B, int64_t E, int64_t T, int64_t Y, int64_t X, int64_t pad,
                      int64_t Dp, int64_t Hp, int64_t Wp, int64_t ldc, dlcs_stream_t stream);
int dlcs_box_zero(float* x, int64_t ld, int64_t C, int64_t B, int64_t Dp, int64_t Hp, int64_t Wp, int64_t D, int64_t H,
                  int64_t W, dlcs_stream_t stream);
int dlcs_box_shift(const float* src, int64_t ld_src, float* dst, int64_t ld_dst, int64_t C, int64_t B, int64_t Dp,
                   int64_t Hp, int64_t Wp, int64_t D, int64_t H, int64_t W, int64_t sd, int64_t sh, int64_t sw,
                   int transpose, const float* residual, int64_t ld_res, int relu, dlcs_stream_t stream);
int dlcs_box_pre_bf16(const void* x, void* u, int64_t B, int64_t E, int64_t T, int64_t Y, int64_t X, int64_t pad,
                      int64_t Dp, int64_t Hp, int64_t Wp, int64_t ldc, dlcs_stream_t stream);
int dlcs_box_post_bwd_bf16(const void* gout, void* go, int64_t B, int64_t E, int64_t T, int64_t Y, int64_t X,
                           int64_t pad, int64_t Dp, int64_t Hp, int64_t Wp, int64_t ldc, dlcs_stream_t stream);
int dlcs_box_zero_bf16(void* x, int64_t ld, int64_t C, int64_t B, int64_t Dp, int64_t Hp, int64_t Wp, int64_t D,
                       int64_t H, int64_t W, dlcs_stream_t stream);

int dlcs_relu_grad(int g_dtype, void* g, int a_dtype, const void* a, int64_t n, dlcs_stream_t stream);
int dlcs_axpby(int x_dtype, int y_dtype, const void* x, void* y, int64_t n, float a, float b, dlcs_stream_t stream);
int dlcs_permute(int src_dtype, int dst_dtype, const void* src, void* dst, int64_t ndim,
                 const int64_t* dst_shape, const int64_t* src_strides, int accumulate, dlcs_stream_t stream);
int dlcs_fill_bias(float* out, const float* bias, int64_t rows, int64_t C, int64_t period, dlcs_stream_t stream);
int dlcs_block_layout(int src_dtype, int dst_dtype, const void* src, void* dst, int64_t B, int64_t C, int64_t D,
                      int64_t H, int64_t W, int64_t ld, int inverse, dlcs_stream_t stream);

#define DLCS_CAST_MULTI_MAX 64
int dlcs_cast_multi_bf16(int64_t count, const float* const* src, void* const* dst, const int64_t* n,
                         dlcs_stream_t stream);

int dlcs_kt_window_average(const void* k, void* out, int64_t P, int64_t T, int64_t YX, int64_t window,
                           int full, dlcs_stream_t stream);
int dlcs_kth_largest_abs(const void* x, int64_t n, int64_t k, float* out, dlcs_stream_t stream);
int dlcs_cplx_mask_scale(const void* x, const float* mask, void* y, int64_t P, int64_t TYX, int64_t mask_planes,
                         const float* scale, int divide, dlcs_stream_t stream);
int dlcs_crop_flip(const void* in, void* out, int64_t P, int64_t T, int64_t Y, int64_t X, int64_t y0, int64_t ny,
                   int64_t x0, int64_t nx, int flip_t, int flip_y, int flip_x, dlcs_stream_t stream);

int dlcs_mhsa_fwd(int dtype, const void* qkv, void* out, float* lse, int64_t nseq, int64_t N, int64_t heads,
                  int64_t head_dim, float scale, dlcs_stream_t stream);
size_t dlcs_mhsa_bwd_workspace_bytes(int64_t nseq, int64_t N, int64_t heads);
int dlcs_mhsa_bwd(int dtype, const void* qkv, const void* out, const void* dout, const float* lse, float* dqkv,
                  int64_t nseq, int64_t N, int64_t heads, int64_t head_dim, float scale, void* workspace,
                  size_t workspace_bytes, dlcs_stream_t stream);

int dlcs_conv3d_thin_im2col(const float* src, int64_t ld_src, int64_t C, float* dst, int64_t ld_dst, int sign,
                            int64_t B, int64_t D, int64_t H, int64_t W, dlcs_stream_t stream);
int dlcs_conv3d_thin_col2im(const float* P, int64_t ld_p, int64_t C, float* out, int64_t ld_out, const float* bias,
                            int sign, int accumulate, int64_t B, int64_t D, int64_t H, int64_t W,
                            dlcs_stream_t stream);

int dlcs_dit_vec(int op, const float* a, const float* b, float* y, int64_t n, dlcs_stream_t stream);
int dlcs_timestep_embedding(const float* t, int64_t B, int64_t dim, float max_period, float* out,
                            dlcs_stream_t stream);
int dlcs_scale_rows(const float* W, const float* b, const float* gate, float* Wo, float* bo, int64_t N, int64_t K,
                    dlcs_stream_t stream);
int dlcs_gated_linear_grad(const float* W, const float* b, const float* G, const float* colsum, const float* gate,
                           float* dW, float* db, float* dgate, int64_t N, int64_t K, dlcs_stream_t stream);
int dlcs_rows_add(float* dst, const int32_t* idx, const float* src, int64_t nrows, int64_t C, dlcs_stream_t stream);

size_t dlcs_se_pool_workspace_bytes(int64_t B, int64_t N, int64_t C);
int dlcs_se_pool(const float* o, int64_t B, int64_t N, int64_t C, int64_t ld, float* mean, void* workspace,
                 size_t workspace_bytes, dlcs_stream_t stream);
int dlcs_se_gate(const float* mean, const float* W1, const float* b1, const float* W2, const float* b2, int64_t B,
                 int64_t C, int64_t R, float* hidden, float* gate, dlcs_stream_t stream);
int dlcs_se_scale_res_relu(const float* o, const float* gate, const float* res, float* out, int64_t B, int64_t N,
                           int64_t C, int64_t ld, dlcs_stream_t stream);
size_t dlcs_se_bwd_reduce_workspace_bytes(int64_t B, int64_t N, int64_t C);
int dlcs_se_bwd_reduce(const float* g, const float* r_next, const float* o, int64_t B, int64_t N, int64_t C, int64_t ld,
                       float* dgate, void* workspace, size_t workspace_bytes, dlcs_stream_t stream);
size_t dlcs_se_gate_bwd_workspace_bytes(int64_t B, int64_t C, int64_t R);
int dlcs_se_gate_bwd(const float* dgate, const float* gate, const float* hidden, const float* mean, const float* W1,
                     const float* W2, int64_t B, int64_t C, int64_t R, float inv_n, float* dW1, float* db1, float* dW2,
                     float* db2, float* dmean, void* workspace, size_t workspace_bytes, dlcs_stream_t stream);
int dlcs_se_bwd_apply(float* g, const float* r_next, const float* gate, const float* dmean, float* dout, int64_t B,
                      int64_t N, int64_t C, int64_t ld, dlcs_stream_t stream);

int dlcs_se_pool_bf16(const void* o, int64_t B, int64_t N, int64_t C, int64_t ld, float* mean, void* workspace,
                      size_t workspace_bytes, dlcs_stream_t stream);
int dlcs_se_scale_res_relu_bf16(const void* o, const float* gate, const void* res, void* out, int64_t B, int64_t N,
                                int64_t C, int64_t ld, dlcs_stream_t stream);
int dlcs_se_bwd_reduce_bf16(const void* g, const void* r_next, const void* o, int64_t B, int64_t N, int64_t C,
                            int64_t ld, float* dgate, void* workspace, size_t workspace_bytes, dlcs_stream_t stream);
int dlcs_se_bwd_apply_bf16(void* g, const void* r_next, const float* gate, const float* dmean, void* dout, int64_t B,
                           int64_t N, int64_t C, int64_t ld, dlcs_stream_t stream);

int dlcs_cbam_chan_mean(const float* o, const float* gate, int64_t B, int64_t D, int64_t H, int64_t W, int64_t C,
                        int64_t ld, float* map, dlcs_stream_t stream);
int dlcs_cbam_stencil5(const float* in, const float* w5, const float* bias, int transposed, float* out, int64_t B,
                       int64_t D, int64_t H, int64_t W, dlcs_stream_t stream);
size_t dlcs_cbam_stencil5_wgrad_workspace_bytes(int64_t B, int64_t D, int64_t H, int64_t W);
int dlcs_cbam_stencil5_wgrad(const float* dq, const float* a, int64_t B, int64_t D, int64_t H, int64_t W, float* dw5,
                             float* db5, void* workspace, size_t workspace_bytes, dlcs_stream_t stream);
int dlcs_cbam_scale_res_relu(const float* o, const float* gate, const float* q, const float* res, float* out, int64_t B,
                             int64_t D, int64_t H, int64_t W, int64_t C, int64_t ld, dlcs_stream_t stream);
int dlcs_cbam_bwd_rowdot(const float* g, const float* r_next, const float* o, const float* gate, int64_t B, int64_t D,
                         int64_t H, int64_t W, int64_t C, int64_t ld, float* dq, dlcs_stream_t stream);
size_t dlcs_cbam_bwd_reduce_workspace_bytes(int64_t B, int64_t D, int64_t H, int64_t W, int64_t C);
int dlcs_cbam_bwd_reduce(const float* g, const float* r_next, const float* o, const float* q, const float* da, int64_t B,
                         int64_t D, int64_t H, int64_t W, int64_t C, int64_t ld, float* dgate, void* workspace,
                         size_t workspace_bytes, dlcs_stream_t stream);
int dlcs_cbam_bwd_apply(float* g, const float* r_next, const float* gate, const float* q, const float* da,
                        const float* dmean, float* dout, int64_t B, int64_t D, int64_t H, int64_t W, int64_t C, int64_t ld,
                        dlcs_stream_t stream);

int dlcs_cbam_chan_mean_bf16(const void* o, const float* gate, int64_t B, int64_t D, int64_t H, int64_t W, int64_t C,
                             int64_t ld, float* map, dlcs_stream_t stream);
int dlcs_cbam_scale_res_relu_bf16(const void* o, const float* gate, const float* q, const void* res, void* out,
                                  int64_t B, int64_t D, int64_t H, int64_t W, int64_t C, int64_t ld,
                                  dlcs_stream_t stream);
int dlcs_cbam_bwd_rowdot_bf16(const void* g, const void* r_next, const void* o, const float* gate, int64_t B, int64_t D,
                              int64_t H, int64_t W, int64_t C, int64_t ld, float* dq, dlcs_stream_t stream);
int dlcs_cbam_bwd_reduce_bf16(const void* g, const void* r_next, const void* o, const float* q, const float* da,
                              int64_t B, int64_t D, int64_t H, int64_t W, int64_t C, int64_t ld, float* dgate,
                              void* workspace, size_t workspace_bytes, dlcs_stream_t stream);
int dlcs_cbam_bwd_apply_bf16(void* g, const void* r_next, const float* gate, const float* q, const float* da,
                             const float* dmean, void* dout, int64_t B, int64_t D, int64_t H, int64_t W, int64_t C,
                             int64_t ld, dlcs_stream_t stream);

int dlcs_lr_extract(const void* image, const float* weights, const float* win, int divide, void* blocks, int64_t E,
                    int64_t T, int64_t Y, int64_t X, int64_t b, dlcs_stream_t stream);
int dlcs_lr_combine(const void* blocks, const float* weights, const float* win, int divide, void* image, int64_t E,
                    int64_t T, int64_t Y, int64_t X, int64_t b, dlcs_stream_t stream);
int dlcs_lr_compose(const void* L, const void* R, const float* weights, const float* win, int divide, void* image,
                    int64_t E, int64_t T, int64_t Y, int64_t X, int64_t b, int64_t r, dlcs_stream_t stream);
int dlcs_lr_project_l(const void* image, const void* R, const float* weights, const float* win, int divide, void* out,
                      int64_t E, int64_t T, int64_t Y, int64_t X, int64_t b, int64_t r, dlcs_stream_t stream);
int dlcs_lr_project_r(const void* image, const void* L, const float* weights, const float* win, int divide, void* out,
                      int64_t E, int64_t T, int64_t Y, int64_t X, int64_t b, int64_t r, dlcs_stream_t stream);

int dlcs_lr_decompose(const void* image, const float* win, void* L, void* R, float* S, int32_t* info, int64_t E,
                      int64_t T, int64_t Y, int64_t X, int64_t b, int64_t r, dlcs_stream_t stream);

int dlcs_conv2d_k3(const void* in, int64_t cin, int64_t cin_ld, const void* wpacked, int64_t cin_pad,
                   const float* bias, void* out, int out_dtype, int64_t cout, int64_t cout_pad, int64_t cout_ld,
                   int64_t N, int64_t H, int64_t W, int KH, const void* mask, int64_t mask_ld,
                   const void* residual, int res_dtype, int64_t res_ld, float res_scale, int relu_out,
                   dlcs_stream_t stream);
int dlcs_conv2d_pack_weights(const float* w, void* packed, int64_t cout, int64_t cin, int64_t rows_pad,
// ... 14 lines not shown
```

Measured before the change: 4.587.

## Restrict thin conv output and wgrad kernels to live temporal frames

Adds windowed variants of the final thin output conv and the k3/thin weight-gradient kernels that only process the temporal slabs whose outputs survive the temporal padding crop. The engine computes the live frame range from the pad and the conv depth remaining, and passes it to these kernels. Padded frames that are later discarded by swin_post no longer cost conv or wgrad work. This adds a templated kernel path with new patch iteration and range splitting. Correctness rests on the padded-region gradients being exactly zero or irrelevant, which the live range margins are meant to guarantee.

```diff
diff --git a/dl-swin-gan_amd/csrc/conv3d_f16x3.hip b/dl-swin-gan_amd/csrc/conv3d_f16x3.hip
--- a/dl-swin-gan_amd/csrc/conv3d_f16x3.hip
+++ b/dl-swin-gan_amd/csrc/conv3d_f16x3.hip
@@ -1,5 +1,6 @@
 #include "conv3d_common.h"
 #include "f16x3_common.h"
+#include "wgrad_live.h"
 #include <type_traits>
 
 namespace {
@@ -229,6 +230,13 @@
 int dlcs_conv3d_k3_wgrad_f16x3(const void* xplanes, const void* gplanes, float* dw_packed, int64_t B, int64_t D,
                                int64_t H, int64_t W, void* workspace, size_t workspace_bytes,
                                dlcs_stream_t stream) {
+    return dlcs_conv3d_k3_wgrad_f16x3_live(xplanes, gplanes, dw_packed, B, D, H, W, 0, D, workspace, workspace_bytes,
+                                           stream);
+}
+
+int dlcs_conv3d_k3_wgrad_f16x3_live(const void* xplanes, const void* gplanes, float* dw_packed, int64_t B, int64_t D,
+                                    int64_t H, int64_t W, int64_t t_lo, int64_t t_hi, void* workspace,
+                                    size_t workspace_bytes, dlcs_stream_t stream) {
     DLCS_CHECK_ARG(xplanes && gplanes && dw_packed && B > 0);
     const long rows = (long)B * D * H * W;
     if (D % 4 || H % 4 || W % 4 || !al16(xplanes) || !al16(gplanes) || rows * 320 >= (1L << 40))
@@ -240,7 +248,9 @@
     if (!ws_ok(workspace, workspace_bytes, dlcs_conv3d_k3_wgrad_f16x3_workspace_bytes(B, D, H, W)))
         return DLCS_ERR_WORKSPACE;
     v.part = static_cast<float*>(workspace);
-    return wgrad_f16x3_launch(v, (hipStream_t)stream);
+    const int lo = (int)std::max<int64_t>(0, std::min<int64_t>(t_lo, D));
+    const int hi = (int)std::max<int64_t>(0, std::min<int64_t>(t_hi, D));
+    return wgrad_f16x3_launch(v, lo, hi, (hipStream_t)stream);
 }
 
 size_t dlcs_conv3d_thin_pack_f16x3_bytes(int kind) {
@@ -338,6 +348,14 @@
 int dlcs_conv3d_thin_out_planes_f16x3(const void* xplanes, const void* wthin, const float* bias, float* out,
                                       int64_t cout, int64_t cout_ld, int64_t B, int64_t D, int64_t H, int64_t W,
                                       int accumulate, int relu_out, dlcs_stream_t stream) {
+    return dlcs_conv3d_thin_out_planes_f16x3_slabs(xplanes, wthin, bias, out, cout, cout_ld, B, D, H, W, accumulate,
+                                                   relu_out, 0, D / 4, stream);
+}
+
+int dlcs_conv3d_thin_out_planes_f16x3_slabs(const void* xplanes, const void* wthin, const float* bias, float* out,
+                                            int64_t cout, int64_t cout_ld, int64_t B, int64_t D, int64_t H, int64_t W,
+                                            int accumulate, int relu_out, int64_t tb0, int64_t tb1,
+                                            dlcs_stream_t stream) {
     DLCS_CHECK_ARG(xplanes && wthin && out && B > 0 && cout >= 1 && cout <= 4 && cout_ld >= 4);
     if (D % 4 || H % 4 || W % 4 || cout_ld % 4 || !al16(xplanes) || !al16(wthin) || !al16(out))
         return DLCS_ERR_UNSUPPORTED_SIZE;
@@ -346,7 +364,9 @@
     v.B = (int)B; v.D = (int)D; v.H = (int)H; v.W = (int)W;
     v.cout_ld = (int)cout_ld; v.accumulate = accumulate; v.relu_out = relu_out; v.cout = (int)cout;
     v.cout_pad = (int)cout;
-    return conv_thin_out_p_launch(v, (const f16*)xplanes, (const f16*)wthin, (hipStream_t)stream);
+    const int64_t nT = D / 4;
+    const int s0 = (int)std::max<int64_t>(0, std::min(tb0, nT)), s1 = (int)std::max<int64_t>(0, std::min(tb1, nT));
+    return conv_thin_out_p_launch(v, (const f16*)xplanes, (const f16*)wthin, s0, s1, (hipStream_t)stream);
 }
 
 size_t dlcs_conv3d_thin_wgrad_planes_f16x3_workspace_bytes(void) { return (size_t)kTwpWG * 160 * 128 * sizeof(float); }
@@ -355,6 +375,17 @@
                                         const unsigned* thin_max, int big_is_co, float* dw_packed, int64_t cout_pad,
                                         int64_t cin_pad, int64_t B, int64_t D, int64_t H, int64_t W, void* workspace,
                                         size_t workspace_bytes, dlcs_stream_t stream) {
+    return dlcs_conv3d_thin_wgrad_planes_f16x3_live(bigplanes, thin, thin_ch, thin_ld, thin_max, big_is_co, dw_packed,
+                                                    cout_pad, cin_pad, B, D, H, W, 0, D, workspace, workspace_bytes,
+                                                    stream);
+}
+
+int dlcs_conv3d_thin_wgrad_planes_f16x3_live(const void* bigplanes, const float* thin, int64_t thin_ch,
+                                             int64_t thin_ld, const unsigned* thin_max, int big_is_co,
+                                             float* dw_packed, int64_t cout_pad, int64_t cin_pad, int64_t B, int64_t D,
+                                             int64_t H, int64_t W, int64_t t_lo, int64_t t_hi, void* workspace,
+                                             size_t workspace_bytes, dlcs_stream_t stream) {
+    DLCS_CHECK_ARG(!big_is_co || (t_lo <= 0 && t_hi >= D));
     DLCS_CHECK_ARG(bigplanes && thin && thin_max && dw_packed && B > 0 && thin_ch >= 1 && thin_ch <= 4 &&
                    thin_ld >= 4);
     if (D % 4 || H % 4 || W % 4 || thin_ld % 4 || !al16(bigplanes) || !al16(thin) ||
@@ -369,7 +400,8 @@
     if (!ws_ok(workspace, workspace_bytes, dlcs_conv3d_thin_wgrad_planes_f16x3_workspace_bytes()))
         return DLCS_ERR_WORKSPACE;
     t.part = static_cast<float*>(workspace);
-    return wgrad_thin_p_launch(t, (hipStream_t)stream);
-}
-
-}
+    const int lo = (int)std::max<int64_t>(0, std::min(t_lo, D)), hi = (int)std::max<int64_t>(0, std::min(t_hi, D));
+    return wgrad_thin_p_launch(t, lo, hi, (hipStream_t)stream);
+}
+
+}
diff --git a/dl-swin-gan_amd/csrc/conv3d_f16x3.inc b/dl-swin-gan_amd/csrc/conv3d_f16x3.inc
--- a/dl-swin-gan_amd/csrc/conv3d_f16x3.inc
+++ b/dl-swin-gan_amd/csrc/conv3d_f16x3.inc
@@ -461,7 +461,10 @@
     int B, D, H, W;
 };
 
-__global__ void __launch_bounds__(768) conv3d_wgrad_f16x3_kernel(WgradH3Args a, int nrange, int ppr) {
+struct WgradH3Live { int hs_lo, hs_hi, upr, urem; };
+
+template <bool WIN>
+__global__ void __launch_bounds__(768) conv3d_wgrad_f16x3_kernel(WgradH3Args a, int nrange, int ppr, WgradH3Live lv) {
     __shared__ __attribute__((aligned(16))) f16 smem_wh[3 * kWhBuf];
     const int b = blockIdx.x;
     int range, grp;
@@ -480,7 +483,10 @@
     const int nYX = nY * nX;
     const int npatch = a.B * nT * nYX;
     const int p0 = range * ppr, p1 = min(npatch, p0 + ppr);
-    if (p0 >= p1) return;
+    if (!WIN && p0 >= p1) return;
+    const WgLiveGeom lg{nT, nY, nX, lv.hs_lo, lv.hs_hi};
+    int lu0, lu1;
+    wgl_range(lv.upr, lv.urem, range, &lu0, &lu1);
     const int lane = threadIdx.x & 63, wave = __builtin_amdgcn_readfirstlane(threadIdx.x >> 6);
     const int kwi = wave >> 2, coh = (wave >> 1) & 1, cih = wave & 1;
     const int bias_rows = (nYX + nX + 1) * 64;
@@ -513,8 +519,11 @@
         pk[k] = wi < 50 ? (off16 << 7) | req : 0u;
     }
     const unsigned dst0 = __builtin_amdgcn_readfirstlane(lds_offset(smem_wh));
-    int ip = p0, ipt, ipy, ipx;
-    {
+    WgLiveIter it{};
+    int &ip = it.ip, &ipt = it.ipt, &ipy = it.ipy, &ipx = it.ipx;
+    if (WIN) it = wgl_seek(lg, lu0);
+    else {
+        ip = p0;
         const int r = ip % (nT * nYX);
         ipt = r / nYX;
         ipy = (r / nX) % nY;
@@ -574,7 +583,20 @@
     const int grow = (8 * gq + q) * 160;
     const int xrow = (32 + ((gq >> 1) * 4 + 2 * swb) * 6 + q + kwi) * 160;
 
-    {
+    if (WIN) {
+#pragma unroll
+        for (int s = 0; s < 2; ++s) {
+            if (lu0 + s < lu1) {
+                const char *gb, *xb;
+                unsigned xz;
+                bases(gb, xb, xz);
+                const unsigned miss = missing();
+#pragma unroll
+                for (int k = 0; k < 5; ++k) issue_piece(k, it.th, s, miss, gb, xb, xz);
+                wgl_advance(lg, it);
+            }
+        }
+    } else {
         const char *gb, *xb;
         unsigned xz;
         bases(gb, xb, xz);
@@ -584,7 +606,7 @@
 #pragma unroll
         for (int k = 0; k < 5; ++k) issue_piece(k, 1, 1, miss, gb, xb, xz);
     }
-    next_patch();
+    if (!WIN) next_patch();
     asm volatile("s_waitcnt vmcnt(0)" ::: "memory");
     __syncthreads();
     int cur = 0;
@@ -630,10 +652,17 @@
         __syncthreads();
         cur = cur == 2 ? 0 : cur + 1;
     };
-    for (int u = 2 * p0; u < 2 * p1; ++u) {
-        const int th = u & 1;
-        unit(th, (u >> 1) + 1 < p1);
-        if (th) next_patch();
+    if (WIN) {
+        for (int u = lu0; u < lu1; ++u) {
+            unit(it.th, u + 2 < lu1);
+            wgl_advance(lg, it);
+        }
+    } else {
+        for (int u = 2 * p0; u < 2 * p1; ++u) {
+            const int th = u & 1;
+            unit(th, (u >> 1) + 1 < p1);
+            if (th) next_patch();
+        }
     }
     const int tap = (kd + 1) * 9 + (kh + 1) * 3 + kwi;
     float* pp = a.part + ((long)range * 27 + tap) * 160 * 160;
@@ -671,15 +700,26 @@
     return patch_ranges(npatch, bound ? kWgH3MaxRanges : env_nr > 0 ? std::min(env_nr, kWgH3MaxRanges) : 28);
 }
 
-static int wgrad_f16x3_launch(const WgradH3Args& a, hipStream_t st) {
+static int wgrad_f16x3_launch(const WgradH3Args& a, int t_lo, int t_hi, hipStream_t st) {
     const long npatch = (long)a.B * (a.D / 4) * (a.H / 4) * (a.W / 4);
+    int hs_lo, hs_hi;
+    wgl_halfslabs(a.D, t_lo, t_hi, &hs_lo, &hs_hi);
+    if (hs_lo >= hs_hi) return DLCS_OK;
     const long bias_rows = ((long)(a.H / 4) * (a.W / 4) + a.W / 4 + 1) * 64;
     if ((2 * bias_rows + 128) * 40 >= (1L << 25) || (npatch * 64 + bias_rows) * 640 + 1024 >= (1L << 32))
         return DLCS_ERR_UNSUPPORTED_SIZE;
     const PatchRanges r = wgh3_ranges(npatch, false);
-    const int nr = r.nr;
+    int nr = r.nr;
     const long pp = r.pp;
-    hipLaunchKernelGGL(conv3d_wgrad_f16x3_kernel, dim3((unsigned)(9 * nr)), dim3(768), 0, st, a, nr, (int)pp);
+    if (hs_lo == 0 && hs_hi == a.D / 2)
+        hipLaunchKernelGGL(conv3d_wgrad_f16x3_kernel<false>, dim3((unsigned)(9 * nr)), dim3(768), 0, st, a, nr, (int)pp,
+                           WgradH3Live{});
+    else {
+        const long nlive = (long)a.B * (hs_hi - hs_lo) * (a.H / 4) * (a.W / 4);
+        nr = (int)std::min<long>(nr, nlive);
+        hipLaunchKernelGGL(conv3d_wgrad_f16x3_kernel<true>, dim3((unsigned)(9 * nr)), dim3(768), 0, st, a, nr, (int)pp,
+                           WgradH3Live{hs_lo, hs_hi, (int)(nlive / nr), (int)(nlive % nr)});
+    }
     hipLaunchKernelGGL(wgrad_f16x3_reduce_kernel, dim3((unsigned)cdiv(27L * 160 * 40, 256)), dim3(256), 0, st, a, nr);
     return dlcs_launch_status();
 }
diff --git a/dl-swin-gan_amd/csrc/conv3d_thin_planes.inc b/dl-swin-gan_amd/csrc/conv3d_thin_planes.inc
--- a/dl-swin-gan_amd/csrc/conv3d_thin_planes.inc
+++ b/dl-swin-gan_amd/csrc/conv3d_thin_planes.inc
@@ -166,7 +166,7 @@
 }
 
 __global__ void __launch_bounds__(512, 1) conv3d_thin_out_p3_kernel(ConvF32Args a, const f16* xp, const f16* wimg,
-                                                                    long rows) {
+                                                                    long rows, int tb0, int tb1) {
     __shared__ __attribute__((aligned(16))) f16 smem_tp3[3 * kTpBuf];
     const float sx = f16x3_scale(*reinterpret_cast<const unsigned*>(reinterpret_cast<const char*>(xp) + rows * 640));
     const float inv = 1.0f / (sx * *reinterpret_cast<const float*>(wimg + kThinOutHalfs));
@@ -193,15 +193,16 @@
     const int npc = wave < kTpPieces - 40 ? 6 : 5;
     const unsigned dst0 = __builtin_amdgcn_readfirstlane(lds_offset(smem_tp3));
     const int nBY = (nYt + 3) >> 2, nBX = (nX + 7) >> 3;
-    const int nblocks = a.B * nT * nBY * nBX, xcd = blockIdx.x & 7, kw = blockIdx.x >> 3;
+    const int nTw = tb1 - tb0;
+    const int nblocks = a.B * nTw * nBY * nBX, xcd = blockIdx.x & 7, kw = blockIdx.x >> 3;
     const int nrounds = xcd < nblocks ? (nblocks - xcd + 7) >> 3 : 0;
     const int nitems = nrounds * 5;
     auto decode = [&](int r, int& b, int& pt, int& py2, int& px) {
         int bid = r * 8 + xcd;
         const int bx = bid % nBX; bid /= nBX;
         const int by = bid % nBY; bid /= nBY;
-        pt = bid % nT;
-        b = bid / nT;
+        pt = tb0 + bid % nTw;
+        b = bid / nTw;
         py2 = by * 4 + (kw >> 3);
         px = bx * 8 + (kw & 7);
         return py2 < nYt && px < nX;
@@ -324,21 +325,27 @@
     }
 }
 
-static int conv_thin_out_p_launch(const ConvF32Args& v, const f16* xp, const f16* wimg, hipStream_t st) {
+static int conv_thin_out_p_launch(const ConvF32Args& v, const f16* xp, const f16* wimg, int tb0, int tb1,
+                                  hipStream_t st) {
     const int nT = v.D / 4, nY = v.H / 4, nX = v.W / 4;
+    tb0 = std::max(tb0, 0);
+    tb1 = std::min(tb1, nT);
+    if (tb0 >= tb1) return DLCS_OK;
     const long rows = (long)v.B * v.D * v.H * v.W;
     const long bias_rows = ((long)nY * nX + nX + 1) * 64;
     if ((2 * bias_rows + 4L * nX * 64 + 256) * 40 >= (1L << 24) || (rows + bias_rows) * 640 + 1024 >= (1L << 32))
         return DLCS_ERR_UNSUPPORTED_SIZE;
 #ifdef DLCS_DIAG_BUILD
     static const bool p2 = [] { const char* e = dlcs_knob("DLCS_THIN_OUT_P2"); return e && e[0] == '1'; }();
-    if (p2) hipLaunchKernelGGL(conv3d_thin_out_p_kernel, dim3(256), dim3(512), 0, st, v, xp, wimg, rows);
+    if (p2 && tb0 == 0 && tb1 == nT)
+        hipLaunchKernelGGL(conv3d_thin_out_p_kernel, dim3(256), dim3(512), 0, st, v, xp, wimg, rows);
     else
 #endif
-    hipLaunchKernelGGL(conv3d_thin_out_p3_kernel, dim3(256), dim3(512), 0, st, v, xp, wimg, rows);
+    hipLaunchKernelGGL(conv3d_thin_out_p3_kernel, dim3(256), dim3(512), 0, st, v, xp, wimg, rows, tb0, tb1);
     return dlcs_launch_status();
 }
 
+struct ThinWgPLive { int per, item, first, base, rem; };
 struct ThinWgPArgs {
     const f16* bp; const float* thin; float* dw; float* part;
     const unsigned* thin_max;
@@ -352,12 +359,14 @@
 constexpr int kTwBuf = kTwBigB + kTwTR;
 constexpr int kTwIm = 32 * 128;
 
-__global__ void __launch_bounds__(512, 1) conv3d_wgrad_thin_p_kernel(ThinWgPArgs a, int ppr) {
+__global__ void __launch_bounds__(512, 1) conv3d_wgrad_thin_p_kernel(ThinWgPArgs a, int ppr, ThinWgPLive lv) {
     __shared__ __attribute__((aligned(16))) f16 smem_twp[2 * kTwBuf + 4 * kTwIm];
     f16* IM = smem_twp + 2 * kTwBuf;
     const int nT = a.D >> 2, nY = a.H >> 2, nX = a.W >> 2;
     const int npatch = a.B * nT * nY * nX;
-    const int p0 = (int)blockIdx.x * ppr, p1 = min(npatch, p0 + ppr);
+    int p0 = (int)blockIdx.x * ppr, p1 = min(npatch, p0 + ppr);
+    if (lv.per) wgl_range(lv.base, lv.rem, (int)blockIdx.x, &p0, &p1);
+    auto patch_of = [&](int u) { return lv.per ? wgl_live_patch(u, lv.per, lv.item, lv.first) : u; };
     const int tid = threadIdx.x, lane = tid & 63, wave = __builtin_amdgcn_readfirstlane(tid >> 6);
     const float st = f16x3_scale(*a.thin_max);
     for (int i = tid; i < 4 * 32 * 20; i += 512) {
@@ -381,8 +390,9 @@
         pt = r % nT;
         bb = r / nT;
     };
-    auto issue = [&](int patch, int buf) {
-        if (patch >= p1) return;
+    auto issue = [&](int u, int buf) {
+        if (u >= p1) return;
+        const int patch = patch_of(u);
         const char* sb = reinterpret_cast<const char*>(a.bp) + (long)patch * 64 * 640;
         const unsigned dst = lds0 + (unsigned)(buf * kTwBuf * 2);
 #pragma unroll
@@ -403,8 +413,9 @@
     };
     const int jtap = tid >> 3, tc = tid & 7;
     const int skd = a.sgn * (jtap / 9 - 1), skh = a.sgn * ((jtap / 3) % 3 - 1), skw = a.sgn * (jtap % 3 - 1);
-    auto build = [&](int patch, int buf) {
+    auto build = [&](int u, int buf) {
         if (tid >= 216) return;
+        const int patch = patch_of(u);
         int bb, pt, py, px;
         coords(patch, bb, pt, py, px);
         const float* TR = reinterpret_cast<const float*>(smem_twp + buf * kTwBuf + kTwBigB);
@@ -515,11 +526,20 @@
 
 constexpr int kTwpWG = 256;
 
-static int wgrad_thin_p_launch(const ThinWgPArgs& a, hipStream_t st) {
-    const long npatch = (long)a.B * (a.D / 4) * (a.H / 4) * (a.W / 4);
+static int wgrad_thin_p_launch(const ThinWgPArgs& a, int t_lo, int t_hi, hipStream_t st) {
+    const int nT = a.D / 4, nYX = (a.H / 4) * (a.W / 4);
+    const long npatch = (long)a.B * nT * nYX;
     if (npatch * 64 * 640 >= (1L << 32)) return DLCS_ERR_UNSUPPORTED_SIZE;
+    int s0, s1;
+    wgl_slabs(a.D, t_lo, t_hi, 1, &s0, &s1);
+    if (s0 >= s1) return DLCS_OK;
     const int ppr = (int)((npatch + kTwpWG - 1) / kTwpWG);
-    hipLaunchKernelGGL(conv3d_wgrad_thin_p_kernel, dim3(kTwpWG), dim3(512), 0, st, a, ppr);
+    ThinWgPLive lv{};
+    if (s0 > 0 || s1 < nT) {
+        const int per = (s1 - s0) * nYX, n = a.B * per;
+        lv = ThinWgPLive{per, nT * nYX, s0 * nYX, n / kTwpWG, n % kTwpWG};
+    }
+    hipLaunchKernelGGL(conv3d_wgrad_thin_p_kernel, dim3(kTwpWG), dim3(512), 0, st, a, ppr, lv);
     hipLaunchKernelGGL(wgrad_thin_p_reduce_kernel, dim3(160 * 128 / 64), dim3(256), 0, st, a, kTwpWG);
     return dlcs_launch_status();
 }
diff --git a/dl-swin-gan_amd/csrc/wgrad_live.h b/dl-swin-gan_amd/csrc/wgrad_live.h
--- /dev/null
+++ b/dl-swin-gan_amd/csrc/wgrad_live.h
@@ -0,0 +1,82 @@
+#pragma once
+
+#if defined(__HIPCC__)
+#define WGL_HD __host__ __device__ __forceinline__
+#else
+#define WGL_HD inline
+#endif
+
+struct WgLiveGeom { int nT, nY, nX, hs_lo, hs_hi; };
+struct WgLiveIter { int ip, ipt, ipy, ipx, th; };
+
+WGL_HD void wgl_halfslabs(int D, int t_lo, int t_hi, int* hs_lo, int* hs_hi) {
+    if (t_lo < 0) t_lo = 0;
+    if (t_hi > D) t_hi = D;
+    *hs_lo = t_lo >> 1;
+    *hs_hi = t_lo < t_hi ? (t_hi + 1) >> 1 : *hs_lo;
+}
+
+WGL_HD void wgl_slabs(int D, int t_lo, int t_hi, int halo, int* s0, int* s1) {
+    if (t_lo < 0) t_lo = 0;
+    if (t_hi > D) t_hi = D;
+    const int lo = t_lo - halo;
+    *s0 = (lo > 0 ? lo : 0) >> 2;
+    const int hi = (t_hi + halo + 3) >> 2;
+    *s1 = t_lo < t_hi ? (hi < (D >> 2) ? hi : (D >> 2)) : *s0;
+}
+
+WGL_HD int wgl_live_patch(int u, int per, int item, int first) {
+    const int bi = u / per;
+    return bi * item + first + (u - bi * per);
+}
+
+WGL_HD int wgl_units_per_item(const WgLiveGeom& g) { return (g.hs_hi - g.hs_lo) * g.nY * g.nX; }
+
+WGL_HD void wgl_range(int base, int rem, int r, int* u0, int* u1) {
+    *u0 = r * base + (r < rem ? r : rem);
+    *u1 = *u0 + base + (r < rem ? 1 : 0);
+}
+
+WGL_HD WgLiveIter wgl_seek(const WgLiveGeom& g, int u) {
+    const int nYX = g.nY * g.nX, per = (g.hs_hi - g.hs_lo) * nYX;
+    const int bi = u / per;
+    int r = u - bi * per;
+    const int t0 = g.hs_lo >> 1;
+    const int nfirst = ((2 * t0 + 2 < g.hs_hi ? 2 * t0 + 2 : g.hs_hi) - g.hs_lo) * nYX;
+    int t, pin, th;
+    if (r < nfirst) {
+        t = t0;
+        if (nfirst == 2 * nYX) { pin = r >> 1; th = r & 1; }
+        else { pin = r; th = g.hs_lo & 1; }
+    } else {
+        r -= nfirst;
+        t = t0 + 1 + r / (2 * nYX);
+        r -= (t - t0 - 1) * 2 * nYX;
+        if (2 * t + 1 < g.hs_hi) { pin = r >> 1; th = r & 1; }
+        else { pin = r; th = 0; }
+    }
+    WgLiveIter it;
+    it.ip = (bi * g.nT + t) * nYX + pin;
+    it.ipt = t;
+    it.ipy = pin / g.nX;
+    it.ipx = pin - it.ipy * g.nX;
+    it.th = th;
+    return it;
+}
+
+WGL_HD void wgl_advance(const WgLiveGeom& g, WgLiveIter& it) {
+    if (it.th == 0 && 2 * it.ipt + 1 < g.hs_hi) { it.th = 1; return; }
+    ++it.ip;
+    if (++it.ipx == g.nX) {
+        it.ipx = 0;
+        if (++it.ipy == g.nY) {
+            it.ipy = 0;
+            if (2 * ++it.ipt >= g.hs_hi) {
+                const int t0 = g.hs_lo >> 1;
+                it.ip += (g.nT - it.ipt + t0) * g.nY * g.nX;
+                it.ipt = t0;
+            }
+        }
+    }
+    it.th = 2 * it.ipt >= g.hs_lo ? 0 : 1;
+}
diff --git a/dl-swin-gan_amd/dl_cs/_lib.py b/dl-swin-gan_amd/dl_cs/_lib.py
--- a/dl-swin-gan_amd/dl_cs/_lib.py
+++ b/dl-swin-gan_amd/dl_cs/_lib.py
@@ -79,6 +79,7 @@
     "dlcs_gemm_f32_splitk_det_workspace_bytes": [_I64, _I64],
     "dlcs_conv3d_k3_wgrad_f16x3_workspace_bytes": [_I64] * 4,
     "dlcs_conv3d_k3_wgrad_f16x3": [_P, _P, _P, _I64, _I64, _I64, _I64, _P, _SZ, _P],
+    "dlcs_conv3d_k3_wgrad_f16x3_live": [_P, _P, _P, _I64, _I64, _I64, _I64, _I64, _I64, _P, _SZ, _P],
     "dlcs_conv3d_k3_f16x3_workspace_bytes": [_I64, _I64, _I64, _I64, _INT],
     "dlcs_conv3d_k3_f16x3": [_P, _P, _P, _P, _I64, _I64, _I64, _I64, _I64, _P, _I64, _P, _I64, _F, _INT, _INT, _P, _P, _P,
                              _P, _P, _SZ, _P],
@@ -89,9 +90,13 @@
     "dlcs_conv3d_thin_f16x3": [_P, _I64, _I64, _P, _P, _P, _P, _I64, _I64, _I64, _I64, _I64, _I64, _P, _I64, _P,
                                _I64, _F, _INT, _INT, _P, _P, _P, _P, _P, _SZ, _P],
     "dlcs_conv3d_thin_out_planes_f16x3": [_P, _P, _P, _P, _I64, _I64, _I64, _I64, _I64, _I64, _INT, _INT, _P],
+    "dlcs_conv3d_thin_out_planes_f16x3_slabs": [_P, _P, _P, _P, _I64, _I64, _I64, _I64, _I64, _I64, _INT, _INT, _I64,
+                                                _I64, _P],
     "dlcs_conv3d_thin_wgrad_planes_f16x3_workspace_bytes": [],
     "dlcs_conv3d_thin_wgrad_planes_f16x3": [_P, _P, _I64, _I64, _P, _INT, _P, _I64, _I64, _I64, _I64, _I64, _I64,
                                             _P, _SZ, _P],
+    "dlcs_conv3d_thin_wgrad_planes_f16x3_live": [_P, _P, _I64, _I64, _P, _INT, _P, _I64, _I64, _I64, _I64, _I64, _I64,
+                                                 _I64, _I64, _P, _SZ, _P],
     "dlcs_conv3d_thin_wgrad_f16x3": [_P, _I64, _I64, _P, _P, _I64, _I64, _P, _P, _I64, _I64, _P, _I64, _I64, _I64,
                                      _I64, _P],
     "dlcs_swin_pre": [_INT, _P, _P, _I64, _I64, _I64, _I64, _I64, _I64, _I64, _P],
diff --git a/dl-swin-gan_amd/dl_cs/models/_ops.py b/dl-swin-gan_amd/dl_cs/models/_ops.py
--- a/dl-swin-gan_amd/dl_cs/models/_ops.py
+++ b/dl-swin-gan_amd/dl_cs/models/_ops.py
@@ -438,10 +438,14 @@
     return out
 
 
-def conv3d_wgrad_f16x3(x_planes, g_planes, grid, dw_packed):
+def conv3d_wgrad_f16x3(x_planes, g_planes, grid, dw_packed, live=None):
     B, D, H, W = grid
     ws, nb = _ws("dlcs_conv3d_k3_wgrad_f16x3", dw_packed.device, B, D, H, W)
-    call("dlcs_conv3d_k3_wgrad_f16x3", p(x_planes), p(g_planes), p(dw_packed), B, D, H, W, p(ws), nb, S())
+    if live is None:
+        call("dlcs_conv3d_k3_wgrad_f16x3", p(x_planes), p(g_planes), p(dw_packed), B, D, H, W, p(ws), nb, S())
+    else:
+        call("dlcs_conv3d_k3_wgrad_f16x3_live", p(x_planes), p(g_planes), p(dw_packed), B, D, H, W, int(live[0]),
+             int(live[1]), p(ws), nb, S())
     return dw_packed
 
 
@@ -484,21 +488,31 @@
     return dw_packed
 
 
-def conv3d_thin_out_planes(planes, wthin, cout, out_ld, grid, bias=None, out=None, accumulate=0, relu_out=0):
+def conv3d_thin_out_planes(planes, wthin, cout, out_ld, grid, bias=None, out=None, accumulate=0, relu_out=0,
+                           slabs=None):
     B, D, H, W = grid
     rows = B * D * H * W
     if out is None:
         out = empty((rows, out_ld), torch.float32, planes.device)
-    call("dlcs_conv3d_thin_out_planes_f16x3", p(planes), p(wthin), p(bias), p(out), cout, out.shape[-1], B, D, H, W,
-         int(accumulate), int(relu_out), S())
-    return out
-
-
-def conv3d_thin_wgrad_planes(big_planes, thin, thin_ch, thin_max, big_is_co, grid, dw_packed):
+    if slabs is None:
+        call("dlcs_conv3d_thin_out_planes_f16x3", p(planes), p(wthin), p(bias), p(out), cout, out.shape[-1], B, D, H,
+             W, int(accumulate), int(relu_out), S())
+    else:
+        call("dlcs_conv3d_thin_out_planes_f16x3_slabs", p(planes), p(wthin), p(bias), p(out), cout, out.shape[-1], B,
+             D, H, W, int(accumulate), int(relu_out), int(slabs[0]), int(slabs[1]), S())
+    return out
+
+
+def conv3d_thin_wgrad_planes(big_planes, thin, thin_ch, thin_max, big_is_co, grid, dw_packed, live=None):
     B, D, H, W = grid
     ws, nb = _ws("dlcs_conv3d_thin_wgrad_planes_f16x3", dw_packed.device)
-    call("dlcs_conv3d_thin_wgrad_planes_f16x3", p(big_planes), p(thin), thin_ch, thin.shape[-1], _word(thin_max),
-         int(big_is_co), p(dw_packed), dw_packed.shape[1], dw_packed.shape[2], B, D, H, W, p(ws), nb, S())
+    if live is None:
+        call("dlcs_conv3d_thin_wgrad_planes_f16x3", p(big_planes), p(thin), thin_ch, thin.shape[-1], _word(thin_max),
+             int(big_is_co), p(dw_packed), dw_packed.shape[1], dw_packed.shape[2], B, D, H, W, p(ws), nb, S())
+    else:
+        call("dlcs_conv3d_thin_wgrad_planes_f16x3_live", p(big_planes), p(thin), thin_ch, thin.shape[-1],
+             _word(thin_max), int(big_is_co), p(dw_packed), dw_packed.shape[1], dw_packed.shape[2], B, D, H, W,
+             int(live[0]), int(live[1]), p(ws), nb, S())
     return dw_packed
 
 
diff --git a/dl-swin-gan_amd/dl_cs/models/engine.py b/dl-swin-gan_amd/dl_cs/models/engine.py
--- a/dl-swin-gan_amd/dl_cs/models/engine.py
+++ b/dl-swin-gan_amd/dl_cs/models/engine.py
@@ -180,6 +180,20 @@
 
 def _conv_flops(grid, cin, cout):
     return 2.0 * grid[0] * grid[1] * grid[2] * grid[3] * cout * cin * 27
+
+
+def _live_frames(grid, pad, nconv):
+    D = grid[1]
+    return max(pad - nconv, 0), min(D - pad + nconv, D)
+
+
+def _live_slabs(grid, pad):
+    return pad // 4, (grid[1] - pad + 3) // 4
+
+
+def _wgrad_live_flops(grid, cin, cout, live):
+    frames = 2 * ((live[1] + 1) // 2 - live[0] // 2)
+    return _conv_flops((grid[0], frames, grid[2], grid[3]), cin, cout)
 
 
 def _timed_conv(*args, **kw):
@@ -393,7 +407,8 @@
     K.planes_bound(ph, rows, m0=inp_max, n0=W.dfe_norm, m1=word(0), c1=2.0, vec=P["dfe_tail.bias"])
     h = _timed("conv_fwd", flops, K.conv3d_f16x3, pout, W.dfe, grid, bias=P["dfe_tail.bias"], res=s,
                res_scale=2.0, relu_out=1, out_max=K.p(hmax), out_planes=ph, planes_only=not keep_fp32)
-    o = K.conv3d_thin_out_planes(ph, W.fin_h3, cin, PAD_CIN, grid, bias=P["final_layer.layers.2.conv.bias"])
+    o = K.conv3d_thin_out_planes(ph, W.fin_h3, cin, PAD_CIN, grid, bias=P["final_layer.layers.2.conv.bias"],
+                                 slabs=_live_slabs(grid, pad))
     out = K.swin_post(o, (B, E, T, Y, X), pad)
     saved = dict(u=u, s=s, b=b, pout=pout, h=h, ph=ph, stages=stages, geos=geos, shape=(B, E, T, Y, X), grid=grid,
                  pad=pad, heads=heads, cin=cin, C=C, ntok=ntok, umax=umax, hmax=hmax)
@@ -498,9 +513,10 @@
     flops = _conv_flops(grid, C, C)
     go = K.swin_post_bwd(gout.contiguous(), dtype, pad, PAD_CIN)
 
-    def split_wgrad(x_planes, g_planes, wname):
+    def split_wgrad(x_planes, g_planes, wname, live=None):
         dwp = torch.zeros((27, C, C), dtype=torch.float32, device=dev)
-        _timed("conv_wgrad", flops, K.conv3d_wgrad_f16x3, x_planes, g_planes, grid, dwp)
+        _timed("conv_wgrad", flops if live is None else _wgrad_live_flops(grid, C, C, live), K.conv3d_wgrad_f16x3,
+               x_planes, g_planes, grid, dwp, live=live)
         K.conv_unpack_grad(dwp, grads[wname], C, C)
 
     wf = K.conv_pack(P["final_layer.layers.2.conv.weight"], dtype, 1)
@@ -513,7 +529,7 @@
                         mask_planes=mask_planes, out_max=K.p(ghmax), out_planes=pg, planes_only=True,
                         colsum=grads["dfe_tail.bias"])
     dwp = torch.zeros((27, K.pad32(cin), C), dtype=torch.float32, device=dev)
-    K.conv3d_thin_wgrad_planes(sv["ph"], go, cin, gomax, 0, grid, dwp)
+    K.conv3d_thin_wgrad_planes(sv["ph"], go, cin, gomax, 0, grid, dwp, live=_live_frames(grid, pad, 0))
     K.conv_unpack_grad(dwp, grads["final_layer.layers.2.conv.weight"], cin, C)
     K.colsum(go, grads["final_layer.layers.2.conv.bias"], rows=rows, C=cin, ld=go.shape[-1])
     gh_pl = pg
@@ -524,7 +540,7 @@
     _timed("conv_dgrad", flops, K.conv3d_f16x3, gh_pl, K.conv_pack_f16x3(P["dfe_tail.weight"], 1), grid,
            mask=mask, mask_planes=mask_planes, out_max=K.p(gom), out_planes=pg, planes_only=True,
            colsum=grads[W.stages[-1].pre + "swin_tail.bias"])
-    split_wgrad(sv["pout"], gh_pl, "dfe_tail.weight")
+    split_wgrad(sv["pout"], gh_pl, "dfe_tail.weight", live=_live_frames(grid, pad, 1))
     g_out = None
     for k in reversed(range(len(W.stages))):
         st, ss = W.stages[k], sv["stages"][k]
@@ -539,7 +555,8 @@
         mask, mask_planes = _relu_mask(ss["a"], ss["planes"])
         g = [_timed("conv_dgrad", flops, K.conv3d_f16x3, gp, K.conv_pack_f16x3(P[pre + "swin_tail.weight"], 1),
                     grid, mask=mask, mask_planes=mask_planes)]
-        split_wgrad(ss["planes"], gp, pre + "swin_tail.weight")
+        split_wgrad(ss["planes"], gp, pre + "swin_tail.weight",
+                    live=_live_frames(grid, pad, 2) if gout_pl is not None else None)
         del gp
         d_tok, d_tok_t = _stage_swin_backward(W, st, ss, sv, g, grads)
         if k == 0:
diff --git a/include/dlcs.h b/include/dlcs.h
--- a/include/dlcs.h
+++ b/include/dlcs.h
@@ -198,6 +198,9 @@
 int dlcs_conv3d_k3_wgrad_f16x3(const void* xplanes, const void* gplanes, float* dw_packed, int64_t B, int64_t D,
                                int64_t H, int64_t W, void* workspace, size_t workspace_bytes,
                                dlcs_stream_t stream);
+int dlcs_conv3d_k3_wgrad_f16x3_live(const void* xplanes, const void* gplanes, float* dw_packed, int64_t B, int64_t D,
+                                    int64_t H, int64_t W, int64_t t_lo, int64_t t_hi, void* workspace,
+                                    size_t workspace_bytes, dlcs_stream_t stream);
 int dlcs_absmax_f32(const float* x, int64_t n, unsigned* out, dlcs_stream_t stream);
 size_t dlcs_conv3d_thin_pack_f16x3_bytes(int kind);
 int dlcs_conv3d_thin_pack_f16x3(const float* wpacked, int64_t cout, int64_t cout_pad, int64_t cin, int64_t cin_pad,
@@ -221,6 +224,15 @@
                                         const unsigned* thin_max, int big_is_co, float* dw_packed, int64_t cout_pad,
                                         int64_t cin_pad, int64_t B, int64_t D, int64_t H, int64_t W, void* workspace,
                                         size_t workspace_bytes, dlcs_stream_t stream);
+int dlcs_conv3d_thin_out_planes_f16x3_slabs(const void* xplanes, const void* wthin, const float* bias, float* out,
+                                            int64_t cout, int64_t cout_ld, int64_t B, int64_t D, int64_t H, int64_t W,
+                                            int accumulate, int relu_out, int64_t tb0, int64_t tb1,
+                                            dlcs_stream_t stream);
+int dlcs_conv3d_thin_wgrad_planes_f16x3_live(const void* bigplanes, const float* thin, int64_t thin_ch,
+                                             int64_t thin_ld, const unsigned* thin_max, int big_is_co,
+                                             float* dw_packed, int64_t cout_pad, int64_t cin_pad, int64_t B, int64_t D,
+                                             int64_t H, int64_t W, int64_t t_lo, int64_t t_hi, void* workspace,
+                                             size_t workspace_bytes, dlcs_stream_t stream);
 int dlcs_conv3d_unpack_wgrad(const float* dw_packed, float* grad, int64_t cout, int64_t cin, int64_t cout_pad,
                              int64_t cin_pad, int accumulate, dlcs_stream_t stream);
 
```

New measurement: 4.670 (median of 6 runs). +1.8%, better.
